# ufukpage/TripleD-Exploring-Depth-Estimation-with-Self-Supervised-Representation-Learning

Hardware: AMD Instinct MI355X
Metric: train imgs/sec at KITTI 192x640 bs=12/GPU (higher is better)
Workload: dtype bf16 convs (MFMA) + f32 loss kernels

## Files before the change

include/tripled_hip.h:

```cpp
#ifndef TRIPLED_HIP_H
#define TRIPLED_HIP_H

#include <stddef.h>
#include <stdint.h>

#ifdef __cplusplus
extern "C" {
#endif

#define TD_ABI_VERSION 3
#define TD_MAX_SRC 4

#define TD_OK 0
#define TD_ERR_BAD_ARG (-1)
#define TD_ERR_UNSUPPORTED (-2)
#define TD_ERR_LAUNCH (-3)
#define TD_ERR_WORKSPACE (-4)

typedef void* td_stream_t;

int td_abi_version(void);
const char* td_error_string(int code);
const char* td_last_hip_error(void);

int td_photo_num_blocks(int B, int H, int W);
int td_photo_bwd_num_blocks(int B, int H, int W);

int td_pack_rgbx(const float* img, int B, int H, int W, float* out, td_stream_t stream);

int td_photo_identity(const float* tgt, const float* const* src, int n_src,
                      int B, int H, int W, float* idloss, float* tgt_rgbx, float* const* src_rgbx, td_stream_t stream);

int td_photo_fwd(const float* tgt, const float* const* src, int n_src,
                 const float* disp, const float* P, const float* invK,
                 const float* idloss, const float* noise,
                 int B, int H, int W, int hs, int ws,
                 float min_depth, float max_depth,
                 uint8_t* argmin, float* warped, float* min_map, float* partial, float* coef,
                 td_stream_t stream);

int td_photo_bwd(const float* tgt, const float* const* src, const float* tgt_rgbx, const float* const* src_rgbx, int n_src,
                 const float* disp, const float* P, const float* invK,
                 const uint8_t* argmin, const float* coef, int automask,
                 const float* gscale, float inv_count,
                 int B, int H, int W, int hs, int ws,
                 float min_depth, float max_depth,
                 float* d_up, float* dP_partial, td_stream_t stream);

int td_upsample_adjoint(const float* d_up, int B, int H, int W, int hs, int ws,
                        float* d_disp, int accumulate, td_stream_t stream);
int td_upsample_adjoint_planes(const float* d_up, int n_planes, int B, int H, int W, int hs, int ws,
                               float* d_disp, int accumulate, td_stream_t stream);

int td_reduce_dP(const float* dP_partial, int n_src, int B, int H, int W,
                 float* dP , td_stream_t stream);

int td_sum_scaled(const float* partial, int n, float scale, float* out, td_stream_t stream);

int td_area_downsample(const float* img, int B, int C, int H, int W, int h, int w,
                       float* out, td_stream_t stream);

int td_smooth_num_blocks(int B, int h, int w);

int td_smooth_fwd(const float* disp, const float* img, int B, int h, int w, int normalize,
                  float* mean, float* partial, td_stream_t stream);

int td_smooth_finish(const float* partial, int B, int h, int w, float weight, float* loss,
                     td_stream_t stream);

int td_smooth_bwd(const float* disp, const float* img, const float* mean,
                  int B, int h, int w, int normalize,
                  const float* gscale, float weight,
                  float* g_hat, float* dot_partial, float* d_disp, int accumulate,
                  td_stream_t stream);

#define TD_DTYPE_F32 0
#define TD_DTYPE_BF16 1

int td_maxpool5_fwd(const void* in, int dtype, int N, int H, int W, int C, void* out, uint8_t* idx,
                    td_stream_t stream);
int td_maxpool5_bwd(const void* grad_out, const uint8_t* idx, int dtype, int N, int H, int W, int C,
                    void* grad_in, td_stream_t stream);
int td_maxpool5_bwd_add(const void* grad_out, const uint8_t* idx, const void* add, int dtype, int N, int H, int W, int C,
                        void* grad_in, td_stream_t stream);

int td_maxpool3s2_fwd(const void* in, int dtype, int N, int H, int W, int C, void* out, uint8_t* idx,
                      td_stream_t stream);
int td_maxpool3s2_bwd(const void* grad_out, const uint8_t* idx, int dtype, int N, int H, int W, int C,
                      void* grad_in, td_stream_t stream);

int td_join_fwd(const void* a, const void* b, const void* tail, int dtype, long long npix, int C0, int C1, int C2,
                void* out, td_stream_t stream);
int td_join_bwd(const void* grad_out, int dtype, long long npix, int C0, int C1, int C2, void* grad_a, void* grad_b,
                void* grad_tail, td_stream_t stream);
int td_join_up2_fwd(const void* a, const void* b_half, const void* tail, int dtype, int N, int H, int W, int C0, int C1,
                    int C2, void* out, td_stream_t stream);
int td_join_up2_bwd(const void* grad_out, int dtype, int N, int H, int W, int C0, int C1, int C2, void* grad_a,
                    void* grad_b_half, void* grad_tail, td_stream_t stream);

long long td_bn_workspace_floats(long long M, int groups, int C);
int td_bn_fwd(const void* x, const void* residual, int dtype, const float* gamma, const float* beta,
              float* running_mean, float* running_var, float momentum, float eps, int relu, long long M, int groups,
              int C, void* y, float* save_mean, float* save_invstd, float* workspace, td_stream_t stream);
int td_bn_bwd(const void* dy, const void* x, const void* y, int dtype, const float* gamma, const float* beta, const float* save_mean,
              const float* save_invstd, int relu, long long M, int groups, int C, void* dx, void* dresidual,
              float* dgamma, float* dbeta, float* workspace, td_stream_t stream);

int td_conv1x1_stat_rows(long long M, int groups, int N);
int td_conv1x1_fwd(const void* x, const void* w, long long M, int groups, int K, int N, int Hi, int Wi, int stride, void* y,
                   float* stat_partials, td_stream_t stream);
int td_conv3x3_fwd(const void* x, const void* w, int B, int groups, int Hi, int Wi, int Cin, int N, int stride, int pad, void* y,
                   float* stat_partials, td_stream_t stream);
long long td_conv3x3_wgrad_workspace_floats(int B, int Ho, int Wo, int C, int N);
int td_conv3x3_wgrad(const void* dy, const void* x, int B, int Ho, int Wo, int C, int N, int pad, int dw_dtype, void* dw,
                     float* workspace, td_stream_t stream);
long long td_conv1x1_wgrad_workspace_floats(long long M, int K, int N);
int td_conv1x1_wgrad(const void* dy, const void* x, long long M, int K, int N, int Hi, int Wi, int stride, int dw_dtype, void* dw,
                     float* workspace, td_stream_t stream);
int td_conv1x1_wgrad_group(int n, const void* const* dy, const void* const* x, const long long* M, const int* K, const int* N,
                           const int* Hi, const int* Wi, const int* stride, const int* dw_dtype, void* const* dw,
                           float* const* workspace, td_stream_t stream);
int td_bn_fwd_from_partials(const void* x, const void* residual, int dtype, const float* gamma, const float* beta,
                            float* running_mean, float* running_var, float momentum, float eps, int relu, long long M,
                            int groups, int C, float* partials, int stat_rows, void* y, float* save_mean,
                            float* save_invstd, td_stream_t stream);

long long td_bias_act_workspace_floats(long long M, int C);
int td_bias_act_fwd(const void* y, const void* bias, int bias_dtype, int dtype, long long M, int C, int act, void* a, td_stream_t stream);
int td_bias_act_bwd(const void* g, const void* a, int dtype, long long M, int C, int act, void* gy, void* dbias, int dbias_dtype,
                    float* workspace, td_stream_t stream);

int td_adam_flat(float* w, const float* grad, float* exp_avg, float* exp_avg_sq, void* lowp, long long n, long long n_lowp,
                 const float* step, const float* lr_dev, float lr_host, double beta1, double beta2, float eps, const float* total_norm,
                 float max_norm, td_stream_t stream);

int td_gather_flat(const void* const* srcs, const long long* dst_offsets, const long long* numels, int n, int src_dtype, float* flat,
                   td_stream_t stream);

int td_bn_partial_rows(long long M, int groups, int C);
int td_bn_fwd_partials(const void* x, int dtype, long long M, int groups, int C, float* partials, td_stream_t stream);
int td_bn_bwd_partials(const void* dy, const void* x, const void* y, int dtype, const float* gamma, const float* beta,
                       const float* save_mean, const float* save_invstd, int relu, long long M, int groups, int C, float* partials,
                       td_stream_t stream);
int td_bn_bwd_from_partials(const void* dy, const void* x, const void* y, int dtype, const float* gamma, const float* beta,
                            const float* save_mean, const float* save_invstd, int relu, long long M, int groups, int C,
                            float* partials, int stat_rows, void* dx, void* dresidual, float* dgamma, float* dbeta,
                            td_stream_t stream);
int td_conv1x1_fwd_bnrelu(const void* z, const void* w, long long M, int groups, int K, int N, float* in_partials, int in_rows,
                          const float* gamma, const float* beta, float* running_mean, float* running_var, float momentum, float eps,
                          float* save_mean, float* save_invstd, void* a_side, void* y, float* stat_partials, td_stream_t stream);
int td_conv1x1_dgrad(const void* dy, const void* w, long long M, int groups, int Cout, int Cin, const void* residual, void* dx,
                     td_stream_t stream);
int td_conv1x1_fwd_sum(const void* x, const void* w, long long M, int K, int N, const void* run_in, void* y, void* run_out,
                       td_stream_t stream);
int td_conv1x1_dgrad_bnsums(const void* dy, const void* w, long long M, int groups, int Cout, int Cin, const void* z,
                            const float* gamma, const float* beta, const float* save_mean, const float* save_invstd, void* dx,
                            float* out_partials, td_stream_t stream);
int td_conv1x1_dgrad_bnbwd(const void* g, const void* z, const void* w, long long M, int groups, int Cout, int Cin, float* in_partials,
                           int in_rows, const float* gamma, const float* beta, const float* save_mean, const float* save_invstd,
                           float* dgamma, float* dbeta, void* dz_side, const void* residual, void* dx, td_stream_t stream);

int td_bn_sync_fwd_sums(const void* x, int dtype, long long M, int groups, int C, float* sums, float* workspace,
                        td_stream_t stream);
int td_bn_sync_fwd_apply(const void* x, const void* residual, int dtype, const float* sums, const float* count,
                         const float* gamma, const float* beta, float* running_mean, float* running_var, float momentum,
                         float eps, int relu, long long M, int groups, int C, void* y, float* save_mean,
                         float* save_invstd, td_stream_t stream);
int td_bn_sync_bwd_sums(const void* dy, const void* x, const void* y, int dtype, const float* gamma, const float* beta,
                        const float* save_mean, const float* save_invstd, int relu, long long M, int groups, int C,
                        float* sums, float* workspace, td_stream_t stream);
int td_bn_sync_bwd_dx(const void* dy, const void* x, const void* y, int dtype, const float* local_sums,
                      const float* global_sums, const float* count, const float* gamma, const float* beta,
                      const float* save_mean, const float* save_invstd, int relu, long long M, int groups, int C,
                      void* dx, void* dresidual, float* dgamma, float* dbeta, float* coef, td_stream_t stream);

int td_edge_weights(const float* img, int B, int h, int w, float a, const float* scale6, float* Wt,
                    td_stream_t stream);
int td_featreg_num_blocks(int B, int h, int w, int C);
int td_featreg_fwd(const void* feat, int dtype, const float* Wt, int B, int h, int w, int C,
                   float* partial, td_stream_t stream);
int td_featreg_bwd(const void* feat, int dtype, const float* Wt, const float* gscale, int B, int h, int w,
                   int C, void* grad, td_stream_t stream);

int td_recon_num_tasks(int B, int h, int w);
int td_recon_fwd(const float* x, const float* y, const float* hole, int B, int h, int w,
                 float* partial, td_stream_t stream);
int td_recon_bwd(const float* x, const float* y, const float* hole, const float* gscale, int B, int h,
                 int w, float* dx, td_stream_t stream);

int td_reflpad1_fwd(const void* in, int dtype, int N, int H, int W, int C, void* out, td_stream_t stream);
int td_reflpad1_bwd(const void* grad_out, int dtype, int N, int H, int W, int C, void* grad_in,
                    td_stream_t stream);

int td_up2_reflpad1_fwd(const void* in, int dtype, int N, int H, int W, int C, void* out, td_stream_t stream);
int td_up2_reflpad1_bwd(const void* grad_out, int dtype, int N, int H, int W, int C, void* grad_in,
                        td_stream_t stream);

int td_featwarp_num_blocks(int B, int h, int w);
int td_featwarp_fwd(const void* tgt, const void* const* src, int n_src, int dtype, const float* disp,
                    const float* P, const float* invK, int B, int h, int w, int C, int hs, int ws,
                    float min_depth, float max_depth, uint8_t* argmin, float* partial, td_stream_t stream);
int td_featwarp_bwd(const void* tgt, const void* const* src, int n_src, int dtype, const float* disp,
                    const float* P, const float* invK, const uint8_t* argmin, const float* gscale,
                    float inv_count, int B, int h, int w, int C, int hs, int ws, float min_depth,
                    float max_depth, void* d_tgt, int* const* d_src, float* d_up, float* dP_partial,
                    td_stream_t stream);
int td_featwarp_dsrc_finish(const int* acc, const float* gscale, float inv_count, int C, long long n, int dtype, void* out,
                            td_stream_t stream);
int td_reduce_partials(const float* partial, int n_src, int B, int blocks_per_sample, float* dP,
                       td_stream_t stream);

int td_l1map_fwd(const void* pred, int dtype, const long long* pred_strides, const float* target, int B, int C,
                 int H, int W, float weight, float* out, td_stream_t stream);
int td_l1map_bwd(const void* pred, int dtype, const long long* pred_strides, const float* target,
                 const float* gmap, int B, int C, int H, int W, float weight, void* dpred, td_stream_t stream);

int td_rgb2lab(const float* rgb, int B, int H, int W, float l_cent, float l_norm, float ab_norm, float* lab,
               td_stream_t stream);

int td_pose_fwd(const float* axisangle, const float* translation, const int* invert, const float* K,
                int n_pairs, int B, float* T, float* P, td_stream_t stream);
int td_pose_bwd(const float* axisangle, const float* translation, const int* invert, const float* K,
                int n_pairs, int B, const float* gT, const float* gP, float* g_axisangle,
                float* g_translation, td_stream_t stream);

int td_color_jitter(const uint8_t* frames_u8, const float* aug, int N, int H, int W, float* means_scratch, float* color,
                    float* color_aug, td_stream_t stream);

int td_fp8_num_blocks(long long n);
int td_fp8_amax_partials(const void* x, int dtype, long long n, float* partials, td_stream_t stream);
int td_fp8_quantize(const void* x, int dtype, long long n, const float* partials, uint8_t* q, float* inv_scale,
                    td_stream_t stream);

int td_infer_preprocess(const uint8_t* img_u8, int B, int H0, int W0, int h, int w, int mirror, float* out,
                        td_stream_t stream);
int td_disp_postprocess(const void* disp, int dtype, int B, int h, int w, int paired, int H0, int W0, float a, float b,
                        float depth_scale, float* disp_out, float* depth_out, td_stream_t stream);
int td_colorize(const float* x, int B, long long n, const float* vmin, const float* vmax, const uint8_t* lut, uint8_t* out,
                td_stream_t stream);

#define TD_STEREO_SCALE_FACTOR 36
long long td_eval_depth_workspace_bytes(int B, int Hmax, int Wmax);
int td_eval_depth(const void* disp, int dtype, int B, int h, int w, float a, float b, const float* gt, int Hmax, int Wmax,
                  const int* sizes, const int* crops, float min_depth, float max_depth, int stereo, void* workspace,
                  long long workspace_bytes, float* metrics, int* counts, td_stream_t stream);
long long td_masked_median_workspace_bytes(int B);
int td_masked_median(const float* values, int B, long long n, void* workspace, long long workspace_bytes, float* median,
                     int* count, td_stream_t stream);

int td_pose_pairs_u8(const uint8_t* frames, int n, int H, int W, int first, int count, int dtype, void* out, long long out_first,
                     td_stream_t stream);
int td_odom_trajectory(const void* rel, int rel_f64, int n, double* poses, td_stream_t stream);
int td_odom_snippet_ate(const void* rel, int rel_f64, const double* gt_poses, int n, int track_length, double* ates,
                        td_stream_t stream);
int td_odom_sequence_errors(const double* gt_poses, const double* pred_poses, int m, const double* lengths, int n_lengths, int step,
                            int align_scale, double* dist, double* rows, uint8_t* valid, double* summary, td_stream_t stream);

int td_lanczos_resize_u8(const uint8_t* src, const int* meta, const int* meta_host, const int* tables, long long table_ints,
                         const int* desc, int n_sizes, int N, int Hc, int Wc, int H, int W, uint8_t* dst, int* status,
                         td_stream_t stream);

int td_lanczos_resize_u8_indexed(const uint8_t* store, long long store_bytes, const long long* offsets, const long long* offsets_host,
                                 const int* meta, const int* meta_host, const int* tables, long long table_ints, const int* desc,
                                 int n_sizes, int N, int H, int W, uint8_t* dst, int* status, td_stream_t stream);

int td_cloud_keys(const float* depth, const uint8_t* color, const double* poses, const double* inv_K, int B, int H, int W,
                  double depth_scale, double pose_scale, double inv_voxel, int stride, int border, double min_depth, double max_range,
                  float edge, long long* key, unsigned long long* payload, long long* stats, td_stream_t stream);
int td_cloud_heads(const long long* keys, long long N, int* flags, td_stream_t stream);
int td_cloud_reduce_packed(const long long* keys, const long long* seg, const long long* perm, const unsigned long long* payload,
                           long long n_src, long long N, long long V, long long* out_keys, long long* sums, td_stream_t stream);
int td_cloud_reduce_rows(const long long* keys, const long long* seg, const long long* perm, const long long* rows, long long n_src,
                         long long N, long long V, long long* out_keys, long long* sums, td_stream_t stream);
int td_cloud_finish(const long long* keys, const long long* sums, long long V, double voxel, long long min_count, float* xyz,
                    uint8_t* rgb, int* count, uint8_t* keep, td_stream_t stream);

int td_cloud_views(const float* depth, const double* poses, const double* K, const double* inv_K, int N, int H, int W, int c0, int c1,
                   int lo, int hi, int radius, int min_views, double tol, double depth_scale, double pose_scale, double min_depth,
                   double max_range, long long* key, unsigned long long* payload, uint8_t* votes, long long* stats, td_stream_t stream);

long long td_velo_depth_workspace_bytes(int B, int Hmax, int Wmax);
int td_velo_depth(const float* points, const long long* offsets, int B, const double* P, const int* sizes, int Hmax, int Wmax,
                  int vel_depth, void* workspace, long long workspace_bytes, float* gt, long long* stats, td_stream_t stream);

long long td_cloud_render_workspace_bytes(int C, int H, int W);
int td_cloud_render(const float* xyz, const uint8_t* rgb, long long V, const double* poses, const double* K, int C, int H, int W,
                    double pose_scale, double z_near, double z_far, double splat, int ortho, int bg_r, int bg_g, int bg_b,
                    void* workspace, long long workspace_bytes, float* depth, uint8_t* color, int* index, long long* stats,
                    td_stream_t stream);

int td_scan_keys(const float* points, long long n, const long long* offsets, int S, const double* Tr, const double* poses,
                 const double* K, int H, int W, double min_depth, double max_range, double inv_voxel, long long* key,
                 unsigned long long* payload, long long* stats, td_stream_t stream);
int td_nn_query(const double* query, long long N, const double* points, const long long* order, long long M, const long long* cell_key,
                const long long* cell_start, long long C, double tau, const double* thr2, int K, double* d2, long long* index,
                long long* counts, td_stream_t stream);

int td_cloud_transform(const double* src, long long N, double c, const double* R, const double* t, double* out, td_stream_t stream);
long long td_icp_moments_workspace(long long N);
int td_icp_moments(const double* cur, long long N, const double* ref, long long M, const long long* index, const double* d2, double trim2,
                   const double* origin, void* workspace, long long workspace_bytes, double* out, td_stream_t stream);

int td_cloud_normals(const double* query, long long N, const double* points, long long M, const long long* cell_key,
                     const long long* cell_start, long long C, double tau, double radius, double Q, long long min_neighbours,
                     double max_curvature, double* normal, double* curvature, long long* count, long long* counters, td_stream_t stream);
long long td_icp_plane_moments_workspace(long long N);
int td_icp_plane_moments(const double* cur, long long N, const double* ref, const double* normals, long long M, const long long* index,
                         const double* d2, double trim2, const double* origin, void* workspace, long long workspace_bytes, double* out,
                         td_stream_t stream);

int td_normals_orient(const float* xyz, const float* normal, long long V, const double* poses, int C, double pose_scale,
                      float* out_normal, int* camera, long long* stats, td_stream_t stream);
int td_cloud_render_surfels(const float* xyz, const uint8_t* rgb, const float* normal, long long V, const double* poses, const double* K,
// ... 9 lines not shown
```

tripled-exploring-depth-estimation-with-self-supervised-representation-learning_amd/csrc/td_bn.hip:

```cpp
#include <hip/hip_bf16.h>

#include "td_common.h"
#include "td_vec8.h"

namespace td {

constexpr int BN_RY = 32;
constexpr int BN_UNROLL = 4;
constexpr int BN_THREADS = 256;

template <typename T, int MODE>
__global__ __launch_bounds__(BN_THREADS) void bn_partials_kernel(const T* __restrict__ x, const T* __restrict__ dy,
                                                                 const T* __restrict__ y, const float* __restrict__ mean,
                                                                 const float* __restrict__ invstd, const float* __restrict__ gamma,
                                                                 const float* __restrict__ beta,
                                                                 long long M, int C, int rows_per_split, int relu,
                                                                 float* __restrict__ ws) {
  __shared__ float lds[2][BN_RY][64 + 1];
  const int tid = threadIdx.x, cx = tid & 7, ry = tid >> 3;
  const int cg = blockIdx.x, s = blockIdx.y, grp = blockIdx.z;
  const long long base = (long long)grp * M;
  const long long r0 = base + (long long)s * rows_per_split;
  const long long r1 = (r0 + rows_per_split < base + M) ? r0 + rows_per_split : base + M;
  const size_t col = (size_t)cg * 64 + (size_t)cx * 8;
  ws += (size_t)grp * gridDim.y * C * 2;
  if (MODE == 1) { mean += (size_t)grp * C; invstd += (size_t)grp * C; }
  float a[8], b[8], mu[8], sc[8], sh[8];
#pragma unroll
  for (int i = 0; i < 8; ++i) { a[i] = 0.f; b[i] = 0.f; mu[i] = 0.f; sc[i] = 0.f; sh[i] = 0.f; }
  if (MODE == 1) {
#pragma unroll
    for (int i = 0; i < 8; ++i) mu[i] = mean[col + i];
    if (relu == 2) {
#pragma unroll
      for (int i = 0; i < 8; ++i) {
        sc[i] = gamma[col + i] * invstd[col + i];
        sh[i] = beta[col + i] - mu[i] * sc[i];
      }
    }
  }
  for (long long r = r0 + ry; r < r1; r += BN_UNROLL * BN_RY) {
    float vx[BN_UNROLL][8], vg[BN_UNROLL][8], vy[BN_UNROLL][8];
    bool ok[BN_UNROLL];
#pragma unroll
    for (int u = 0; u < BN_UNROLL; ++u) {
      const long long rr = r + (long long)u * BN_RY;
      ok[u] = rr < r1;
      const size_t off = (size_t)(ok[u] ? rr : r) * C + col;
      load8(x + off, vx[u]);
      if (MODE == 1) {
        load8(dy + off, vg[u]);
        if (relu == 1) load8(y + off, vy[u]);
      }
    }
#pragma unroll
    for (int u = 0; u < BN_UNROLL; ++u) {
#pragma unroll
      for (int i = 0; i < 8; ++i) {
        if (MODE == 0) {
          const float t = ok[u] ? vx[u][i] : 0.f;
          a[i] += t;
          b[i] = fmaf(t, t, b[i]);
        } else {
          float g = vg[u][i];
          if (relu == 1) g = vy[u][i] <= 0.f ? 0.f : g;
          if (relu == 2) g = fmaf(vx[u][i], sc[i], sh[i]) <= 0.f ? 0.f : g;
          g = ok[u] ? g : 0.f;
          a[i] += g;
          b[i] = fmaf(g, vx[u][i] - mu[i], b[i]);
        }
      }
    }
  }
#pragma unroll
  for (int i = 0; i < 8; ++i) { lds[0][ry][cx * 8 + i] = a[i]; lds[1][ry][cx * 8 + i] = b[i]; }
  __syncthreads();
  if (tid < 128) {
    const int which = tid >> 6, c = tid & 63;
    float acc = 0.f;
#pragma unroll
    for (int j = 0; j < BN_RY; ++j) acc += lds[which][j][c];
    ws[((size_t)s * C + (size_t)cg * 64 + c) * 2 + which] = acc;
  }
}

constexpr int BN_FIN_CH = 16;
constexpr int BN_FIN_PARTS = 16;
constexpr int BN_FIN_THREADS = BN_FIN_CH * BN_FIN_PARTS;
__device__ __forceinline__ void bn_sum_partials(const float* __restrict__ ws, int S, int C, int cg, float& A, float& B) {
  __shared__ float red[2][BN_FIN_PARTS][BN_FIN_CH];
  const int tid = threadIdx.x, c = tid % BN_FIN_CH, part = tid / BN_FIN_CH;
  float a = 0.f, b = 0.f;
  int s = part;
  for (; s + 11 * BN_FIN_PARTS < S; s += 12 * BN_FIN_PARTS) {
    float2 p[12];
#pragma unroll
    for (int u = 0; u < 12; ++u) p[u] = *reinterpret_cast<const float2*>(ws + ((size_t)(s + u * BN_FIN_PARTS) * C + (size_t)cg * BN_FIN_CH + c) * 2);
#pragma unroll
    for (int u = 0; u < 12; ++u) { a += p[u].x; b += p[u].y; }
  }
  for (; s < S; s += BN_FIN_PARTS) {
    const float2 p = *reinterpret_cast<const float2*>(ws + ((size_t)s * C + (size_t)cg * BN_FIN_CH + c) * 2);
    a += p.x;
    b += p.y;
  }
  red[0][part][c] = a;
  red[1][part][c] = b;
  __syncthreads();
  A = 0.f;
  B = 0.f;
  if (tid < BN_FIN_CH) {
#pragma unroll
    for (int j = 0; j < BN_FIN_PARTS; ++j) { A += red[0][j][c]; B += red[1][j][c]; }
  }
}

__global__ __launch_bounds__(BN_FIN_THREADS) void bn_shrink_kernel(float* __restrict__ ws, int S, int C, int Sq) {
  const int q = blockIdx.y, grp = blockIdx.z;
  float* w = ws + ((size_t)grp * S + (size_t)q * Sq) * C * 2;
  const int rows = S - q * Sq < Sq ? S - q * Sq : Sq;
  float A, B;
  bn_sum_partials(w, rows, C, blockIdx.x, A, B);
  if (threadIdx.x < BN_FIN_CH) {
    float* o = w + ((size_t)blockIdx.x * BN_FIN_CH + threadIdx.x) * 2;
    o[0] = A;
    o[1] = B;
  }
}

__global__ __launch_bounds__(64) void bn_stats_from_sums_kernel(const float* __restrict__ sums, const float* __restrict__ count,
                                                               int C, int G, float eps, float momentum,
                                                               float* __restrict__ running_mean, float* __restrict__ running_var,
                                                               float* __restrict__ save_mean, float* __restrict__ save_invstd) {
  const int c = blockIdx.x * 64 + threadIdx.x;
  if (c >= C) return;
  const double M = (double)count[0];
  for (int grp = 0; grp < G; ++grp) {
    const size_t i = (size_t)grp * C + c;
    const double m = (double)sums[i * 2] / M;
    double var = (double)sums[i * 2 + 1] / M - m * m;
    var = var > 0.0 ? var : 0.0;
    save_mean[i] = (float)m;
    save_invstd[i] = (float)(1.0 / sqrt(var + (double)eps));
    if (running_mean) {
      const double unbiased = M > 1.0 ? var * (M / (M - 1.0)) : var;
      running_mean[c] = (float)((1.0 - momentum) * running_mean[c] + momentum * m);
      running_var[c] = (float)((1.0 - momentum) * running_var[c] + momentum * unbiased);
    }
  }
}

__global__ __launch_bounds__(64) void bn_coef_from_sums_kernel(const float* __restrict__ local, const float* __restrict__ global,
                                                              const float* __restrict__ count, int C, int G,
                                                              const float* __restrict__ gamma, const float* __restrict__ mean,
                                                              const float* __restrict__ invstd, float* __restrict__ dgamma,
                                                              float* __restrict__ dbeta, float* __restrict__ coef) {
  const int c = blockIdx.x * 64 + threadIdx.x;
  if (c >= C) return;
  const float inv_m = 1.f / count[0];
  float dg_tot = 0.f, db_tot = 0.f;
  for (int grp = 0; grp < G; ++grp) {
    const size_t i = (size_t)grp * C + c;
    const float is = invstd[i], mu = mean[i];
    dg_tot += local[i * 2 + 1] * is;
    db_tot += local[i * 2];
    const float A = global[i * 2], dg = global[i * 2 + 1] * is;
    const float k0 = gamma[c] * is;
    const float k1 = -k0 * is * dg * inv_m;
    coef[i * 3 + 0] = k0;
    coef[i * 3 + 1] = k1;
    coef[i * 3 + 2] = -k0 * A * inv_m - k1 * mu;
  }
  dgamma[c] = dg_tot;
  dbeta[c] = db_tot;
}

constexpr int BN_PRO_MAX_S = 96;
constexpr int BN_PRO_PARTS = BN_THREADS / 64;
constexpr int BN_PRO_DEPTH = BN_PRO_MAX_S / BN_PRO_PARTS;
__device__ __forceinline__ void bn_tile_sums(const float* __restrict__ ws, int S, int stride, int C, int ct, float& A, float& B) {
  __shared__ float red[2][BN_PRO_PARTS][64];
  const int tid = threadIdx.x, c = tid & 63, part = tid >> 6;
  const float* p = ws + ((size_t)ct * 64 + c) * 2;
  float2 v[BN_PRO_DEPTH];
#pragma unroll
  for (int u = 0; u < BN_PRO_DEPTH; ++u) {
    const int row = part + BN_PRO_PARTS * u;
    v[u] = *reinterpret_cast<const float2*>(p + (size_t)(row < S ? row : 0) * stride * C * 2);
  }
  float a = 0.f, b = 0.f;
#pragma unroll
  for (int u = 0; u < BN_PRO_DEPTH; ++u) {
    const bool ok = part + BN_PRO_PARTS * u < S;
    a += ok ? v[u].x : 0.f;
    b += ok ? v[u].y : 0.f;
  }
  red[0][part][c] = a;
  red[1][part][c] = b;
  __syncthreads();
  A = 0.f;
  B = 0.f;
  if (tid < 64) {
#pragma unroll
    for (int j = 0; j < BN_PRO_PARTS; ++j) { A += red[0][j][c]; B += red[1][j][c]; }
  }
  __syncthreads();
}

struct BnFinFwd {
  const float* ws;
  int S, stride, rows, G;
  float eps, momentum;
  float* running_mean;
  float* running_var;
  float* save_mean;
  float* save_invstd;
};
struct BnFinBwd {
  const float* ws;
  int S, stride, rows, G;
  float* dgamma;
  float* dbeta;
};
// ... 122 lines not shown
  const int grp = blockIdx.z;
  const long long base = (long long)grp * M;
  const long long r0 = base + (long long)blockIdx.y * rows_per_split;
  const long long r1 = (r0 + rows_per_split < base + M) ? r0 + rows_per_split : base + M;
  const size_t col = (size_t)blockIdx.x * 64 + (size_t)cx * 8;
  Raw8<T> qx[BN_UNROLL], qg[BN_UNROLL], qy[BN_UNROLL];
  bool ok[BN_UNROLL];
#define BN_DX_ISSUE(rr0)                                                          \
  {                                                                               \
    _Pragma("unroll") for (int u = 0; u < BN_UNROLL; ++u) {                       \
      const long long rr = (rr0) + (long long)u * BN_RY;                          \
      ok[u] = rr < r1;                                                            \
      const size_t off = (size_t)(ok[u] ? rr : (rr0)) * C + col;                  \
      qx[u].load(x + off);                                                        \
      qg[u].load(dy + off);                                                       \
      if (relu == 1) qy[u].load(y + off);                                         \
    }                                                                             \
  }
  long long r = r0 + ry;
  if (r < r1) BN_DX_ISSUE(r)
  float k0[8], k1[8], k2[8];
  if constexpr (FIN) {
    __shared__ float s_k[3][64];
    const int c = blockIdx.x * 64 + (tid & 63);
    const float inv_m = 1.f / (float)M;
    float A, B;
    bn_tile_sums(fin.ws + (size_t)grp * fin.rows * C * 2, fin.S, fin.stride, C, blockIdx.x, A, B);
    if (tid < 64) {
      const float is = invstd[(size_t)grp * C + c], mu = mean[(size_t)grp * C + c];
      const float dg = B * is;
      const float c0 = gamma[c] * is;
      const float c1 = -c0 * is * dg * inv_m;
      s_k[0][tid] = c0;
      s_k[1][tid] = c1;
      s_k[2][tid] = -c0 * A * inv_m - c1 * mu;
    }
    if (blockIdx.y == 0 && blockIdx.z == 0) {
      float dg_tot = 0.f, db_tot = 0.f;
      for (int g2 = 0; g2 < fin.G; ++g2) {
        float A2 = A, B2 = B;
        if (g2 != 0) bn_tile_sums(fin.ws + (size_t)g2 * fin.rows * C * 2, fin.S, fin.stride, C, blockIdx.x, A2, B2);
        if (tid < 64) {
          dg_tot += B2 * invstd[(size_t)g2 * C + c];
          db_tot += A2;
        }
      }
      if (tid < 64) { fin.dgamma[c] = dg_tot; fin.dbeta[c] = db_tot; }
    }
    __syncthreads();
#pragma unroll
    for (int i = 0; i < 8; ++i) { k0[i] = s_k[0][cx * 8 + i]; k1[i] = s_k[1][cx * 8 + i]; k2[i] = s_k[2][cx * 8 + i]; }
  } else {
    coef += (size_t)grp * C * 3;
#pragma unroll
    for (int i = 0; i < 8; ++i) {
      k0[i] = coef[(col + i) * 3 + 0];
      k1[i] = coef[(col + i) * 3 + 1];
      k2[i] = coef[(col + i) * 3 + 2];
    }
  }
  mean += (size_t)grp * C;
  invstd += (size_t)grp * C;
  float sc[8], sh[8];
#pragma unroll
  for (int i = 0; i < 8; ++i) { sc[i] = 0.f; sh[i] = 0.f; }
  if (relu == 2) {
#pragma unroll
    for (int i = 0; i < 8; ++i) {
      sc[i] = gamma[col + i] * invstd[col + i];
      sh[i] = beta[col + i] - mean[col + i] * sc[i];
    }
  }
  for (; r < r1; r += BN_UNROLL * BN_RY) {
    float vx[BN_UNROLL][8], vg[BN_UNROLL][8], vy[BN_UNROLL][8];
    bool okc[BN_UNROLL];
#pragma unroll
    for (int u = 0; u < BN_UNROLL; ++u) {
      qx[u].unpack(vx[u]);
      qg[u].unpack(vg[u]);
      if (relu == 1) qy[u].unpack(vy[u]);
      okc[u] = ok[u];
    }
    const long long rn = r + BN_UNROLL * BN_RY;
    if (rn < r1) BN_DX_ISSUE(rn)
#pragma unroll
    for (int u = 0; u < BN_UNROLL; ++u) {
      float o[8], g[8];
#pragma unroll
      for (int i = 0; i < 8; ++i) {
        g[i] = vg[u][i];
        if (relu == 1) g[i] = vy[u][i] <= 0.f ? 0.f : g[i];
        if (relu == 2) g[i] = fmaf(vx[u][i], sc[i], sh[i]) <= 0.f ? 0.f : g[i];
        o[i] = fmaf(k0[i], g[i], fmaf(k1[i], vx[u][i], k2[i]));
      }
      if (okc[u]) {
        const size_t off = (size_t)(r + (long long)u * BN_RY) * C + col;
        store8(dx + off, o);
        if (dres) store8(dres + off, g);
      }
    }
  }
#undef BN_DX_ISSUE
}

constexpr int BN_STAT_BLOCKS = 512;
static inline int bn_splits(long long M, int C, int target_blocks, int cap) {
  const int groups = C / 64;
  long long s = (target_blocks + groups - 1) / groups;
  const long long by_rows = (M + 63) / 64;
  if (s > by_rows) s = by_rows;
  if (s > cap) s = cap;
  if (s < 1) s = 1;
  return (int)s;
}
static inline int bn_rows_per_split(long long M, int S) {
  const long long r = (M + S - 1) / S;
  return (int)((r + BN_RY - 1) / BN_RY * BN_RY);
}

BnRows bn_shrink_partials_to(float* partials, int S, int G, int C, int max_rows, hipStream_t st) {
  if (S <= max_rows) return {S, 1};
  const int Sq = (S + max_rows - 1) / max_rows, Q = (S + Sq - 1) / Sq;
  hipLaunchKernelGGL(bn_shrink_kernel, dim3(C / BN_FIN_CH, Q, G), dim3(BN_FIN_THREADS), 0, st, partials, S, C, Sq);
  return {Q, Sq};
}
static BnRows shrink_partials(float* partials, int S, int G, int C, hipStream_t st) {
  return bn_shrink_partials_to(partials, S, G, C, BN_PRO_MAX_S, st);
}

template <typename T>
static void launch_bn_finalize_apply(const void* x, const void* res, const float* gamma, const float* beta, float* rmean, float* rvar,
                                     float momentum, float eps, int relu, long long Mg, int G, int C, float* partials, int S, void* y,
                                     float* save_mean, float* save_invstd, hipStream_t st) {
  const BnRows rows = shrink_partials(partials, S, G, C, st);
  const int S2 = bn_splits(Mg, C, BN_STAT_BLOCKS, 4096), rps2 = bn_rows_per_split(Mg, S2);
  const dim3 grid(C / 64, (unsigned)((Mg + rps2 - 1) / rps2), G);
  const BnFinFwd fin = {partials, rows.n, rows.stride, S, G, eps, momentum, rmean, rvar, save_mean, save_invstd};
  hipLaunchKernelGGL((bn_apply_kernel<T, true>), grid, dim3(BN_THREADS), 0, st, (const T*)x, (const T*)res, gamma, beta,
                     (const float*)nullptr, (const float*)nullptr, Mg, C, rps2, relu, (T*)y, fin);
}

static inline int bn_stat_splits(long long Mg, int C) {
  const int S = bn_splits(Mg, C, BN_STAT_BLOCKS, 512);
  if (S > 16 && (C / 64) * 16 >= 128) return bn_splits(Mg, C, (C / 64) * 16, 16);
  return S;
}
static inline int bn_stat_rows(long long Mg, int C) {
  const int S = bn_stat_splits(Mg, C), rps = bn_rows_per_split(Mg, S);
  return (int)((Mg + rps - 1) / rps);
}

template <typename T>
static int run_bn_partials(int mode, const void* x, const void* dy, const void* y, const float* gamma, const float* beta, const float* mean,
                           const float* invstd, int relu, long long M, int G, int C, float* ws, hipStream_t st) {
  const long long Mg = M / G;
  const int S = bn_stat_splits(Mg, C), rps = bn_rows_per_split(Mg, S);
  const int S_eff = (int)((Mg + rps - 1) / rps);
  if (mode == 0)
    hipLaunchKernelGGL((bn_partials_kernel<T, 0>), dim3(C / 64, S_eff, G), dim3(BN_THREADS), 0, st, (const T*)x, (const T*)nullptr,
                       (const T*)nullptr, (const float*)nullptr, (const float*)nullptr, (const float*)nullptr, (const float*)nullptr, Mg, C,
                       rps, 0, ws);
  else
    hipLaunchKernelGGL((bn_partials_kernel<T, 1>), dim3(C / 64, S_eff, G), dim3(BN_THREADS), 0, st, (const T*)x, (const T*)dy,
                       (const T*)y, mean, invstd, gamma, beta, Mg, C, rps, relu, ws);
  return hipGetLastError() == hipSuccess ? TD_OK : TD_ERR_LAUNCH;
}

template <typename T>
static int run_bn_dx_from_partials(const void* dy, const void* x, const void* y, const float* gamma, const float* beta, const float* mean,
                                   const float* invstd, int relu, long long M, int G, int C, float* partials, int S, void* dx, void* dres,
                                   float* dgamma, float* dbeta, hipStream_t st) {
  const long long Mg = M / G;
  const BnRows rows = shrink_partials(partials, S, G, C, st);
  const int S2 = bn_splits(Mg, C, BN_STAT_BLOCKS, 4096), rps2 = bn_rows_per_split(Mg, S2);
  const dim3 grid(C / 64, (unsigned)((Mg + rps2 - 1) / rps2), G);
  const BnFinBwd fin = {partials, rows.n, rows.stride, S, G, dgamma, dbeta};
  hipLaunchKernelGGL((bn_dx_kernel<T, true>), grid, dim3(BN_THREADS), 0, st, (const T*)dy, (const T*)x, (const T*)y, (const float*)nullptr,
                     mean, invstd, gamma, beta, Mg, C, rps2, relu, (T*)dx, (T*)dres, fin);
  return hipGetLastError() == hipSuccess ? TD_OK : TD_ERR_LAUNCH;
}

template <typename T>
static int run_bn_fwd(const void* x, const void* res, const float* gamma, const float* beta, float* rmean, float* rvar,
                      float momentum, float eps, int relu, long long M, int G, int C, void* y, float* save_mean, float* save_invstd,
                      float* ws, hipStream_t st) {
  const long long Mg = M / G;
  const int S = bn_splits(Mg, C, BN_STAT_BLOCKS, 512), rps = bn_rows_per_split(Mg, S);
  const int S_eff = (int)((Mg + rps - 1) / rps);
  hipLaunchKernelGGL((bn_partials_kernel<T, 0>), dim3(C / 64, S_eff, G), dim3(BN_THREADS), 0, st, (const T*)x, (const T*)nullptr,
                     (const T*)nullptr, (const float*)nullptr, (const float*)nullptr, (const float*)nullptr, (const float*)nullptr, Mg, C, rps, 0, ws);
  launch_bn_finalize_apply<T>(x, res, gamma, beta, rmean, rvar, momentum, eps, relu, Mg, G, C, ws, S_eff, y, save_mean, save_invstd, st);
  return hipGetLastError() == hipSuccess ? TD_OK : TD_ERR_LAUNCH;
}

template <typename T>
static int run_bn_bwd(const void* dy, const void* x, const void* y, const float* gamma, const float* beta, const float* mean, const float* invstd,
                      int relu, long long M, int G, int C, void* dx, void* dres, float* dgamma, float* dbeta, float* ws, hipStream_t st) {
  const long long Mg = M / G;
  const int S = bn_splits(Mg, C, BN_STAT_BLOCKS, 512), rps = bn_rows_per_split(Mg, S);
  const int S_eff = (int)((Mg + rps - 1) / rps);
  hipLaunchKernelGGL((bn_partials_kernel<T, 1>), dim3(C / 64, S_eff, G), dim3(BN_THREADS), 0, st, (const T*)x, (const T*)dy,
                     (const T*)y, mean, invstd, gamma, beta, Mg, C, rps, relu, ws);
  const BnRows rows = shrink_partials(ws, S_eff, G, C, st);
  const int S2 = bn_splits(Mg, C, BN_STAT_BLOCKS, 4096), rps2 = bn_rows_per_split(Mg, S2);
  const dim3 grid(C / 64, (unsigned)((Mg + rps2 - 1) / rps2), G);
  const BnFinBwd fin = {ws, rows.n, rows.stride, S_eff, G, dgamma, dbeta};
  hipLaunchKernelGGL((bn_dx_kernel<T, true>), grid, dim3(BN_THREADS), 0, st, (const T*)dy, (const T*)x, (const T*)y, (const float*)nullptr,
                     mean, invstd, gamma, beta, Mg, C, rps2, relu, (T*)dx, (T*)dres, fin);
  return hipGetLastError() == hipSuccess ? TD_OK : TD_ERR_LAUNCH;
}

template <typename T>
static int run_bn_local_sums(int mode, const void* x, const void* dy, const void* y, const float* gamma, const float* beta,
                             const float* mean, const float* invstd, int relu, long long M, int G, int C, float* sums, float* ws,
                             hipStream_t st) {
  const long long Mg = M / G;
  const int S = bn_splits(Mg, C, BN_STAT_BLOCKS, 512), rps = bn_rows_per_split(Mg, S);
  const int S_eff = (int)((Mg + rps - 1) / rps);
  if (mode == 0)
    hipLaunchKernelGGL((bn_partials_kernel<T, 0>), dim3(C / 64, S_eff, G), dim3(BN_THREADS), 0, st, (const T*)x, (const T*)nullptr,
                       (const T*)nullptr, (const float*)nullptr, (const float*)nullptr, (const float*)nullptr, (const float*)nullptr, Mg, C,
                       rps, 0, ws);
  else
    hipLaunchKernelGGL((bn_partials_kernel<T, 1>), dim3(C / 64, S_eff, G), dim3(BN_THREADS), 0, st, (const T*)x, (const T*)dy,
                       (const T*)y, mean, invstd, gamma, beta, Mg, C, rps, relu, ws);
  const BnRows rows = shrink_partials(ws, S_eff, G, C, st);
  hipLaunchKernelGGL(bn_tile_reduce_kernel, dim3(C / 64), dim3(BN_THREADS), 0, st, (const float*)ws, rows.n, rows.stride, S_eff, C, G, sums);
  return hipGetLastError() == hipSuccess ? TD_OK : TD_ERR_LAUNCH;
}

template <typename T>
static int run_bn_sync_apply(const void* x, const void* res, const float* sums, const float* count, const float* gamma, const float* beta,
                             float* rmean, float* rvar, float momentum, float eps, int relu, long long M, int G, int C, void* y,
                             float* save_mean, float* save_invstd, hipStream_t st) {
  const long long Mg = M / G;
  hipLaunchKernelGGL(bn_stats_from_sums_kernel, dim3(C / 64), dim3(64), 0, st, sums, count, C, G, eps, momentum, rmean, rvar, save_mean,
                     save_invstd);
  const int S2 = bn_splits(Mg, C, 2048 / G, 4096), rps2 = bn_rows_per_split(Mg, S2);
  hipLaunchKernelGGL((bn_apply_kernel<T, false>), dim3(C / 64, (unsigned)((Mg + rps2 - 1) / rps2), G), dim3(BN_THREADS), 0, st, (const T*)x,
                     (const T*)res, gamma, beta, (const float*)save_mean, (const float*)save_invstd, Mg, C, rps2, relu, (T*)y, BnFinFwd{});
  return hipGetLastError() == hipSuccess ? TD_OK : TD_ERR_LAUNCH;
}

template <typename T>
static int run_bn_sync_dx(const void* dy, const void* x, const void* y, const float* local, const float* global, const float* count,
                          const float* gamma, const float* beta, const float* mean, const float* invstd, int relu, long long M, int G,
                          int C, void* dx, void* dres, float* dgamma, float* dbeta, float* coef, hipStream_t st) {
  const long long Mg = M / G;
  hipLaunchKernelGGL(bn_coef_from_sums_kernel, dim3(C / 64), dim3(64), 0, st, local, global, count, C, G, gamma, mean, invstd, dgamma, dbeta,
                     coef);
  const int S2 = bn_splits(Mg, C, 2048 / G, 4096), rps2 = bn_rows_per_split(Mg, S2);
  hipLaunchKernelGGL((bn_dx_kernel<T, false>), dim3(C / 64, (unsigned)((Mg + rps2 - 1) / rps2), G), dim3(BN_THREADS), 0, st, (const T*)dy,
                     (const T*)x, (const T*)y, (const float*)coef, mean, invstd, gamma, beta, Mg, C, rps2, relu, (T*)dx, (T*)dres, BnFinBwd{});
  return hipGetLastError() == hipSuccess ? TD_OK : TD_ERR_LAUNCH;
}

}

static bool bn_shape_ok(long long M, int G, int C) { return G >= 1 && G <= 64 && M > 0 && C > 0 && M % G == 0; }

extern "C" long long td_bn_workspace_floats(long long M, int groups, int C) {
  if (!bn_shape_ok(M, groups, C) || C % 64 != 0) return 0;
  const int S = td::bn_splits(M / groups, C, td::BN_STAT_BLOCKS, 512);
  return ((long long)2 * S * C + (long long)3 * C) * groups;
}

extern "C" int td_bn_fwd(const void* x, const void* residual, int dtype, const float* gamma, const float* beta,
                         float* running_mean, float* running_var, float momentum, float eps, int relu, long long M, int groups,
                         int C, void* y, float* save_mean, float* save_invstd, float* workspace, td_stream_t stream) {
  if (!x || !gamma || !beta || !y || !save_mean || !save_invstd || !workspace || !bn_shape_ok(M, groups, C)) return TD_ERR_BAD_ARG;
  if ((running_mean == nullptr) != (running_var == nullptr)) return TD_ERR_BAD_ARG;
  if (C % 64 != 0 || M * (long long)C >= (1ll << 40)) return TD_ERR_UNSUPPORTED;
  if (dtype == TD_DTYPE_BF16)
    return td::run_bn_fwd<__hip_bfloat16>(x, residual, gamma, beta, running_mean, running_var, momentum, eps, relu, M, groups, C, y,
                                          save_mean, save_invstd, workspace, (hipStream_t)stream);
  if (dtype == TD_DTYPE_F32)
    return td::run_bn_fwd<float>(x, residual, gamma, beta, running_mean, running_var, momentum, eps, relu, M, groups, C, y, save_mean,
                                 save_invstd, workspace, (hipStream_t)stream);
  return TD_ERR_UNSUPPORTED;
}

extern "C" int td_bn_bwd(const void* dy, const void* x, const void* y, int dtype, const float* gamma, const float* beta, const float* save_mean,
                         const float* save_invstd, int relu, long long M, int groups, int C, void* dx, void* dresidual,
                         float* dgamma, float* dbeta, float* workspace, td_stream_t stream) {
  if (!dy || !x || !gamma || !save_mean || !save_invstd || !dx || !dgamma || !dbeta || !workspace || !bn_shape_ok(M, groups, C))
    return TD_ERR_BAD_ARG;
  if (relu < 0 || relu > 1) return TD_ERR_BAD_ARG;
  if (relu && !y && (!beta || dresidual)) return TD_ERR_BAD_ARG;
  if (relu && !y) relu = 2;
  if (C % 64 != 0 || M * (long long)C >= (1ll << 40)) return TD_ERR_UNSUPPORTED;
  if (dtype == TD_DTYPE_BF16)
    return td::run_bn_bwd<__hip_bfloat16>(dy, x, y, gamma, beta, save_mean, save_invstd, relu, M, groups, C, dx, dresidual, dgamma, dbeta,
                                          workspace, (hipStream_t)stream);
  if (dtype == TD_DTYPE_F32)
    return td::run_bn_bwd<float>(dy, x, y, gamma, beta, save_mean, save_invstd, relu, M, groups, C, dx, dresidual, dgamma, dbeta, workspace,
                                 (hipStream_t)stream);
  return TD_ERR_UNSUPPORTED;
}

extern "C" int td_bn_fwd_from_partials(const void* x, const void* residual, int dtype, const float* gamma, const float* beta,
                                       float* running_mean, float* running_var, float momentum, float eps, int relu, long long M,
                                       int groups, int C, float* partials, int stat_rows, void* y, float* save_mean,
                                       float* save_invstd, td_stream_t stream) {
  if (!x || !gamma || !beta || !y || !save_mean || !save_invstd || !partials || stat_rows < 1 || !bn_shape_ok(M, groups, C))
    return TD_ERR_BAD_ARG;
  if ((running_mean == nullptr) != (running_var == nullptr)) return TD_ERR_BAD_ARG;
  if (C % 64 != 0 || M * (long long)C >= (1ll << 40)) return TD_ERR_UNSUPPORTED;
  if (dtype != TD_DTYPE_BF16 && dtype != TD_DTYPE_F32) return TD_ERR_UNSUPPORTED;
  hipStream_t st = (hipStream_t)stream;
  const long long Mg = M / groups;
  if (dtype == TD_DTYPE_BF16)
    td::launch_bn_finalize_apply<__hip_bfloat16>(x, residual, gamma, beta, running_mean, running_var, momentum, eps, relu, Mg, groups, C, partials,
                                                 stat_rows, y, save_mean, save_invstd, st);
  else
    td::launch_bn_finalize_apply<float>(x, residual, gamma, beta, running_mean, running_var, momentum, eps, relu, Mg, groups, C, partials, stat_rows,
                                        y, save_mean, save_invstd, st);
  return hipGetLastError() == hipSuccess ? TD_OK : TD_ERR_LAUNCH;
}

extern "C" int td_bn_partial_rows(long long M, int groups, int C) {
  if (!bn_shape_ok(M, groups, C) || C % 64 != 0) return 0;
  return td::bn_stat_rows(M / groups, C);
}

extern "C" int td_bn_fwd_partials(const void* x, int dtype, long long M, int groups, int C, float* partials, td_stream_t stream) {
  if (!x || !partials || !bn_shape_ok(M, groups, C)) return TD_ERR_BAD_ARG;
  if (C % 64 != 0 || M * (long long)C >= (1ll << 40)) return TD_ERR_UNSUPPORTED;
  if (dtype == TD_DTYPE_BF16)
    return td::run_bn_partials<__hip_bfloat16>(0, x, nullptr, nullptr, nullptr, nullptr, nullptr, nullptr, 0, M, groups, C, partials, (hipStream_t)stream);
  if (dtype == TD_DTYPE_F32)
    return td::run_bn_partials<float>(0, x, nullptr, nullptr, nullptr, nullptr, nullptr, nullptr, 0, M, groups, C, partials, (hipStream_t)stream);
  return TD_ERR_UNSUPPORTED;
}

extern "C" int td_bn_bwd_partials(const void* dy, const void* x, const void* y, int dtype, const float* gamma, const float* beta,
                                  const float* save_mean, const float* save_invstd, int relu, long long M, int groups, int C,
                                  float* partials, td_stream_t stream) {
  if (!dy || !x || !gamma || !save_mean || !save_invstd || !partials || !bn_shape_ok(M, groups, C)) return TD_ERR_BAD_ARG;
  if (relu < 0 || relu > 1 || (relu && !y && !beta)) return TD_ERR_BAD_ARG;
  if (relu && !y) relu = 2;
  if (C % 64 != 0 || M * (long long)C >= (1ll << 40)) return TD_ERR_UNSUPPORTED;
  if (dtype == TD_DTYPE_BF16)
    return td::run_bn_partials<__hip_bfloat16>(1, x, dy, y, gamma, beta, save_mean, save_invstd, relu, M, groups, C, partials, (hipStream_t)stream);
  if (dtype == TD_DTYPE_F32)
    return td::run_bn_partials<float>(1, x, dy, y, gamma, beta, save_mean, save_invstd, relu, M, groups, C, partials, (hipStream_t)stream);
  return TD_ERR_UNSUPPORTED;
}

extern "C" int td_bn_bwd_from_partials(const void* dy, const void* x, const void* y, int dtype, const float* gamma, const float* beta,
                                       const float* save_mean, const float* save_invstd, int relu, long long M, int groups, int C,
                                       float* partials, int stat_rows, void* dx, void* dresidual, float* dgamma, float* dbeta,
                                       td_stream_t stream) {
  if (!dy || !x || !gamma || !save_mean || !save_invstd || !dx || !dgamma || !dbeta || !partials || stat_rows < 1 || !bn_shape_ok(M, groups, C))
    return TD_ERR_BAD_ARG;
  if (relu < 0 || relu > 1) return TD_ERR_BAD_ARG;
  if (relu && !y && (!beta || dresidual)) return TD_ERR_BAD_ARG;
  if (relu && !y) relu = 2;
  if (C % 64 != 0 || M * (long long)C >= (1ll << 40)) return TD_ERR_UNSUPPORTED;
  if (dtype == TD_DTYPE_BF16)
    return td::run_bn_dx_from_partials<__hip_bfloat16>(dy, x, y, gamma, beta, save_mean, save_invstd, relu, M, groups, C, partials, stat_rows,
                                                       dx, dresidual, dgamma, dbeta, (hipStream_t)stream);
  if (dtype == TD_DTYPE_F32)
    return td::run_bn_dx_from_partials<float>(dy, x, y, gamma, beta, save_mean, save_invstd, relu, M, groups, C, partials, stat_rows, dx,
                                              dresidual, dgamma, dbeta, (hipStream_t)stream);
  return TD_ERR_UNSUPPORTED;
}


extern "C" int td_bn_sync_fwd_sums(const void* x, int dtype, long long M, int groups, int C, float* sums, float* workspace,
                                   td_stream_t stream) {
  if (!x || !sums || !workspace || !bn_shape_ok(M, groups, C)) return TD_ERR_BAD_ARG;
  if (C % 64 != 0 || M * (long long)C >= (1ll << 40)) return TD_ERR_UNSUPPORTED;
  if (dtype == TD_DTYPE_BF16)
    return td::run_bn_local_sums<__hip_bfloat16>(0, x, nullptr, nullptr, nullptr, nullptr, nullptr, nullptr, 0, M, groups, C, sums, workspace,
                                                 (hipStream_t)stream);
  if (dtype == TD_DTYPE_F32)
    return td::run_bn_local_sums<float>(0, x, nullptr, nullptr, nullptr, nullptr, nullptr, nullptr, 0, M, groups, C, sums, workspace,
                                        (hipStream_t)stream);
  return TD_ERR_UNSUPPORTED;
}

extern "C" int td_bn_sync_fwd_apply(const void* x, const void* residual, int dtype, const float* sums, const float* count,
                                    const float* gamma, const float* beta, float* running_mean, float* running_var, float momentum,
                                    float eps, int relu, long long M, int groups, int C, void* y, float* save_mean, float* save_invstd,
                                    td_stream_t stream) {
  if (!x || !sums || !count || !gamma || !beta || !y || !save_mean || !save_invstd || !bn_shape_ok(M, groups, C)) return TD_ERR_BAD_ARG;
  if ((running_mean == nullptr) != (running_var == nullptr)) return TD_ERR_BAD_ARG;
  if (C % 64 != 0 || M * (long long)C >= (1ll << 40)) return TD_ERR_UNSUPPORTED;
  if (dtype == TD_DTYPE_BF16)
    return td::run_bn_sync_apply<__hip_bfloat16>(x, residual, sums, count, gamma, beta, running_mean, running_var, momentum, eps, relu, M,
                                                 groups, C, y, save_mean, save_invstd, (hipStream_t)stream);
  if (dtype == TD_DTYPE_F32)
    return td::run_bn_sync_apply<float>(x, residual, sums, count, gamma, beta, running_mean, running_var, momentum, eps, relu, M, groups, C,
                                        y, save_mean, save_invstd, (hipStream_t)stream);
  return TD_ERR_UNSUPPORTED;
}

extern "C" int td_bn_sync_bwd_sums(const void* dy, const void* x, const void* y, int dtype, const float* gamma, const float* beta,
                                   const float* save_mean, const float* save_invstd, int relu, long long M, int groups, int C,
                                   float* sums, float* workspace, td_stream_t stream) {
  if (!dy || !x || !gamma || !save_mean || !save_invstd || !sums || !workspace || !bn_shape_ok(M, groups, C)) return TD_ERR_BAD_ARG;
  if (relu < 0 || relu > 1 || (relu && !y && !beta)) return TD_ERR_BAD_ARG;
  if (relu && !y) relu = 2;
  if (C % 64 != 0 || M * (long long)C >= (1ll << 40)) return TD_ERR_UNSUPPORTED;
  if (dtype == TD_DTYPE_BF16)
    return td::run_bn_local_sums<__hip_bfloat16>(1, x, dy, y, gamma, beta, save_mean, save_invstd, relu, M, groups, C, sums, workspace,
                                                 (hipStream_t)stream);
  if (dtype == TD_DTYPE_F32)
    return td::run_bn_local_sums<float>(1, x, dy, y, gamma, beta, save_mean, save_invstd, relu, M, groups, C, sums, workspace,
                                        (hipStream_t)stream);
  return TD_ERR_UNSUPPORTED;
}

extern "C" int td_bn_sync_bwd_dx(const void* dy, const void* x, const void* y, int dtype, const float* local_sums, const float* global_sums,
                                 const float* count, const float* gamma, const float* beta, const float* save_mean,
                                 const float* save_invstd, int relu, long long M, int groups, int C, void* dx, void* dresidual,
                                 float* dgamma, float* dbeta, float* coef, td_stream_t stream) {
  if (!dy || !x || !local_sums || !global_sums || !count || !gamma || !save_mean || !save_invstd || !dx || !dgamma || !dbeta || !coef ||
      !bn_shape_ok(M, groups, C))
    return TD_ERR_BAD_ARG;
  if (relu < 0 || relu > 1 || (relu && !y && (!beta || dresidual))) return TD_ERR_BAD_ARG;
  if (relu && !y) relu = 2;
  if (C % 64 != 0 || M * (long long)C >= (1ll << 40)) return TD_ERR_UNSUPPORTED;
  if (dtype == TD_DTYPE_BF16)
    return td::run_bn_sync_dx<__hip_bfloat16>(dy, x, y, local_sums, global_sums, count, gamma, beta, save_mean, save_invstd, relu, M, groups,
                                              C, dx, dresidual, dgamma, dbeta, coef, (hipStream_t)stream);
  if (dtype == TD_DTYPE_F32)
    return td::run_bn_sync_dx<float>(dy, x, y, local_sums, global_sums, count, gamma, beta, save_mean, save_invstd, relu, M, groups, C, dx,
                                     dresidual, dgamma, dbeta, coef, (hipStream_t)stream);
  return TD_ERR_UNSUPPORTED;
}
```

tripled-exploring-depth-estimation-with-self-supervised-representation-learning_amd/csrc/td_conv1x1.hip:

```cpp
#include "td_conv_tile.h"

namespace td {

struct ConvRows {
  int Wo, HoWo, Wi, HiWi, stride;
};

__device__ __forceinline__ long long cv_src_row(long long m, const ConvRows& g) {
  if (g.stride == 1) return m;
  const long long b = m / g.HoWo;
  const int rem = (int)(m - b * g.HoWo);
  const int ho = rem / g.Wo, wo = rem - ho * g.Wo;
  return b * g.HiWi + (long long)ho * g.stride * g.Wi + (long long)wo * g.stride;
}

struct CvFuse {
  const __hip_bfloat16* a2;
  const float* part;
  int part_S, part_stride, part_rows;
  const float* gamma;
  const float* beta;
  float* mean;
  float* invstd;
  float* rmean;
  float* rvar;
  float momentum, eps;
  float* dgamma;
  float* dbeta;
  __hip_bfloat16* a_side;
  int G;
  CvEpi ep;
};

constexpr int CV_PRO_MAX_K = 512;
constexpr int CV_PRO_MAX_S = 16;

__device__ __forceinline__ uint4 cv_pro1(uint4 x, const float* sc, const float* sh) {
  const unsigned w[4] = {x.x, x.y, x.z, x.w};
  unsigned o[4];
#pragma unroll
  for (int e = 0; e < 4; ++e) {
    float v0 = fmaf(bf2f((unsigned short)(w[e] & 0xffff)), sc[2 * e], sh[2 * e]);
    float v1 = fmaf(bf2f((unsigned short)(w[e] >> 16)), sc[2 * e + 1], sh[2 * e + 1]);
    v0 = v0 < 0.f ? 0.f : v0;
    v1 = v1 < 0.f ? 0.f : v1;
    o[e] = (unsigned)f2bf(v0) | ((unsigned)f2bf(v1) << 16);
  }
  return make_uint4(o[0], o[1], o[2], o[3]);
}
__device__ __forceinline__ uint4 cv_pro2(uint4 g, uint4 z, const float* k0, const float* k1, const float* k2, const float* sc,
                                         const float* sh) {
  const unsigned gw[4] = {g.x, g.y, g.z, g.w}, zw[4] = {z.x, z.y, z.z, z.w};
  unsigned o[4];
#pragma unroll
  for (int e = 0; e < 4; ++e) {
    const float z0 = bf2f((unsigned short)(zw[e] & 0xffff)), z1 = bf2f((unsigned short)(zw[e] >> 16));
    float g0 = bf2f((unsigned short)(gw[e] & 0xffff)), g1 = bf2f((unsigned short)(gw[e] >> 16));
    g0 = fmaf(z0, sc[2 * e], sh[2 * e]) <= 0.f ? 0.f : g0;
    g1 = fmaf(z1, sc[2 * e + 1], sh[2 * e + 1]) <= 0.f ? 0.f : g1;
    const float v0 = fmaf(k0[2 * e], g0, fmaf(k1[2 * e], z0, k2[2 * e]));
    const float v1 = fmaf(k0[2 * e + 1], g1, fmaf(k1[2 * e + 1], z1, k2[2 * e + 1]));
    o[e] = (unsigned)f2bf(v0) | ((unsigned)f2bf(v1) << 16);
  }
  return make_uint4(o[0], o[1], o[2], o[3]);
}

__device__ __forceinline__ void cv_sum_rows(const float* __restrict__ part, int S, int stride, int K, int c, float& A, float& B) {
  float2 v[CV_PRO_MAX_S];
#pragma unroll
  for (int u = 0; u < CV_PRO_MAX_S; ++u)
    v[u] = *reinterpret_cast<const float2*>(part + ((size_t)(u < S ? u : 0) * stride * K + c) * 2);
  A = 0.f;
  B = 0.f;
#pragma unroll
  for (int u = 0; u < CV_PRO_MAX_S; ++u) {
    A += u < S ? v[u].x : 0.f;
    B += u < S ? v[u].y : 0.f;
  }
}

template <int BM, int BN, bool BT, int PRO, int EPI, bool DEEP>
__global__ __launch_bounds__(CV_THREADS, 2) void conv1x1_mfma_kernel(
    const __hip_bfloat16* __restrict__ x, const __hip_bfloat16* __restrict__ w, __hip_bfloat16* __restrict__ y,
    float* __restrict__ ws, long long Mg, int K, int N, int tiles_per_group, int total_blocks, ConvRows geom, CvFuse fz) {
  using T = CvTile<BM, BN, BT>;
  constexpr int A_BYTES = T::A_BYTES, STAGE = T::STAGE, TN = T::TN, TM = T::TM;
  __shared__ __attribute__((aligned(16))) unsigned char lds[T::LDS_BYTES];
  __shared__ __attribute__((aligned(16))) float s_pro[PRO == 0 ? 4 : (PRO == 1 ? 2 : 5) * CV_PRO_MAX_K];

  const int tid = threadIdx.x, lane = tid & 63, wid = tid >> 6;
  const int wm = wid >> 1, wn = wid & 1, l31 = lane & 31, h = lane >> 5;

  const int L = cv_xcd_tile(blockIdx.x, total_blocks);
  const int NT = N / BN;
  const int nt = L % NT, mt = L / NT;
  const int grp = mt / tiles_per_group, s = mt - grp * tiles_per_group;
  const long long row0 = (long long)grp * Mg + (long long)s * BM;
  const int rows_valid = (int)((Mg - (long long)s * BM) < BM ? (Mg - (long long)s * BM) : BM);
  const int n0 = nt * BN;

  const int lc = tid & 7, lr = tid >> 3;
  constexpr int NA = BM / 32, NB = BN / 32;
  auto a_off = [&](int i) {
    int r = lr + 32 * i;
    r = r < rows_valid ? r : rows_valid - 1;
    return cv_src_row(row0 + r, geom) * (long long)K + lc * 8;
  };
  const long long oa0 = a_off(0), oa1 = a_off(1), oa2 = NA > 2 ? a_off(2) : oa0, oa3 = NA > 2 ? a_off(3) : oa0;
  const __hip_bfloat16 *pa0 = x + oa0, *pa1 = x + oa1, *pa2 = x + oa2, *pa3 = x + oa3;
  constexpr int CPR = BN / 8, RPP = CV_THREADS / CPR;
  const int bc = tid % CPR, br = tid / CPR;
  const __hip_bfloat16* pb0 = BT ? w + (long long)br * N + n0 + bc * 8 : w + (long long)(n0 + lr) * K + lc * 8;
  const long long bstep = BT ? (long long)RPP * N : 32ll * K;
  const __hip_bfloat16 *pb1 = pb0 + bstep, *pb2 = pb0 + (NB > 2 ? 2 : 0) * bstep, *pb3 = pb0 + (NB > 2 ? 3 : 0) * bstep;
  const long long bkt = BT ? (long long)CV_BK * N : (long long)CV_BK;
#define CV_DECL(S)                                                                          \
  uint4 ra0##S, ra1##S, ra2##S, ra3##S, rb0##S, rb1##S, rb2##S, rb3##S, rz0##S, rz1##S, rz2##S, rz3##S; \
  ra0##S = ra1##S = ra2##S = ra3##S = rb0##S = rb1##S = rb2##S = rb3##S = make_uint4(0, 0, 0, 0);       \
  rz0##S = rz1##S = rz2##S = rz3##S = make_uint4(0, 0, 0, 0);
  CV_DECL(A)
  CV_DECL(B)
#define CV_LD(p, kt) (*reinterpret_cast<const uint4*>((p) + (kt) * CV_BK))
#define CV_LDB(p, kt) (*reinterpret_cast<const uint4*>((p) + (kt) * bkt))
#define CV_LOAD_GLOBAL(kt, S)                                  \
  {                                                            \
    ra0##S = CV_LD(pa0, kt);                                   \
    ra1##S = CV_LD(pa1, kt);                                   \
    if (NA > 2) { ra2##S = CV_LD(pa2, kt); ra3##S = CV_LD(pa3, kt); } \
    if constexpr (PRO == 2) {                                  \
      rz0##S = CV_LD(fz.a2 + oa0, kt);                         \
      rz1##S = CV_LD(fz.a2 + oa1, kt);                         \
      if (NA > 2) { rz2##S = CV_LD(fz.a2 + oa2, kt); rz3##S = CV_LD(fz.a2 + oa3, kt); } \
    }                                                          \
    rb0##S = CV_LDB(pb0, kt);                                  \
    rb1##S = CV_LDB(pb1, kt);                                  \
    if (NB > 2) { rb2##S = CV_LDB(pb2, kt); rb3##S = CV_LDB(pb3, kt); } \
  }
#define CV_ST(base, i, v) (*reinterpret_cast<uint4*>((base) + cv_swz(lr + 32 * (i), lc)) = (v))
#define CV_STB(base, i, v)                                                                              \
  {                                                                                                     \
    if constexpr (BT) *reinterpret_cast<uint4*>((base) + (br + RPP * (i)) * T::PITCH_T + bc * 16) = (v); \
    else CV_ST(base, i, v);                                                                             \
  }
#define CV_PRO_A(kt, S)                                                                                 \
  {                                                                                                     \
    if constexpr (PRO != 0) {                                                                           \
      const int c0_ = (kt) * CV_BK + lc * 8;                                                            \
      float q0[8], q1[8], q2[8], q3[8], q4[8];                                                          \
      _Pragma("unroll") for (int e = 0; e < 8; ++e) {                                                   \
        q0[e] = s_pro[0 * CV_PRO_MAX_K + c0_ + e];                                                      \
        q1[e] = s_pro[1 * CV_PRO_MAX_K + c0_ + e];                                                      \
        if constexpr (PRO == 2) {                                                                       \
          q2[e] = s_pro[2 * CV_PRO_MAX_K + c0_ + e];                                                    \
          q3[e] = s_pro[3 * CV_PRO_MAX_K + c0_ + e];                                                    \
          q4[e] = s_pro[4 * CV_PRO_MAX_K + c0_ + e];                                                    \
        }                                                                                               \
      }                                                                                                 \
      if constexpr (PRO == 1) {                                                                         \
        ra0##S = cv_pro1(ra0##S, q0, q1);                                                               \
        ra1##S = cv_pro1(ra1##S, q0, q1);                                                               \
        if (NA > 2) { ra2##S = cv_pro1(ra2##S, q0, q1); ra3##S = cv_pro1(ra3##S, q0, q1); }             \
      } else {                                                                                          \
        ra0##S = cv_pro2(ra0##S, rz0##S, q0, q1, q2, q3, q4);                                           \
        ra1##S = cv_pro2(ra1##S, rz1##S, q0, q1, q2, q3, q4);                                           \
        if (NA > 2) { ra2##S = cv_pro2(ra2##S, rz2##S, q0, q1, q2, q3, q4); ra3##S = cv_pro2(ra3##S, rz3##S, q0, q1, q2, q3, q4); } \
      }                                                                                                 \
      if (fz.a_side && nt == 0) {                                                                       \
        __hip_bfloat16* sd_ = fz.a_side + (row0 + lr) * (long long)K + c0_;                             \
        if (lr < rows_valid) *reinterpret_cast<uint4*>(sd_) = ra0##S;                                   \
        if (lr + 32 < rows_valid) *reinterpret_cast<uint4*>(sd_ + 32ll * K) = ra1##S;                   \
        if (NA > 2) {                                                                                   \
          if (lr + 64 < rows_valid) *reinterpret_cast<uint4*>(sd_ + 64ll * K) = ra2##S;                 \
          if (lr + 96 < rows_valid) *reinterpret_cast<uint4*>(sd_ + 96ll * K) = ra3##S;                 \
        }                                                                                               \
      }                                                                                                 \
    }                                                                                                   \
  }
#define CV_WRITE_LDS(stage, kt, S)                                       \
  {                                                                      \
    unsigned char* base_ = lds + (stage) * STAGE;                        \
    CV_PRO_A(kt, S)                                                      \
    CV_ST(base_, 0, ra0##S);                                             \
    CV_ST(base_, 1, ra1##S);                                             \
    if (NA > 2) { CV_ST(base_, 2, ra2##S); CV_ST(base_, 3, ra3##S); }    \
    CV_STB(base_ + A_BYTES, 0, rb0##S);                                  \
    CV_STB(base_ + A_BYTES, 1, rb1##S);                                  \
    if (NB > 2) { CV_STB(base_ + A_BYTES, 2, rb2##S); CV_STB(base_ + A_BYTES, 3, rb3##S); } \
  }

  CvAcc<BM, BN> acc;
#pragma unroll
  for (int i = 0; i < TN; ++i)
#pragma unroll
    for (int j = 0; j < TM; ++j)
#pragma unroll
      for (int e = 0; e < 16; ++e) acc.v[i][j][e] = 0.f;

  const int nk = K / CV_BK;
  CV_LOAD_GLOBAL(0, A)
  if constexpr (DEEP) CV_LOAD_GLOBAL(nk > 1 ? 1 : 0, B)

  if constexpr (PRO == 1) {
    const float* part = fz.part + (size_t)grp * fz.part_rows * K * 2;
    const bool first = (s == 0 && nt == 0);
    for (int c = tid; c < K; c += CV_THREADS) {
      float A, B;
      cv_sum_rows(part, fz.part_S, fz.part_stride, K, c, A, B);
      const double m = (double)A / (double)Mg;
      double var = (double)B / (double)Mg - m * m;
      var = var > 0.0 ? var : 0.0;
      const float mf = (float)m, isf = (float)(1.0 / sqrt(var + (double)fz.eps));
      const float scv = fz.gamma[c] * isf;
      s_pro[c] = scv;
      s_pro[CV_PRO_MAX_K + c] = fz.beta[c] - mf * scv;
      if (first) {
        fz.mean[(size_t)grp * K + c] = mf;
        fz.invstd[(size_t)grp * K + c] = isf;
      }
      if (fz.rmean && first && grp == 0) {
        double rm = fz.rmean[c], rv = fz.rvar[c];
        for (int g2 = 0; g2 < fz.G; ++g2) {
          float A2 = A, B2 = B;
          if (g2 != 0) cv_sum_rows(fz.part + (size_t)g2 * fz.part_rows * K * 2, fz.part_S, fz.part_stride, K, c, A2, B2);
          const double m2 = (double)A2 / (double)Mg;
          double v2 = (double)B2 / (double)Mg - m2 * m2;
          v2 = v2 > 0.0 ? v2 : 0.0;
          const double unbiased = Mg > 1 ? v2 * ((double)Mg / (double)(Mg - 1)) : v2;
          rm = (double)(float)((1.0 - fz.momentum) * rm + fz.momentum * m2);
          rv = (double)(float)((1.0 - fz.momentum) * rv + fz.momentum * unbiased);
        }
        fz.rmean[c] = (float)rm;
        fz.rvar[c] = (float)rv;
      }
    }
    __syncthreads();
  }
  if constexpr (PRO == 2) {
    const float* part = fz.part + (size_t)grp * fz.part_rows * K * 2;
    const float inv_m = 1.f / (float)Mg;
    const bool first = (s == 0 && nt == 0 && grp == 0);
    for (int c = tid; c < K; c += CV_THREADS) {
      float A, B;
      cv_sum_rows(part, fz.part_S, fz.part_stride, K, c, A, B);
      const float is = fz.invstd[(size_t)grp * K + c], mu = fz.mean[(size_t)grp * K + c];
      const float dg = B * is;
      const float c0 = fz.gamma[c] * is;
      const float c1 = -c0 * is * dg * inv_m;
      s_pro[0 * CV_PRO_MAX_K + c] = c0;
      s_pro[1 * CV_PRO_MAX_K + c] = c1;
      s_pro[2 * CV_PRO_MAX_K + c] = -c0 * A * inv_m - c1 * mu;
      s_pro[3 * CV_PRO_MAX_K + c] = c0;
      s_pro[4 * CV_PRO_MAX_K + c] = fz.beta[c] - mu * c0;
      if (first) {
        float dg_tot = 0.f, db_tot = 0.f;
        for (int g2 = 0; g2 < fz.G; ++g2) {
          float A2 = A, B2 = B;
          if (g2 != 0) cv_sum_rows(fz.part + (size_t)g2 * fz.part_rows * K * 2, fz.part_S, fz.part_stride, K, c, A2, B2);
          dg_tot += B2 * fz.invstd[(size_t)g2 * K + c];
          db_tot += A2;
        }
        fz.dgamma[c] = dg_tot;
        fz.dbeta[c] = db_tot;
      }
    }
    __syncthreads();
  }

  CV_WRITE_LDS(0, 0, A)
  __syncthreads();
  if constexpr (!DEEP) {
    for (int kt = 0; kt < nk; ++kt) {
      const bool more = kt + 1 < nk;
      if (more) CV_LOAD_GLOBAL(kt + 1, A)
      const unsigned char* sa = lds + (kt & 1) * STAGE;
      cv_stage_mfma<BM, BN, BT>(acc, sa, sa + A_BYTES, wm, wn, l31, h);
      if (more) CV_WRITE_LDS((kt + 1) & 1, kt + 1, A)
      __syncthreads();
    }
  } else {
    const int last = nk - 1;
    for (int kt = 0; kt < nk; kt += 2) {
      const int k2 = kt + 2 < last ? kt + 2 : last, k1 = kt + 1 < last ? kt + 1 : last, k3 = kt + 3 < last ? kt + 3 : last;
      CV_LOAD_GLOBAL(k2, A)
      __builtin_amdgcn_sched_barrier(0);
      cv_stage_mfma<BM, BN, BT>(acc, lds, lds + A_BYTES, wm, wn, l31, h);
      CV_WRITE_LDS(1, k1, B)
      __syncthreads();
      if (kt + 1 >= nk) break;
      CV_LOAD_GLOBAL(k3, B)
      __builtin_amdgcn_sched_barrier(0);
      cv_stage_mfma<BM, BN, BT>(acc, lds + STAGE, lds + STAGE + A_BYTES, wm, wn, l31, h);
      CV_WRITE_LDS(0, k2, A)
      __syncthreads();
    }
  }

  CvEpi ep = fz.ep;
  if constexpr (EPI == 2) { ep.mean += (size_t)grp * N; ep.invstd += (size_t)grp * N; }
  cv_epilogue<BM, BN, EPI>(acc, lds, y, ws, row0, rows_valid, n0, N, (long long)grp * tiles_per_group + s, tid, wm, wn, l31, h, ep);
}

#undef CV_LOAD_GLOBAL
#undef CV_DECL
#undef CV_WRITE_LDS
#undef CV_PRO_A
#undef CV_LD
#undef CV_LDB
#undef CV_ST
#undef CV_STB

constexpr int WG_T = 64;
constexpr int WG_PITCH = WG_T * 2 + 64;

typedef __attribute__((ext_vector_type(4))) short cv_s16x4;

__device__ __forceinline__ cv_bf16x8 wg_frag(const unsigned char* tile, int col0, int ks, int lane) {
  const int g = lane >> 4, i = lane & 15;
  const int row = 16 * ks + 8 * (g >> 1) + (i >> 2);
  const unsigned char* p = tile + row * WG_PITCH + (col0 + 16 * (g & 1) + 4 * (i & 3)) * 2;
  typedef __attribute__((address_space(3))) cv_s16x4* lds_ptr;
  const cv_s16x4 lo = __builtin_amdgcn_ds_read_tr16_b64_v4i16((lds_ptr)(p));
  const cv_s16x4 hi = __builtin_amdgcn_ds_read_tr16_b64_v4i16((lds_ptr)(p + 4 * WG_PITCH));
  typedef __attribute__((ext_vector_type(8))) short s16x8;
  const s16x8 v = {lo[0], lo[1], lo[2], lo[3], hi[0], hi[1], hi[2], hi[3]};
  return __builtin_bit_cast(cv_bf16x8, v);
}

constexpr int WG_TILE_BYTES = WG_T * WG_PITCH, WG_STAGE = 2 * WG_TILE_BYTES, WG_LDS_BYTES = 2 * WG_STAGE;

__device__ __forceinline__ void wgrad_block(
    const __hip_bfloat16* __restrict__ dy, const __hip_bfloat16* __restrict__ x, float* __restrict__ part, long long M, int K, int N,
    int rows_per_split, int tiles_n, int tiles_k, ConvRows geom, int L, unsigned char* lds) {
  constexpr int TILE_BYTES = WG_TILE_BYTES, STAGE = WG_STAGE;
  const int tid = threadIdx.x, lane = tid & 63, wid = tid >> 6;
  const int wn = wid >> 1, wk = wid & 1;
  const int nt = L % tiles_n, kt = (L / tiles_n) % tiles_k, sp = L / (tiles_n * tiles_k);
  const int n0 = nt * WG_T, k0 = kt * WG_T;
  const long long m_lo = (long long)sp * rows_per_split;
  const long long m_hi = (m_lo + rows_per_split < M) ? m_lo + rows_per_split : M;
  const int nstage = (int)((m_hi - m_lo + WG_T - 1) / WG_T);

  const int lc = tid & 7, lr = tid >> 3;
  uint4 ry0a, ry1a, rx0a, rx1a, ry0b, ry1b, rx0b, rx1b;
#define WG_LOAD(st, S)                                                                                             \
  {                                                                                                                \
    const long long r0 = m_lo + (long long)(st) * WG_T + lr, r1 = r0 + 32;                                         \
    const uint4 z = make_uint4(0, 0, 0, 0);                                                                        \
    ry0##S = r0 < m_hi ? *reinterpret_cast<const uint4*>(dy + r0 * N + n0 + lc * 8) : z;                           \
    ry1##S = r1 < m_hi ? *reinterpret_cast<const uint4*>(dy + r1 * N + n0 + lc * 8) : z;                           \
    rx0##S = r0 < m_hi ? *reinterpret_cast<const uint4*>(x + cv_src_row(r0, geom) * (long long)K + k0 + lc * 8) : z; \
    rx1##S = r1 < m_hi ? *reinterpret_cast<const uint4*>(x + cv_src_row(r1, geom) * (long long)K + k0 + lc * 8) : z; \
  }
#define WG_WRITE(buf, S)                                                                         \
  {                                                                                              \
    unsigned char* b_ = lds + (buf) * STAGE;                                                     \
    *reinterpret_cast<uint4*>(b_ + lr * WG_PITCH + lc * 16) = ry0##S;                            \
    *reinterpret_cast<uint4*>(b_ + (lr + 32) * WG_PITCH + lc * 16) = ry1##S;                     \
    *reinterpret_cast<uint4*>(b_ + TILE_BYTES + lr * WG_PITCH + lc * 16) = rx0##S;               \
    *reinterpret_cast<uint4*>(b_ + TILE_BYTES + (lr + 32) * WG_PITCH + lc * 16) = rx1##S;        \
  }
#define WG_MFMA(buf)                                                                             \
  {                                                                                              \
    const unsigned char* ty = lds + (buf) * STAGE;                                               \
    const unsigned char* tx = ty + TILE_BYTES;                                                   \
    _Pragma("unroll") for (int ks = 0; ks < WG_T / 16; ++ks) {                                   \
      const cv_bf16x8 fa = wg_frag(ty, wn * 32, ks, lane);                  \
      const cv_bf16x8 fb = wg_frag(tx, wk * 32, ks, lane);                  \
      acc = __builtin_amdgcn_mfma_f32_32x32x16_bf16(fa, fb, acc, 0, 0, 0);                       \
    }                                                                                            \
  }
  cv_f32x16 acc;
#pragma unroll
  for (int e = 0; e < 16; ++e) acc[e] = 0.f;
  WG_LOAD(0, a)
  if (nstage > 1) WG_LOAD(1, b)
  WG_WRITE(0, a)
  __syncthreads();
  for (int st = 0; st < nstage; st += 2) {
    if (st + 2 < nstage) WG_LOAD(st + 2, a)
    WG_MFMA(0)
    if (st + 1 < nstage) WG_WRITE(1, b)
    __syncthreads();
    if (st + 1 >= nstage) break;
    if (st + 3 < nstage) WG_LOAD(st + 3, b)
    WG_MFMA(1)
    if (st + 2 < nstage) WG_WRITE(0, a)
    __syncthreads();
  }
#undef WG_MFMA
#undef WG_LOAD
#undef WG_WRITE
  float* out = part + ((size_t)sp * N + n0 + wn * 32 + 4 * (lane >> 5)) * K + k0 + wk * 32 + (lane & 31);
#pragma unroll
  for (int r = 0; r < 16; ++r) out[(size_t)((r & 3) + 8 * (r >> 2)) * K] = acc[r];
}

__global__ __launch_bounds__(CV_THREADS, 2) void conv1x1_wgrad_kernel(
    const __hip_bfloat16* __restrict__ dy, const __hip_bfloat16* __restrict__ x, float* __restrict__ part, long long M, int K, int N,
    int rows_per_split, int tiles_n, int tiles_k, ConvRows geom) {
  __shared__ __attribute__((aligned(16))) unsigned char lds[WG_LDS_BYTES];
  wgrad_block(dy, x, part, M, K, N, rows_per_split, tiles_n, tiles_k, geom, cv_xcd_tile(blockIdx.x, gridDim.x), lds);
}

constexpr int WG_GROUP_MAX = 40;
struct WgProblem {
  const __hip_bfloat16* dy;
  const __hip_bfloat16* x;
  float* part;
  long long M;
  int K, N, rows_per_split, tiles_n, tiles_k;
  ConvRows geom;
};
struct WgGroupArgs {
  WgProblem p[WG_GROUP_MAX];
  int first_block[WG_GROUP_MAX + 1];
  int n;
};
__global__ __launch_bounds__(CV_THREADS, 2) void conv1x1_wgrad_group_kernel(const WgGroupArgs a) {
  __shared__ __attribute__((aligned(16))) unsigned char lds[WG_LDS_BYTES];
  const int L = cv_xcd_tile(blockIdx.x, gridDim.x);
  int lo = 0, hi = a.n;
  while (hi - lo > 1) {
    const int mid = (lo + hi) >> 1;
    if (a.first_block[mid] <= L) lo = mid; else hi = mid;
  }
  const WgProblem& q = a.p[lo];
  wgrad_block(q.dy, q.x, q.part, q.M, q.K, q.N, q.rows_per_split, q.tiles_n, q.tiles_k, q.geom, L - a.first_block[lo], lds);
}

template <typename T>
__global__ __launch_bounds__(TD_THREADS) void conv1x1_wgrad_reduce_kernel(const float* __restrict__ part, int P, long long NK, T* __restrict__ dw) {
  __shared__ float4 red[16][16];
  const int c = threadIdx.x & 15, g = threadIdx.x >> 4;
  const long long i = ((long long)blockIdx.x * 16 + c) * 4;
  float4 a = make_float4(0.f, 0.f, 0.f, 0.f);
  if (i < NK) {
    for (int p = g; p < P; p += 16) {
      const float4 b = *reinterpret_cast<const float4*>(part + (size_t)p * NK + i);
      a.x += b.x; a.y += b.y; a.z += b.z; a.w += b.w;
    }
  }
  red[g][c] = a;
  __syncthreads();
  if (g == 0 && i < NK) {
#pragma unroll
    for (int j = 1; j < 16; ++j) {
      const float4 b = red[j][c];
      a.x += b.x; a.y += b.y; a.z += b.z; a.w += b.w;
    }
    if constexpr (sizeof(T) == 2) {
      uint2 o;
      o.x = (unsigned)f2bf(a.x) | ((unsigned)f2bf(a.y) << 16);
      o.y = (unsigned)f2bf(a.z) | ((unsigned)f2bf(a.w) << 16);
      *reinterpret_cast<uint2*>(dw + i) = o;
    } else {
      *reinterpret_cast<float4*>(dw + i) = a;
    }
  }
}

constexpr int RD_GROUP_MAX = 96;
struct RdProblem {
  const float* part;
  void* dw;
  long long NK;
  int P, bf16;
};
struct RdGroupArgs {
  RdProblem p[RD_GROUP_MAX];
  int first_block[RD_GROUP_MAX + 1];
  int n;
};
__global__ __launch_bounds__(TD_THREADS) void conv1x1_wgrad_reduce_group_kernel(const RdGroupArgs a) {
  __shared__ float4 red[16][16];
  int lo = 0, hi = a.n;
  const int b = (int)blockIdx.x;
  while (hi - lo > 1) {
    const int mid = (lo + hi) >> 1;
    if (a.first_block[mid] <= b) lo = mid; else hi = mid;
  }
  const RdProblem& q = a.p[lo];
  const int c = threadIdx.x & 15, g = threadIdx.x >> 4;
  const long long i = ((long long)(b - a.first_block[lo]) * 16 + c) * 4;
  float4 s4 = make_float4(0.f, 0.f, 0.f, 0.f);
  if (i < q.NK) {
    for (int p = g; p < q.P; p += 16) {
      const float4 v = *reinterpret_cast<const float4*>(q.part + (size_t)p * q.NK + i);
      s4.x += v.x; s4.y += v.y; s4.z += v.z; s4.w += v.w;
    }
  }
  red[g][c] = s4;
  __syncthreads();
  if (g == 0 && i < q.NK) {
#pragma unroll
    for (int j = 1; j < 16; ++j) {
      const float4 v = red[j][c];
      s4.x += v.x; s4.y += v.y; s4.z += v.z; s4.w += v.w;
    }
    if (q.bf16) {
      uint2 o;
      o.x = (unsigned)f2bf(s4.x) | ((unsigned)f2bf(s4.y) << 16);
      o.y = (unsigned)f2bf(s4.z) | ((unsigned)f2bf(s4.w) << 16);
      *reinterpret_cast<uint2*>(reinterpret_cast<__hip_bfloat16*>(q.dw) + i) = o;
    } else {
      *reinterpret_cast<float4*>(reinterpret_cast<float*>(q.dw) + i) = s4;
    }
  }
}

int cv_wgrad_reduce(const float* part, int P, long long NK, int dw_dtype, void* dw, hipStream_t st) {
  const unsigned blocks = (unsigned)((NK / 4 + 15) / 16);
  if (dw_dtype == TD_DTYPE_BF16)
    hipLaunchKernelGGL((conv1x1_wgrad_reduce_kernel<__hip_bfloat16>), dim3(blocks), dim3(TD_THREADS), 0, st, part, P, NK, (__hip_bfloat16*)dw);
  else
    hipLaunchKernelGGL((conv1x1_wgrad_reduce_kernel<float>), dim3(blocks), dim3(TD_THREADS), 0, st, part, P, NK, (float*)dw);
  return hipGetLastError() == hipSuccess ? TD_OK : TD_ERR_LAUNCH;
}

static inline int wg_splits(long long M, int K, int N) {
  const long long tiles = (long long)(N / WG_T) * (K / WG_T);
  long long p = (768 + tiles - 1) / tiles;
  const long long by_rows = (M + 4 * WG_T - 1) / (4 * WG_T);
  if (p > by_rows) p = by_rows;
  if (p > 512) p = 512;
  return (int)(p < 1 ? 1 : p);
}

template <int BM, int BN, bool BT, int PRO, int EPI, bool DEEP>
static int cv_launch(const void* x, const void* w, void* y, float* ws, long long Mg, int G, int K, int N, ConvRows geom, hipStream_t st,
                     const CvFuse& fz) {
  const int tpg = (int)((Mg + BM - 1) / BM);
  const long long nblk = (long long)G * tpg * (N / BN);
  if (nblk > 0x7fffffffll) return TD_ERR_UNSUPPORTED;
  hipLaunchKernelGGL((conv1x1_mfma_kernel<BM, BN, BT, PRO, EPI, DEEP>), dim3((unsigned)nblk), dim3(CV_THREADS), 0, st, (const __hip_bfloat16*)x,
                     (const __hip_bfloat16*)w, (__hip_bfloat16*)y, ws, Mg, K, N, tpg, (int)nblk, geom, fz);
  return hipGetLastError() == hipSuccess ? TD_OK : TD_ERR_LAUNCH;
}

template <bool BT, int PRO, int EPI>
static int cv_dispatch(const void* x, const void* w, void* y, float* ws, long long M, int G, int K, int N, ConvRows geom, hipStream_t st,
                       const CvFuse& fz) {
  const long long Mg = M / G;
  ConvTile t = cv_pick_tile(Mg, G, N);
  const bool deep = K >= 3 * CV_BK;
  if constexpr (PRO == 2) {
    if (t.bm == 128 && t.bn == 128) t.bn = 64;
  } else
    if (t.bm == 128 && t.bn == 128) return cv_launch<128, 128, BT, PRO, EPI, false>(x, w, y, ws, Mg, G, K, N, geom, st, fz);
  if (t.bm == 128 && t.bn == 64) {
    if constexpr (PRO == 0)
      if (deep) return cv_launch<128, 64, BT, PRO, EPI, true>(x, w, y, ws, Mg, G, K, N, geom, st, fz);
    return cv_launch<128, 64, BT, PRO, EPI, false>(x, w, y, ws, Mg, G, K, N, geom, st, fz);
  }
  if (deep) return cv_launch<64, 64, BT, PRO, EPI, true>(x, w, y, ws, Mg, G, K, N, geom, st, fz);
  return cv_launch<64, 64, BT, PRO, EPI, false>(x, w, y, ws, Mg, G, K, N, geom, st, fz);
}

}

static bool cv_shape_ok(long long M, int G, int K, int N) {
  return M > 0 && G >= 1 && G <= 64 && M % G == 0 && K > 0 && N > 0 && K % 64 == 0 && N % 64 == 0;
}

extern "C" int td_conv1x1_stat_rows(long long M, int groups, int N) {
  if (M <= 0 || groups < 1 || M % groups != 0 || N <= 0 || N % 64 != 0) return 0;
  const td::ConvTile t = td::cv_pick_tile(M / groups, groups, N);
  return (int)((M / groups + t.bm - 1) / t.bm);
}

extern "C" int td_conv1x1_fwd(const void* x, const void* w, long long M, int groups, int K, int N, int Hi, int Wi, int stride, void* y,
                              float* stat_partials, td_stream_t stream) {
  if (!x || !w || !y || !cv_shape_ok(M, groups, K, N) || stride < 1) return TD_ERR_BAD_ARG;
  td::ConvRows geom = {0, 0, 0, 0, 1};
  if (stride > 1) {
    if (Hi <= 0 || Wi <= 0) return TD_ERR_BAD_ARG;
    const int Ho = (Hi - 1) / stride + 1, Wo = (Wi - 1) / stride + 1;
    if (M % ((long long)Ho * Wo) != 0) return TD_ERR_BAD_ARG;
    geom = {Wo, Ho * Wo, Wi, Hi * Wi, stride};
  }
  if (M * (long long)(K > N ? K : N) >= (1ll << 40)) return TD_ERR_UNSUPPORTED;
  return td::cv_dispatch<false, 0, 0>(x, w, y, stat_partials, M, groups, K, N, geom, (hipStream_t)stream, td::CvFuse{});
}

namespace td {
BnRows bn_shrink_partials_to(float* partials, int S, int G, int C, int max_rows, hipStream_t st);
}

extern "C" int td_conv1x1_fwd_bnrelu(const void* z, const void* w, long long M, int groups, int K, int N, float* in_partials,
                                     int in_rows, const float* gamma, const float* beta, float* running_mean, float* running_var,
                                     float momentum, float eps, float* save_mean, float* save_invstd, void* a_side, void* y,
                                     float* stat_partials, td_stream_t stream) {
  if (!z || !w || !y || !in_partials || in_rows < 1 || !gamma || !beta || !save_mean || !save_invstd || !cv_shape_ok(M, groups, K, N))
    return TD_ERR_BAD_ARG;
  if ((running_mean == nullptr) != (running_var == nullptr)) return TD_ERR_BAD_ARG;
  if (K > td::CV_PRO_MAX_K || M * (long long)(K > N ? K : N) >= (1ll << 40)) return TD_ERR_UNSUPPORTED;
  hipStream_t st = (hipStream_t)stream;
  const td::BnRows rows = td::bn_shrink_partials_to(in_partials, in_rows, groups, K, td::CV_PRO_MAX_S, st);
  td::CvFuse fz = {};
  fz.part = in_partials; fz.part_S = rows.n; fz.part_stride = rows.stride; fz.part_rows = in_rows;
  fz.gamma = gamma; fz.beta = beta; fz.mean = save_mean; fz.invstd = save_invstd; fz.rmean = running_mean; fz.rvar = running_var;
  fz.momentum = momentum; fz.eps = eps; fz.a_side = (__hip_bfloat16*)a_side; fz.G = groups;
  return td::cv_dispatch<false, 1, 0>(z, w, y, stat_partials, M, groups, K, N, td::ConvRows{0, 0, 0, 0, 1}, st, fz);
}

extern "C" int td_conv1x1_fwd_sum(const void* x, const void* w, long long M, int K, int N, const void* run_in, void* y, void* run_out,
                                  td_stream_t stream) {
  if (!x || !w || !y || !run_in || !run_out || !cv_shape_ok(M, 1, K, N)) return TD_ERR_BAD_ARG;
  if (M * (long long)(K > N ? K : N) >= (1ll << 40)) return TD_ERR_UNSUPPORTED;
  td::CvFuse fz = {};
  fz.ep.res = (const __hip_bfloat16*)run_in;
  fz.ep.y2 = (__hip_bfloat16*)run_out;
  return td::cv_dispatch<false, 0, 3>(x, w, y, nullptr, M, 1, K, N, td::ConvRows{0, 0, 0, 0, 1}, (hipStream_t)stream, fz);
}

extern "C" int td_conv1x1_dgrad(const void* dy, const void* w, long long M, int groups, int Cout, int Cin, const void* residual,
                                void* dx, td_stream_t stream) {
  if (!dy || !w || !dx || !cv_shape_ok(M, groups, Cout, Cin)) return TD_ERR_BAD_ARG;
  if (M * (long long)(Cout > Cin ? Cout : Cin) >= (1ll << 40)) return TD_ERR_UNSUPPORTED;
  td::CvFuse fz = {};
  fz.ep.res = (const __hip_bfloat16*)residual;
  const td::ConvRows geom = {0, 0, 0, 0, 1};
  if (residual) return td::cv_dispatch<true, 0, 1>(dy, w, dx, nullptr, M, groups, Cout, Cin, geom, (hipStream_t)stream, fz);
  return td::cv_dispatch<true, 0, 0>(dy, w, dx, nullptr, M, groups, Cout, Cin, geom, (hipStream_t)stream, fz);
}

extern "C" int td_conv1x1_dgrad_bnsums(const void* dy, const void* w, long long M, int groups, int Cout, int Cin, const void* z,
                                       const float* gamma, const float* beta, const float* save_mean, const float* save_invstd,
                                       void* dx, float* out_partials, td_stream_t stream) {
  if (!dy || !w || !dx || !z || !gamma || !beta || !save_mean || !save_invstd || !out_partials || !cv_shape_ok(M, groups, Cout, Cin))
    return TD_ERR_BAD_ARG;
  if (M * (long long)(Cout > Cin ? Cout : Cin) >= (1ll << 40)) return TD_ERR_UNSUPPORTED;
  td::CvFuse fz = {};
  fz.ep.z = (const __hip_bfloat16*)z; fz.ep.gamma = gamma; fz.ep.beta = beta; fz.ep.mean = save_mean; fz.ep.invstd = save_invstd;
  return td::cv_dispatch<true, 0, 2>(dy, w, dx, out_partials, M, groups, Cout, Cin, td::ConvRows{0, 0, 0, 0, 1}, (hipStream_t)stream, fz);
}

extern "C" int td_conv1x1_dgrad_bnbwd(const void* g, const void* z, const void* w, long long M, int groups, int Cout, int Cin,
                                      float* in_partials, int in_rows, const float* gamma, const float* beta, const float* save_mean,
                                      const float* save_invstd, float* dgamma, float* dbeta, void* dz_side, const void* residual,
                                      void* dx, td_stream_t stream) {
  if (!g || !z || !w || !dx || !in_partials || in_rows < 1 || !gamma || !beta || !save_mean || !save_invstd || !dgamma || !dbeta ||
      !cv_shape_ok(M, groups, Cout, Cin))
    return TD_ERR_BAD_ARG;
  if (Cout > td::CV_PRO_MAX_K || M * (long long)(Cout > Cin ? Cout : Cin) >= (1ll << 40)) return TD_ERR_UNSUPPORTED;
  hipStream_t st = (hipStream_t)stream;
  const td::BnRows rows = td::bn_shrink_partials_to(in_partials, in_rows, groups, Cout, td::CV_PRO_MAX_S, st);
  td::CvFuse fz = {};
  fz.a2 = (const __hip_bfloat16*)z; fz.part = in_partials; fz.part_S = rows.n; fz.part_stride = rows.stride; fz.part_rows = in_rows;
  fz.gamma = gamma; fz.beta = beta; fz.mean = const_cast<float*>(save_mean); fz.invstd = const_cast<float*>(save_invstd);
  fz.dgamma = dgamma; fz.dbeta = dbeta; fz.a_side = (__hip_bfloat16*)dz_side; fz.G = groups;
  fz.ep.res = (const __hip_bfloat16*)residual;
  const td::ConvRows geom = {0, 0, 0, 0, 1};
  if (residual) return td::cv_dispatch<true, 2, 1>(g, w, dx, nullptr, M, groups, Cout, Cin, geom, st, fz);
  return td::cv_dispatch<true, 2, 0>(g, w, dx, nullptr, M, groups, Cout, Cin, geom, st, fz);
}

extern "C" long long td_conv1x1_wgrad_workspace_floats(long long M, int K, int N) {
  if (M <= 0 || K <= 0 || N <= 0 || K % 64 != 0 || N % 64 != 0) return 0;
  return (long long)td::wg_splits(M, K, N) * N * K;
}

extern "C" int td_conv1x1_wgrad(const void* dy, const void* x, long long M, int K, int N, int Hi, int Wi, int stride, int dw_dtype,
                                void* dw, float* workspace, td_stream_t stream) {
  if (!dy || !x || !dw || !workspace || M <= 0 || K <= 0 || N <= 0 || K % 64 != 0 || N % 64 != 0 || stride < 1) return TD_ERR_BAD_ARG;
  if (dw_dtype != TD_DTYPE_BF16 && dw_dtype != TD_DTYPE_F32) return TD_ERR_UNSUPPORTED;
  td::ConvRows geom = {0, 0, 0, 0, 1};
  if (stride > 1) {
    if (Hi <= 0 || Wi <= 0) return TD_ERR_BAD_ARG;
    const int Ho = (Hi - 1) / stride + 1, Wo = (Wi - 1) / stride + 1;
    if (M % ((long long)Ho * Wo) != 0) return TD_ERR_BAD_ARG;
    geom = {Wo, Ho * Wo, Wi, Hi * Wi, stride};
  }
  if (M * (long long)(K > N ? K : N) >= (1ll << 40)) return TD_ERR_UNSUPPORTED;
  hipStream_t st = (hipStream_t)stream;
  const int P = td::wg_splits(M, K, N);
  long long rps = (M + P - 1) / P;
  rps = (rps + td::WG_T - 1) / td::WG_T * td::WG_T;
  const int P_eff = (int)((M + rps - 1) / rps);
  const int tn = N / td::WG_T, tk = K / td::WG_T;
  hipLaunchKernelGGL(td::conv1x1_wgrad_kernel, dim3((unsigned)(tn * tk * P_eff)), dim3(td::CV_THREADS), 0, st, (const __hip_bfloat16*)dy,
                     (const __hip_bfloat16*)x, workspace, M, K, N, (int)rps, tn, tk, geom);
  const long long NK = (long long)N * K;
  const unsigned blocks = (unsigned)((NK / 4 + 15) / 16);
  if (dw_dtype == TD_DTYPE_BF16)
    hipLaunchKernelGGL((td::conv1x1_wgrad_reduce_kernel<__hip_bfloat16>), dim3(blocks), dim3(TD_THREADS), 0, st, (const float*)workspace, P_eff,
                       NK, (__hip_bfloat16*)dw);
  else
    hipLaunchKernelGGL((td::conv1x1_wgrad_reduce_kernel<float>), dim3(blocks), dim3(TD_THREADS), 0, st, (const float*)workspace, P_eff, NK,
                       (float*)dw);
  return hipGetLastError() == hipSuccess ? TD_OK : TD_ERR_LAUNCH;
}

extern "C" int td_conv1x1_wgrad_group(int n, const void* const* dy, const void* const* x, const long long* M, const int* K, const int* N,
                                      const int* Hi, const int* Wi, const int* stride, const int* dw_dtype, void* const* dw,
                                      float* const* workspace, td_stream_t stream) {
  if (n < 0 || (n > 0 && (!dy || !x || !M || !K || !N || !Hi || !Wi || !stride || !dw_dtype || !dw || !workspace))) return TD_ERR_BAD_ARG;
  hipStream_t st = (hipStream_t)stream;
  for (int i = 0; i < n; ++i) {
    if (!dy[i] || !x[i] || !dw[i] || !workspace[i] || M[i] <= 0 || K[i] <= 0 || N[i] <= 0 || K[i] % 64 != 0 || N[i] % 64 != 0 || stride[i] < 1)
      return TD_ERR_BAD_ARG;
    if (dw_dtype[i] != TD_DTYPE_BF16 && dw_dtype[i] != TD_DTYPE_F32) return TD_ERR_UNSUPPORTED;
    if (M[i] * (long long)(K[i] > N[i] ? K[i] : N[i]) >= (1ll << 40)) return TD_ERR_UNSUPPORTED;
    if (stride[i] > 1) {
      if (Hi[i] <= 0 || Wi[i] <= 0) return TD_ERR_BAD_ARG;
      const int Ho = (Hi[i] - 1) / stride[i] + 1, Wo = (Wi[i] - 1) / stride[i] + 1;
      if (M[i] % ((long long)Ho * Wo) != 0) return TD_ERR_BAD_ARG;
    }
  }
  int P_eff[4096];
  if (n > 4096) return TD_ERR_UNSUPPORTED;
  for (int base = 0; base < n; base += td::WG_GROUP_MAX) {
    td::WgGroupArgs a;
    a.n = n - base < td::WG_GROUP_MAX ? n - base : td::WG_GROUP_MAX;
    long long blocks = 0;
    for (int j = 0; j < a.n; ++j) {
      const int i = base + j;
      td::ConvRows geom = {0, 0, 0, 0, 1};
      if (stride[i] > 1) {
        const int Ho = (Hi[i] - 1) / stride[i] + 1, Wo = (Wi[i] - 1) / stride[i] + 1;
        geom = {Wo, Ho * Wo, Wi[i], Hi[i] * Wi[i], stride[i]};
      }
      const int P = td::wg_splits(M[i], K[i], N[i]);
      long long rps = (M[i] + P - 1) / P;
      rps = (rps + td::WG_T - 1) / td::WG_T * td::WG_T;
      P_eff[i] = (int)((M[i] + rps - 1) / rps);
      td::WgProblem& q = a.p[j];
      q.dy = (const __hip_bfloat16*)dy[i]; q.x = (const __hip_bfloat16*)x[i]; q.part = workspace[i]; q.M = M[i]; q.K = K[i]; q.N = N[i];
      q.rows_per_split = (int)rps; q.tiles_n = N[i] / td::WG_T; q.tiles_k = K[i] / td::WG_T; q.geom = geom;
      a.first_block[j] = (int)blocks;
      blocks += (long long)q.tiles_n * q.tiles_k * P_eff[i];
      if (blocks > 0x7fffffffll) return TD_ERR_UNSUPPORTED;
    }
    for (int j = a.n; j <= td::WG_GROUP_MAX; ++j) a.first_block[j] = (int)blocks;
    hipLaunchKernelGGL(td::conv1x1_wgrad_group_kernel, dim3((unsigned)blocks), dim3(td::CV_THREADS), 0, st, a);
  }
  for (int base = 0; base < n; base += td::RD_GROUP_MAX) {
    td::RdGroupArgs a;
    a.n = n - base < td::RD_GROUP_MAX ? n - base : td::RD_GROUP_MAX;
    long long blocks = 0;
    for (int j = 0; j < a.n; ++j) {
      const int i = base + j;
      td::RdProblem& q = a.p[j];
      q.part = workspace[i]; q.dw = dw[i]; q.NK = (long long)N[i] * K[i]; q.P = P_eff[i]; q.bf16 = dw_dtype[i] == TD_DTYPE_BF16;
      a.first_block[j] = (int)blocks;
      blocks += (q.NK / 4 + 15) / 16;
    }
    for (int j = a.n; j <= td::RD_GROUP_MAX; ++j) a.first_block[j] = (int)blocks;
    hipLaunchKernelGGL(td::conv1x1_wgrad_reduce_group_kernel, dim3((unsigned)blocks), dim3(TD_THREADS), 0, st, a);
  }
  return hipGetLastError() == hipSuccess ? TD_OK : TD_ERR_LAUNCH;
}
```

tripled-exploring-depth-estimation-with-self-supervised-representation-learning_amd/hostside/mono/model/networks.py:

```python
import os

import numpy as np
import torch
import torch.nn as nn
import torch.nn.functional as F



FUSED_BN_OFF = bool(os.environ.get("TD_NO_FUSED_BN"))


def _ops():
    from tripled_amd import ops
    return ops


def _dense_cl(x):
    if x.is_cuda and x.dim() == 4 and x.shape[1] % 8 == 0 and x.dtype in (torch.float32, torch.bfloat16) \
            and not x.is_contiguous(memory_format=torch.channels_last) and x.stride(1) == 1:
        return x.contiguous(memory_format=torch.channels_last)
    return x


def _fell_back(site, x, why=""):
    if x.is_cuda and torch.is_grad_enabled():
        from tripled_amd import dispatch
        dispatch.fallback(site, why or "dtype %s, shape %s, channels_last %s" % (
            x.dtype, tuple(x.shape), x.dim() == 4 and x.is_contiguous(memory_format=torch.channels_last)))


class BatchNorm(nn.BatchNorm2d):

    _pending = 0
    _sync = None

    def _hip_ok_params(self):
        return bool(self.training and self.track_running_stats and self.momentum is not None and self.affine) and not FUSED_BN_OFF

    def _hip_ok(self, x):
        if not (x.is_cuda and self._hip_ok_params()):
            return False
        return _ops().batchnorm_act_supported(x, self.weight)

    def forward(self, x):
        if self.training and self.track_running_stats and self.momentum is not None:
            g = _BN_GROUPS[0]
            self._pending += g
            if self._hip_ok(x):
                if self._sync is not None:
                    return _ops().sync_batchnorm_act(x, self.weight, self.bias, self.running_mean, self.running_var,
                                                     self.momentum, self.eps, self._sync[0], groups=g)
                return _ops().batchnorm_act(x, self.weight, self.bias, self.running_mean, self.running_var,
                                            self.momentum, self.eps, groups=g)
            _fell_back("BatchNorm", x)
            if self._sync is not None:
                return _ATenSyncBatchNorm.apply(x, self.weight, self.bias, self.running_mean, self.running_var,
                                                self.momentum, self.eps, g, self._sync[0])
            if g > 1:
                return torch.cat([F.batch_norm(c, self.running_mean, self.running_var, self.weight, self.bias, True,
                                               self.momentum, self.eps) for c in x.chunk(g, 0)], 0)
            return F.batch_norm(x, self.running_mean, self.running_var, self.weight, self.bias, True,
                                self.momentum, self.eps)
        return super().forward(x)

    def fused(self, x, residual=None, relu=True):
        if self._hip_ok(x):
            g = _BN_GROUPS[0]
            self._pending += g
            if self._sync is not None:
                return _ops().sync_batchnorm_act(x, self.weight, self.bias, self.running_mean, self.running_var,
                                                 self.momentum, self.eps, self._sync[0], residual=residual, relu=relu, groups=g)
            return _ops().batchnorm_act(x, self.weight, self.bias, self.running_mean, self.running_var,
                                        self.momentum, self.eps, residual=residual, relu=relu, groups=g)
        return _plain_bn_act(self, x, residual, relu)


_BN_GROUPS = [1]


class _ATenSyncBatchNorm(torch.autograd.Function):

    @staticmethod
    def forward(ctx, x, weight, bias, running_mean, running_var, momentum, eps, groups, process_group):
        import torch.distributed as dist
        n, c = x.shape[0], x.shape[1]
        xs = x.float().reshape(groups, n // groups, c, -1)
        packed = torch.cat([xs.sum((1, 3)).reshape(-1), (xs * xs).sum((1, 3)).reshape(-1),
                            xs.new_full((1,), float(xs.shape[1] * xs.shape[3]))])
        dist.all_reduce(packed, op=dist.ReduceOp.SUM, group=process_group)
        count = packed[-1]
        mean = (packed[:groups * c] / count).reshape(groups, 1, c, 1)
        var = ((packed[groups * c:2 * groups * c] / count).reshape(groups, 1, c, 1) - mean * mean).clamp_min(0)
        invstd = torch.rsqrt(var + eps)
        if running_mean is not None:
            with torch.no_grad():
                for g in range(groups):
                    running_mean.mul_(1 - momentum).add_(momentum * mean[g].reshape(-1))
                    running_var.mul_(1 - momentum).add_(momentum * (var[g].reshape(-1) * (count / (count - 1))))
        xhat = (xs - mean) * invstd
        y = xhat * weight.float().reshape(1, 1, c, 1) + bias.float().reshape(1, 1, c, 1)
        ctx.save_for_backward(xhat, invstd, weight, count)
        ctx.shape, ctx.dtype, ctx.groups, ctx.group = x.shape, x.dtype, groups, process_group
        return y.reshape(x.shape).to(x.dtype)

    @staticmethod
    def backward(ctx, dy):
        import torch.distributed as dist
        xhat, invstd, weight, count = ctx.saved_tensors
        groups, c = ctx.groups, ctx.shape[1]
        g = dy.float().reshape(xhat.shape)
        sg, sgx = g.sum((1, 3)), (g * xhat).sum((1, 3))
        total = torch.cat([sg.reshape(-1), sgx.reshape(-1)])
        dist.all_reduce(total, op=dist.ReduceOp.SUM, group=ctx.group)
        tg = (total[:groups * c] / count).reshape(groups, 1, c, 1)
        tgx = (total[groups * c:] / count).reshape(groups, 1, c, 1)
        dx = (g - tg - xhat * tgx) * (invstd * weight.float().reshape(1, 1, c, 1))
        return (dx.reshape(ctx.shape).to(ctx.dtype), sgx.sum(0).to(weight.dtype), sg.sum(0).to(weight.dtype),
                None, None, None, None, None, None)


def enable_sync_batchnorm(model, process_group=None, force=False):
    import torch.distributed as dist
    if not (dist.is_available() and dist.is_initialized()):
        raise RuntimeError("enable_sync_batchnorm needs an initialised process group")
    if dist.get_world_size(process_group) == 1 and not force:
        return 0
    n = 0
    for m in model.modules():
        if isinstance(m, BatchNorm):
            m._sync = (process_group,)
            n += 1

    def foreign(parent):
        for name, child in parent.named_children():
            if isinstance(child, nn.modules.batchnorm._BatchNorm) and not isinstance(child, (BatchNorm, nn.SyncBatchNorm)):
                setattr(parent, name, nn.SyncBatchNorm.convert_sync_batchnorm(child, process_group))
            else:
                foreign(child)
    foreign(model)
    return n


class bn_groups:

    def __init__(self, groups):
        self.groups = int(groups)

    def __enter__(self):
        self.prev = _BN_GROUPS[0]
        _BN_GROUPS[0] = self.groups

    def __exit__(self, *exc):
        _BN_GROUPS[0] = self.prev
        return False


def bn_groups_supported(model):
    return not any(isinstance(m, nn.modules.batchnorm._BatchNorm) and not isinstance(m, BatchNorm)
                   for m in model.modules())


def _plain_bn_act(bn, x, residual, relu):
    y = bn(x)
    if residual is not None:
        y = y + residual
    return F.relu(y, inplace=True) if relu else y


def bn_act(bn, x, residual=None, relu=True):
    if isinstance(bn, BatchNorm):
        return bn.fused(x, residual, relu)
    return _plain_bn_act(bn, x, residual, relu)


FUSED_1X1_OFF = bool(os.environ.get("TD_NO_MFMA_1X1"))
FUSED_BLOCK_OFF = bool(os.environ.get("TD_NO_FUSED_BLOCK"))


def conv_bn_act(conv, bn, x, residual=None, relu=True):
    if (not FUSED_1X1_OFF and conv.kernel_size == (1, 1) and conv.padding == (0, 0) and conv.groups == 1 and conv.bias is None
            and conv.stride[0] == conv.stride[1] and isinstance(bn, BatchNorm) and bn._sync is None and not _FP8_1X1[0]
            and x.is_cuda and torch.is_autocast_enabled() and torch.get_autocast_gpu_dtype() == torch.bfloat16
            and bn._hip_ok_params()):
        xb = _dense_cl(x if x.dtype == torch.bfloat16 else x.to(torch.bfloat16))
        w = conv.weight if conv.weight.dtype == torch.bfloat16 else conv.weight.to(torch.bfloat16)
        if _ops().conv1x1_bn_act_supported(xb, w, bn.weight, conv.stride[0]):
            g = _BN_GROUPS[0]
            bn._pending += g
            return _ops().conv1x1_bn_act(xb, w, bn.weight, bn.bias, bn.running_mean, bn.running_var, bn.momentum, bn.eps,
                                         residual=residual, relu=relu, groups=g, stride=conv.stride[0])
    return bn_act(bn, conv(x), residual, relu)


def bump_batch_counters(model):
    counters, amounts = [], []
    for m in model.modules():
        if isinstance(m, BatchNorm) and m._pending:
            counters.append(m.num_batches_tracked)
            amounts.append(m._pending)
            m._pending = 0
    if counters:
        torch._foreach_add_(counters, amounts)


def install_counter_hook(model):
    def hook(module, args, output):
        if module.training:
            bump_batch_counters(module)
    model.register_forward_hook(hook)


RESNET_SPECS = {18: ("basic", (2, 2, 2, 2)), 34: ("basic", (3, 4, 6, 3)),
                50: ("bottleneck", (3, 4, 6, 3)), 101: ("bottleneck", (3, 4, 23, 3))}


_FP8_1X1 = [False]


def set_fp8_conv1x1(on):
    prev = _FP8_1X1[0]
    _FP8_1X1[0] = bool(on)
    return prev


class Conv2d(nn.Conv2d):

    def forward(self, x):
        if _FP8_1X1[0] and self.kernel_size == (1, 1) and self.stride == (1, 1) and self.padding == (0, 0) and self.groups == 1 \
                and x.is_cuda and torch.is_autocast_enabled():
            xb = x if x.dtype == torch.bfloat16 else x.to(torch.bfloat16)
            xb = _dense_cl(xb)
            if _ops().conv1x1_fp8_supported(xb, self.weight):
                return _ops().conv1x1_fp8(xb, self.weight, self.bias)
            _fell_back("Conv2d.fp8_1x1", x)
        return super().forward(x)


def _conv(cin, cout, k, stride=1, pad=0, bias=False):
    return Conv2d(cin, cout, kernel_size=k, stride=stride, padding=pad, bias=bias)


class BasicBlock(nn.Module):
    expansion = 1

    def __init__(self, inplanes, planes, stride=1, downsample=None, use_residual=True):
        super().__init__()
        self.conv1 = _conv(inplanes, planes, 3, stride, 1)
        self.bn1 = BatchNorm(planes)
        self.relu = nn.ReLU(inplace=True)
        self.conv2 = _conv(planes, planes, 3, 1, 1)
        self.bn2 = BatchNorm(planes)
        self.downsample = downsample
        self.stride = stride
        self.use_residual = use_residual

    def forward(self, x):
        y = bn_act(self.bn1, self.conv1(x))
        shortcut = None
        if self.use_residual:
            ds = self.downsample
            if ds is None:
                shortcut = x
            elif isinstance(ds, nn.Sequential) and len(ds) == 2 and isinstance(ds[0], nn.Conv2d):
                shortcut = conv_bn_act(ds[0], ds[1], x, relu=False)
            else:
                shortcut = ds(x)
        return bn_act(self.bn2, self.conv2(y), shortcut)


class Bottleneck(nn.Module):
    expansion = 4

    def __init__(self, inplanes, planes, stride=1, downsample=None):
        super().__init__()
        self.conv1 = _conv(inplanes, planes, 1)
        self.bn1 = BatchNorm(planes)
        self.conv2 = _conv(planes, planes, 3, stride, 1)
        self.bn2 = BatchNorm(planes)
        self.conv3 = _conv(planes, planes * 4, 1)
        self.bn3 = BatchNorm(planes * 4)
        self.relu = nn.ReLU(inplace=True)
        self.downsample = downsample
        self.stride = stride

    def _shortcut(self, x):
        ds = self.downsample
        if ds is None:
            return x
        if isinstance(ds, nn.Sequential) and len(ds) == 2 and isinstance(ds[0], nn.Conv2d):
            return conv_bn_act(ds[0], ds[1], x, relu=False)
        return ds(x)

    def _fused(self, x):
        if FUSED_BLOCK_OFF or FUSED_1X1_OFF or _FP8_1X1[0] or not (self.training and x.is_cuda and torch.is_grad_enabled()):
            return None
        if not (torch.is_autocast_enabled() and torch.get_autocast_gpu_dtype() == torch.bfloat16):
            return None
        ds = self.downsample
        bns = [self.bn1, self.bn2, self.bn3]
        wd = bnd = None
        if ds is not None:
            if not (isinstance(ds, nn.Sequential) and len(ds) == 2 and isinstance(ds[0], nn.Conv2d) and ds[0].kernel_size == (1, 1)
                    and ds[0].bias is None and ds[0].stride == (self.stride, self.stride)):
                return None
            wd, bnd = ds[0].weight, ds[1]
            bns.append(bnd)
        if not all(isinstance(b, BatchNorm) and b._sync is None and b._hip_ok_params() for b in bns):
            return None
        if any(cv.bias is not None or cv.groups != 1 for cv in (self.conv1, self.conv2, self.conv3)):
            return None
        bf = lambda w: w if w.dtype == torch.bfloat16 else w.to(torch.bfloat16)
        xb = _dense_cl(x if x.dtype == torch.bfloat16 else x.to(torch.bfloat16))
        w1, w2, w3 = bf(self.conv1.weight), bf(self.conv2.weight), bf(self.conv3.weight)
        wd = bf(wd) if wd is not None else None
        if not _ops().bottleneck_supported(xb, w1, w2, w3, self.bn1.weight, wd, self.stride):
            return None
        g = _BN_GROUPS[0]
        for b in bns:
            b._pending += g
        return _ops().bottleneck(xb, w1, self.bn1, w2, self.bn2, w3, self.bn3, wd, bnd, groups=g, stride=self.stride)

    def forward(self, x):
        y = self._fused(x)
        if y is not None:
            return y
        y = conv_bn_act(self.conv1, self.bn1, x)
        y = bn_act(self.bn2, self.conv2(y))
        return conv_bn_act(self.conv3, self.bn3, y, self._shortcut(x))


class ResNet(nn.Module):

    def __init__(self, block, layers, num_classes=1000, in_channels=3):
        super().__init__()
        self.inplanes = 64
        self.conv1 = _conv(in_channels, 64, 7, 2, 3)
        self.bn1 = BatchNorm(64)
        self.relu = nn.ReLU(inplace=True)
        self.maxpool = nn.MaxPool2d(kernel_size=3, stride=2, padding=1)
        self.layer1 = self._make_layer(block, 64, layers[0])
        self.layer2 = self._make_layer(block, 128, layers[1], stride=2)
        self.layer3 = self._make_layer(block, 256, layers[2], stride=2)
        self.layer4 = self._make_layer(block, 512, layers[3], stride=2)
        self.avgpool = nn.AdaptiveAvgPool2d((1, 1))
        self.fc = nn.Linear(512 * block.expansion, num_classes)
        init_resnet_weights(self)

    def _make_layer(self, block, planes, blocks, stride=1):
        out_ch = planes * block.expansion
        shortcut = None
        if stride != 1 or self.inplanes != out_ch:
            shortcut = nn.Sequential(_conv(self.inplanes, out_ch, 1, stride), BatchNorm(out_ch))
        stage = [block(self.inplanes, planes, stride, shortcut)]
        self.inplanes = out_ch
        stage += [block(out_ch, planes) for _ in range(1, blocks)]
        return nn.Sequential(*stage)

    def stem(self, x):
        return bn_act(self.bn1, self.conv1(x))

    def pool(self, x):
        if x.is_cuda and x.shape[1] % 8 == 0 and x.dtype in (torch.float32, torch.bfloat16) \
                and x.is_contiguous(memory_format=torch.channels_last) and not os.environ.get("TD_NO_HIP_STEM_POOL"):
            return _ops().maxpool3s2(x)
        _fell_back("ResNet.maxpool", x)
        return self.maxpool(x)

    def pyramid(self, x, extra=None):
        if extra is None:
            f0 = self.stem(x)
            f1 = self.layer1(self.pool(f0))
            f2 = self.layer2(f1)
            f3 = self.layer3(f2)
            return [f0, f1, f2, f3, self.layer4(f3)]
        f0 = self.stem(x) + extra[0]
        f1 = self.layer1(self.pool(f0)) + extra[1]
        f2 = self.layer2(f1) + extra[2]
        f3 = self.layer3(f2) + extra[3]
        f4 = self.layer4(f3) + extra[4]
        return [f0, f1, f2, f3, f4]

    def forward(self, x):
        return self.pyramid(x)[-1]


def init_resnet_weights(net):
    for m in net.modules():
        if isinstance(m, nn.Conv2d):
            nn.init.kaiming_normal_(m.weight, mode="fan_out", nonlinearity="relu")
        elif isinstance(m, nn.BatchNorm2d):
            nn.init.constant_(m.weight, 1)
            nn.init.constant_(m.bias, 0)


def build_resnet(num_layers, in_channels=3):
    if num_layers not in RESNET_SPECS:
        raise ValueError("{} is not a valid number of resnet layers".format(num_layers))
    kind, layers = RESNET_SPECS[num_layers]
    return ResNet(BasicBlock if kind == "basic" else Bottleneck, list(layers), in_channels=in_channels)


def resnet18(pretrained_path=None):
    return _maybe_load(build_resnet(18), pretrained_path)


def resnet34(pretrained_path=None, **kw):
    return _maybe_load(build_resnet(34), pretrained_path, "resnet34.pth")


def resnet50(pretrained_path=None, **kw):
    return _maybe_load(build_resnet(50), pretrained_path, "resnet50.pth")


def resnet101(pretrained_path=None, **kw):
    return _maybe_load(build_resnet(101), pretrained_path, "resnet101.pth")


def _maybe_load(net, path, fname=None):
    if path is not None:
        import os
        full = os.path.join(path, fname) if fname else path
        net.load_state_dict(torch.load(full, map_location="cpu", weights_only=True))
    return net


def enc_channels(num_layers):
    ch = np.array([64, 64, 128, 256, 512])
    if num_layers > 34:
        ch[1:] *= 4
    return ch


def _load_encoder_weights(net, path, n_images=1):
    state = torch.load(path, map_location="cpu", weights_only=True)
    if n_images > 1:
        state["conv1.weight"] = torch.cat([state["conv1.weight"]] * n_images, 1) / n_images
    net.load_state_dict(state, strict=False)


class DepthEncoder(nn.Module):

    def __init__(self, num_layers, pretrained_path=None):
        super().__init__()
        self.num_ch_enc = enc_channels(num_layers)
        self.encoder = build_resnet(num_layers)
        if pretrained_path is not None:
            _load_encoder_weights(self.encoder, pretrained_path)

    def forward(self, input_image):
        self.features = self.encoder.pyramid((input_image - 0.45) / 0.225)
        return self.features


class PoseEncoder(nn.Module):

    def __init__(self, num_layers, pretrained_path=None, num_input_images=2):
        super().__init__()
        self.num_ch_enc = enc_channels(num_layers)
        self.encoder = build_resnet(num_layers, in_channels=3 * num_input_images)
        if pretrained_path is not None:
            _load_encoder_weights(self.encoder, pretrained_path, num_input_images)

    def forward(self, input_image):
        self.features = self.encoder.pyramid((input_image - 0.45) / 0.225)
        return self.features


class Encoder(nn.Module):

    def __init__(self, num_layers, pretrained_path=None):
        super().__init__()
        self.num_ch_enc = enc_channels(num_layers)
        self.encoder = build_resnet(num_layers)
        if pretrained_path is not None:
            _load_encoder_weights(self.encoder, pretrained_path)
        self.features = []

    def forward(self, input_image, input_features=None):
        self.features = self.encoder.pyramid(input_image, input_features)
        return self.features

    def stem_only(self, input_image):
        return self.encoder.stem(input_image)


class PoseDecoder(nn.Module):

    def __init__(self, num_ch_enc, stride=1):
        super().__init__()
        self.reduce = Conv2d(int(num_ch_enc[-1]), 256, 1)
        self.conv1 = nn.Conv2d(256, 256, 3, stride, 1)
        self.conv2 = nn.Conv2d(256, 256, 3, stride, 1)
        self.conv3 = nn.Conv2d(256, 6, 1)
        self.relu = nn.ReLU()

    def forward(self, input_features):
        x = self.relu(self.reduce(input_features[-1]))
        x = self.relu(self.conv1(x))
        x = self.relu(self.conv2(x))
        x = self.conv3(x).float()
        x = 0.01 * x.mean(3).mean(2).view(-1, 1, 1, 6)
        return x[..., :3], x[..., 3:]



def upsample(x):
    if x.is_cuda and torch.is_autocast_enabled():
        with torch.autocast("cuda", enabled=False):
            return F.interpolate(x, scale_factor=2, mode="nearest")
# ... 386 lines not shown
```

tripled-exploring-depth-estimation-with-self-supervised-representation-learning_amd/native.py:

```python
import ctypes
import os

import torch

from . import dispatch

_HERE = os.path.dirname(os.path.abspath(__file__))
LIB_PATH = os.path.join(_HERE, "lib", "libtripled_hip.so")

TD_MAX_SRC = 4

_PTRARR = ctypes.POINTER(ctypes.c_void_p)
_I, _F, _P = ctypes.c_int, ctypes.c_float, ctypes.c_void_p
_LLARR = ctypes.POINTER(ctypes.c_longlong)
_IARR = ctypes.POINTER(ctypes.c_int)
ABI_VERSION = 3

SIGNATURES = {
    "td_abi_version": (_I, []),
    "td_error_string": (ctypes.c_char_p, [_I]),
    "td_last_hip_error": (ctypes.c_char_p, []),
    "td_photo_num_blocks": (_I, [_I, _I, _I]),
    "td_photo_bwd_num_blocks": (_I, [_I, _I, _I]),
    "td_photo_identity": (_I, [_P, _PTRARR, _I, _I, _I, _I, _P, _P, _PTRARR, _P]),
    "td_photo_fwd": (_I, [_P, _PTRARR, _I, _P, _P, _P, _P, _P, _I, _I, _I, _I, _I, _F, _F, _P, _P, _P, _P, _P, _P]),
    "td_photo_bwd": (_I, [_P, _PTRARR, _P, _PTRARR, _I, _P, _P, _P, _P, _P, _I, _P, _F, _I, _I, _I, _I, _I, _F, _F, _P, _P, _P]),
    "td_pack_rgbx": (_I, [_P, _I, _I, _I, _P, _P]),
    "td_upsample_adjoint": (_I, [_P, _I, _I, _I, _I, _I, _P, _I, _P]),
    "td_upsample_adjoint_planes": (_I, [_P, _I, _I, _I, _I, _I, _I, _P, _I, _P]),
    "td_reduce_dP": (_I, [_P, _I, _I, _I, _I, _P, _P]),
    "td_sum_scaled": (_I, [_P, _I, _F, _P, _P]),
    "td_area_downsample": (_I, [_P, _I, _I, _I, _I, _I, _I, _P, _P]),
    "td_smooth_num_blocks": (_I, [_I, _I, _I]),
    "td_smooth_fwd": (_I, [_P, _P, _I, _I, _I, _I, _P, _P, _P]),
    "td_smooth_finish": (_I, [_P, _I, _I, _I, _F, _P, _P]),
    "td_smooth_bwd": (_I, [_P, _P, _P, _I, _I, _I, _I, _P, _F, _P, _P, _P, _I, _P]),
    "td_maxpool5_fwd": (_I, [_P, _I, _I, _I, _I, _I, _P, _P, _P]),
    "td_maxpool5_bwd": (_I, [_P, _P, _I, _I, _I, _I, _I, _P, _P]),
    "td_maxpool5_bwd_add": (_I, [_P, _P, _P, _I, _I, _I, _I, _I, _P, _P]),
    "td_conv1x1_fwd_sum": (_I, [_P, _P, ctypes.c_longlong, _I, _I, _P, _P, _P, _P]),
    "td_maxpool3s2_fwd": (_I, [_P, _I, _I, _I, _I, _I, _P, _P, _P]),
    "td_maxpool3s2_bwd": (_I, [_P, _P, _I, _I, _I, _I, _I, _P, _P]),
    "td_join_fwd": (_I, [_P, _P, _P, _I, ctypes.c_longlong, _I, _I, _I, _P, _P]),
    "td_join_bwd": (_I, [_P, _I, ctypes.c_longlong, _I, _I, _I, _P, _P, _P, _P]),
    "td_join_up2_fwd": (_I, [_P, _P, _P, _I, _I, _I, _I, _I, _I, _I, _P, _P]),
    "td_join_up2_bwd": (_I, [_P, _I, _I, _I, _I, _I, _I, _I, _P, _P, _P, _P]),
    "td_bn_workspace_floats": (ctypes.c_longlong, [ctypes.c_longlong, _I, _I]),
    "td_bn_fwd": (_I, [_P, _P, _I, _P, _P, _P, _P, _F, _F, _I, ctypes.c_longlong, _I, _I, _P, _P, _P, _P, _P]),
    "td_conv1x1_stat_rows": (_I, [ctypes.c_longlong, _I, _I]),
    "td_conv1x1_fwd": (_I, [_P, _P, ctypes.c_longlong, _I, _I, _I, _I, _I, _I, _P, _P, _P]),
    "td_conv3x3_fwd": (_I, [_P, _P, _I, _I, _I, _I, _I, _I, _I, _I, _P, _P, _P]),
    "td_conv3x3_wgrad_workspace_floats": (ctypes.c_longlong, [_I, _I, _I, _I, _I]),
    "td_conv3x3_wgrad": (_I, [_P, _P, _I, _I, _I, _I, _I, _I, _I, _P, _P, _P]),
    "td_conv1x1_wgrad_workspace_floats": (ctypes.c_longlong, [ctypes.c_longlong, _I, _I]),
    "td_conv1x1_wgrad": (_I, [_P, _P, ctypes.c_longlong, _I, _I, _I, _I, _I, _I, _P, _P, _P]),
    "td_conv1x1_wgrad_group": (_I, [_I, _PTRARR, _PTRARR, _LLARR, _IARR, _IARR, _IARR, _IARR, _IARR, _IARR, _PTRARR, _PTRARR, _P]),
    "td_bn_fwd_from_partials": (_I, [_P, _P, _I, _P, _P, _P, _P, _F, _F, _I, ctypes.c_longlong, _I, _I, _P, _I, _P, _P, _P, _P]),
    "td_bias_act_workspace_floats": (ctypes.c_longlong, [ctypes.c_longlong, _I]),
    "td_bias_act_fwd": (_I, [_P, _P, _I, _I, ctypes.c_longlong, _I, _I, _P, _P]),
    "td_bias_act_bwd": (_I, [_P, _P, _I, ctypes.c_longlong, _I, _I, _P, _P, _I, _P, _P]),
    "td_gather_flat": (_I, [_PTRARR, _LLARR, _LLARR, _I, _I, _P, _P]),
    "td_adam_flat": (_I, [_P, _P, _P, _P, _P, ctypes.c_longlong, ctypes.c_longlong, _P, _P, _F, ctypes.c_double, ctypes.c_double, _F, _P, _F, _P]),
    "td_bn_partial_rows": (_I, [ctypes.c_longlong, _I, _I]),
    "td_bn_fwd_partials": (_I, [_P, _I, ctypes.c_longlong, _I, _I, _P, _P]),
    "td_bn_bwd_partials": (_I, [_P, _P, _P, _I, _P, _P, _P, _P, _I, ctypes.c_longlong, _I, _I, _P, _P]),
    "td_bn_bwd_from_partials": (_I, [_P, _P, _P, _I, _P, _P, _P, _P, _I, ctypes.c_longlong, _I, _I, _P, _I, _P, _P, _P, _P, _P]),
    "td_conv1x1_fwd_bnrelu": (_I, [_P, _P, ctypes.c_longlong, _I, _I, _I, _P, _I, _P, _P, _P, _P, _F, _F, _P, _P, _P, _P, _P, _P]),
    "td_conv1x1_dgrad": (_I, [_P, _P, ctypes.c_longlong, _I, _I, _I, _P, _P, _P]),
    "td_conv1x1_dgrad_bnsums": (_I, [_P, _P, ctypes.c_longlong, _I, _I, _I, _P, _P, _P, _P, _P, _P, _P, _P]),
    "td_conv1x1_dgrad_bnbwd": (_I, [_P, _P, _P, ctypes.c_longlong, _I, _I, _I, _P, _I, _P, _P, _P, _P, _P, _P, _P, _P, _P, _P]),
    "td_bn_bwd": (_I, [_P, _P, _P, _I, _P, _P, _P, _P, _I, ctypes.c_longlong, _I, _I, _P, _P, _P, _P, _P, _P]),
    "td_edge_weights": (_I, [_P, _I, _I, _I, _F, ctypes.POINTER(ctypes.c_float), _P, _P]),
    "td_featreg_num_blocks": (_I, [_I, _I, _I, _I]),
    "td_featreg_fwd": (_I, [_P, _I, _P, _I, _I, _I, _I, _P, _P]),
    "td_featreg_bwd": (_I, [_P, _I, _P, _P, _I, _I, _I, _I, _P, _P]),
    "td_recon_num_tasks": (_I, [_I, _I, _I]),
    "td_recon_fwd": (_I, [_P, _P, _P, _I, _I, _I, _P, _P]),
    "td_recon_bwd": (_I, [_P, _P, _P, _P, _I, _I, _I, _P, _P]),
    "td_reflpad1_fwd": (_I, [_P, _I, _I, _I, _I, _I, _P, _P]),
    "td_reflpad1_bwd": (_I, [_P, _I, _I, _I, _I, _I, _P, _P]),
    "td_up2_reflpad1_fwd": (_I, [_P, _I, _I, _I, _I, _I, _P, _P]),
    "td_up2_reflpad1_bwd": (_I, [_P, _I, _I, _I, _I, _I, _P, _P]),
    "td_featwarp_num_blocks": (_I, [_I, _I, _I]),
    "td_featwarp_fwd": (_I, [_P, _PTRARR, _I, _I, _P, _P, _P, _I, _I, _I, _I, _I, _I, _F, _F, _P, _P, _P]),
    "td_featwarp_bwd": (_I, [_P, _PTRARR, _I, _I, _P, _P, _P, _P, _P, _F, _I, _I, _I, _I, _I, _I, _F, _F, _P, _PTRARR,
                             _P, _P, _P]),
    "td_featwarp_dsrc_finish": (_I, [_P, _P, _F, _I, ctypes.c_longlong, _I, _P, _P]),
    "td_reduce_partials": (_I, [_P, _I, _I, _I, _P, _P]),
    "td_bn_sync_fwd_sums": (_I, [_P, _I, ctypes.c_longlong, _I, _I, _P, _P, _P]),
    "td_bn_sync_fwd_apply": (_I, [_P, _P, _I, _P, _P, _P, _P, _P, _P, _F, _F, _I, ctypes.c_longlong, _I, _I, _P, _P, _P, _P]),
    "td_bn_sync_bwd_sums": (_I, [_P, _P, _P, _I, _P, _P, _P, _P, _I, ctypes.c_longlong, _I, _I, _P, _P, _P]),
    "td_bn_sync_bwd_dx": (_I, [_P, _P, _P, _I, _P, _P, _P, _P, _P, _P, _P, _I, ctypes.c_longlong, _I, _I, _P, _P, _P, _P, _P, _P]),
    "td_fp8_num_blocks": (_I, [ctypes.c_longlong]),
    "td_fp8_amax_partials": (_I, [_P, _I, ctypes.c_longlong, _P, _P]),
    "td_fp8_quantize": (_I, [_P, _I, ctypes.c_longlong, _P, _P, _P, _P]),
    "td_color_jitter": (_I, [_P, _P, _I, _I, _I, _P, _P, _P, _P]),
    "td_l1map_fwd": (_I, [_P, _I, _LLARR, _P, _I, _I, _I, _I, _F, _P, _P]),
    "td_l1map_bwd": (_I, [_P, _I, _LLARR, _P, _P, _I, _I, _I, _I, _F, _P, _P]),
    "td_rgb2lab": (_I, [_P, _I, _I, _I, _F, _F, _F, _P, _P]),
    "td_pose_fwd": (_I, [_P, _P, _IARR, _P, _I, _I, _P, _P, _P]),
    "td_pose_bwd": (_I, [_P, _P, _IARR, _P, _I, _I, _P, _P, _P, _P, _P]),
    "td_infer_preprocess": (_I, [_P, _I, _I, _I, _I, _I, _I, _P, _P]),
    "td_disp_postprocess": (_I, [_P, _I, _I, _I, _I, _I, _I, _I, _F, _F, _F, _P, _P, _P]),
    "td_colorize": (_I, [_P, _I, ctypes.c_longlong, _P, _P, _P, _P, _P]),
    "td_eval_depth_workspace_bytes": (ctypes.c_longlong, [_I, _I, _I]),
    "td_eval_depth": (_I, [_P, _I, _I, _I, _I, _F, _F, _P, _I, _I, _P, _P, _F, _F, _I, _P, ctypes.c_longlong, _P, _P, _P]),
    "td_masked_median_workspace_bytes": (ctypes.c_longlong, [_I]),
    "td_masked_median": (_I, [_P, _I, ctypes.c_longlong, _P, ctypes.c_longlong, _P, _P, _P]),
    "td_pose_pairs_u8": (_I, [_P, _I, _I, _I, _I, _I, _I, _P, ctypes.c_longlong, _P]),
    "td_odom_trajectory": (_I, [_P, _I, _I, _P, _P]),
    "td_odom_snippet_ate": (_I, [_P, _I, _P, _I, _I, _P, _P]),
    "td_odom_sequence_errors": (_I, [_P, _P, _I, ctypes.POINTER(ctypes.c_double), _I, _I, _I, _P, _P, _P, _P, _P]),
    "td_lanczos_resize_u8": (_I, [_P, _P, _IARR, _P, ctypes.c_longlong, _IARR, _I, _I, _I, _I, _I, _I, _P, _P, _P]),
    "td_lanczos_resize_u8_indexed": (_I, [_P, ctypes.c_longlong, _P, _LLARR, _P, _IARR, _P, ctypes.c_longlong, _IARR, _I, _I, _I, _I, _P,
                                          _P, _P]),
    "td_cloud_keys": (_I, [_P, _P, _P, ctypes.POINTER(ctypes.c_double), _I, _I, _I, ctypes.c_double, ctypes.c_double, ctypes.c_double,
                           _I, _I, ctypes.c_double, ctypes.c_double, _F, _P, _P, _P, _P]),
    "td_cloud_heads": (_I, [_P, ctypes.c_longlong, _P, _P]),
    "td_cloud_reduce_packed": (_I, [_P, _P, _P, _P, ctypes.c_longlong, ctypes.c_longlong, ctypes.c_longlong, _P, _P, _P]),
    "td_cloud_reduce_rows": (_I, [_P, _P, _P, _P, ctypes.c_longlong, ctypes.c_longlong, ctypes.c_longlong, _P, _P, _P]),
    "td_cloud_finish": (_I, [_P, _P, ctypes.c_longlong, ctypes.c_double, ctypes.c_longlong, _P, _P, _P, _P, _P]),
    "td_cloud_views": (_I, [_P, _P, ctypes.POINTER(ctypes.c_double), ctypes.POINTER(ctypes.c_double), _I, _I, _I, _I, _I, _I, _I, _I, _I,
                            ctypes.c_double, ctypes.c_double, ctypes.c_double, ctypes.c_double, ctypes.c_double, _P, _P, _P, _P, _P]),
    "td_velo_depth_workspace_bytes": (ctypes.c_longlong, [_I, _I, _I]),
    "td_velo_depth": (_I, [_P, _P, _I, _P, _P, _I, _I, _I, _P, ctypes.c_longlong, _P, _P, _P]),
    "td_cloud_render_workspace_bytes": (ctypes.c_longlong, [_I, _I, _I]),
    "td_cloud_render": (_I, [_P, _P, ctypes.c_longlong, _P, ctypes.POINTER(ctypes.c_double), _I, _I, _I, ctypes.c_double, ctypes.c_double,
                             ctypes.c_double, ctypes.c_double, _I, _I, _I, _I, _P, ctypes.c_longlong, _P, _P, _P, _P, _P]),
    "td_scan_keys": (_I, [_P, ctypes.c_longlong, _P, _I, ctypes.POINTER(ctypes.c_double), _P, ctypes.POINTER(ctypes.c_double), _I, _I,
                          ctypes.c_double, ctypes.c_double, ctypes.c_double, _P, _P, _P, _P]),
    "td_nn_query": (_I, [_P, ctypes.c_longlong, _P, _P, ctypes.c_longlong, _P, _P, ctypes.c_longlong, ctypes.c_double,
                         ctypes.POINTER(ctypes.c_double), _I, _P, _P, _P, _P]),
    "td_cloud_transform": (_I, [_P, ctypes.c_longlong, ctypes.c_double, ctypes.POINTER(ctypes.c_double), ctypes.POINTER(ctypes.c_double),
                                _P, _P]),
    "td_icp_moments_workspace": (ctypes.c_longlong, [ctypes.c_longlong]),
    "td_icp_moments": (_I, [_P, ctypes.c_longlong, _P, ctypes.c_longlong, _P, _P, ctypes.c_double, ctypes.POINTER(ctypes.c_double), _P,
                            ctypes.c_longlong, _P, _P]),
    "td_cloud_normals": (_I, [_P, ctypes.c_longlong, _P, ctypes.c_longlong, _P, _P, ctypes.c_longlong, ctypes.c_double, ctypes.c_double,
                              ctypes.c_double, ctypes.c_longlong, ctypes.c_double, _P, _P, _P, _P, _P]),
    "td_icp_plane_moments_workspace": (ctypes.c_longlong, [ctypes.c_longlong]),
    "td_icp_plane_moments": (_I, [_P, ctypes.c_longlong, _P, _P, ctypes.c_longlong, _P, _P, ctypes.c_double,
                                  ctypes.POINTER(ctypes.c_double), _P, ctypes.c_longlong, _P, _P]),
    "td_normals_orient": (_I, [_P, _P, ctypes.c_longlong, _P, _I, ctypes.c_double, _P, _P, _P, _P]),
    "td_cloud_render_surfels": (_I, [_P, _P, _P, ctypes.c_longlong, _P, ctypes.POINTER(ctypes.c_double), _I, _I, _I, ctypes.c_double,
                                     ctypes.c_double, ctypes.c_double, ctypes.c_double, _I, _I, ctypes.c_double, _I, _I, _I, _I, _P,
                                     ctypes.c_longlong, _P, _P, _P, _P, _P, _P]),
}

DTYPE_CODES = {torch.float32: 0, torch.bfloat16: 1}


class NativeLibraryError(RuntimeError):
    pass


_lib = None


def load(path=None):
    global _lib
    if _lib is not None:
        return _lib
    path = path or os.environ.get("TD_HIP_LIB") or LIB_PATH
    if not os.path.exists(path):
        raise NativeLibraryError(
            "libtripled_hip.so not found at %s -- build it with `python -c 'import __graft_entry__ as g; "
            "g.build()'` or `make -C <package>/csrc`; there is no non-HIP fallback" % path)
    try:
        lib = ctypes.CDLL(path)
    except OSError as e:
        raise NativeLibraryError("cannot load %s: %s" % (path, e)) from e
    for name, (res, args) in SIGNATURES.items():
        try:
            fn = getattr(lib, name)
        except AttributeError as e:
            raise NativeLibraryError("%s does not export %s" % (path, name)) from e
        fn.restype = res
        fn.argtypes = args
    if lib.td_abi_version() != ABI_VERSION:
        raise NativeLibraryError("ABI version mismatch: library %d, binding %d" % (lib.td_abi_version(), ABI_VERSION))
    _lib = lib
    return lib


def check(code, what):
    dispatch.hip(what)
    if code != 0:
        lib = load()
        msg = lib.td_error_string(code).decode()
        hip = lib.td_last_hip_error().decode()
        raise NativeLibraryError("%s failed: %s (%d)%s" % (what, msg, code, (" [" + hip + "]") if hip else ""))


def require_device(*tensors):
    for t in tensors:
        if not t.is_cuda:
            raise NativeLibraryError("libtripled_hip needs device tensors (got a %s tensor)" % t.device)


def ptr(t):
    if t is None:
        return None
    require_device(t)
    if not t.is_contiguous():
        raise NativeLibraryError("libtripled_hip needs contiguous tensors")
    return ctypes.c_void_p(t.data_ptr())


def ptr_array(tensors):
    arr = (ctypes.c_void_p * len(tensors))()
    for i, t in enumerate(tensors):
        arr[i] = t.data_ptr()
    return arr


def stream():
    return ctypes.c_void_p(torch._C._cuda_getCurrentRawStream(torch.cuda.current_device()))


_PLANS = {}


def _plan(name):
# ... 42 lines not shown
```

tripled-exploring-depth-estimation-with-self-supervised-representation-learning_amd/ops.py:

```python
import ctypes
import os
import types

import torch

from . import native
from .native import call

_CL = torch.channels_last


def _f32c(t):
    if t.dtype != torch.float32:
        t = t.float()
    return t if t.is_contiguous() else t.contiguous()


def _f32(n, like):
    return torch.empty(n, device=like.device, dtype=torch.float32)


def _cl(t, dtype=None):
    return (t if dtype is None else t.to(dtype)).contiguous(memory_format=_CL)

# ... 432 lines not shown
        y, mean, invstd = _bn_apply(yc, part, S, weight, bias, st, residual, relu, groups)
        ctx.save_for_backward(x, w, yc, y if (relu and residual is not None) else None, weight, bias, mean, invstd)
        ctx.relu, ctx.has_res, ctx.groups, ctx.stride = bool(relu), residual is not None, groups, stride
        return y

    @staticmethod
    def backward(ctx, dy):
        x, w, yc, y, weight, bias, mean, invstd = ctx.saved_tensors
        Nb, N, Ho, Wo = yc.shape
        dyc, dres, dgamma, dbeta = _bn_backward(_cl(dy, yc.dtype), yc, y, weight, bias, mean, invstd, ctx.relu, ctx.has_res,
                                                ctx.groups)
        dx = dw = None
        if ctx.needs_input_grad[0]:
            dx = torch.ops.aten.convolution_backward(dyc, x, w, None, [ctx.stride, ctx.stride], [0, 0], [1, 1], False, [0, 0], 1,
                                                     [True, False, False])[0]
        if ctx.needs_input_grad[1]:
            K, Hi, Wi = x.shape[1], x.shape[2], x.shape[3]
            dw = conv1x1_wgrad(dyc, x, w, Nb * Ho * Wo, K, N, Hi, Wi, ctx.stride)
        return dx, dw, dgamma.to(weight.dtype), dbeta.to(weight.dtype), None, None, dres, None, None, None, None, None


def conv1x1_bn_act_supported(x, w, bn_weight, stride=1):
    return (_cl_tensor(x, 64, _BF16) and w.dim() == 4 and _weight_1x1_ok(w)
            and w.shape[2] == 1 and w.shape[3] == 1 and w.shape[1] == x.shape[1] and w.shape[0] % 64 == 0
            and stride in (1, 2) and bn_weight is not None and bn_weight.dtype == torch.float32)


def conv1x1_bn_act(x, w, weight, bias, running_mean, running_var, momentum, eps, residual=None, relu=False, groups=1, stride=1):
    if x.shape[0] % groups:
        raise ValueError("batch %d is not %d stacked passes" % (x.shape[0], groups))
    if not conv1x1_bn_act_supported(x, w, weight, stride):
        raise native.NativeLibraryError("conv1x1_bn_act needs bf16 channels_last HIP tensors with Cin % 64 == Cout % 64 == 0")
    return _Conv1x1BatchNormAct.apply(x, w, weight, bias, running_mean, running_var, _residual(residual, x), momentum, eps, relu,
                                      groups, stride)


ACT_CODES = {None: 0, "elu": 1, "leaky_relu": 2}


class _ConvBiasAct(torch.autograd.Function):

    @staticmethod
    def forward(ctx, x, w, b, act):
        y = _cl(torch.ops.aten.convolution(x, w, None, [1, 1], [0, 0], [1, 1], False, [0, 0], 1))
        B, C, H, W = y.shape
        call("td_bias_act_fwd", y, b, b.dtype if b is not None else 0, y.dtype, B * H * W, C, ACT_CODES[act], y)
        ctx.save_for_backward(x, w, y if act is not None else None, b)
        ctx.act = act
        return y

    @staticmethod
    def backward(ctx, g):
        x, w, a, b = ctx.saved_tensors
        B, C, H, W = g.shape
        g = _cl(g, w.dtype)
        M = B * H * W
        gy = torch.empty_like(g, memory_format=_CL) if ctx.act is not None else g
        db = torch.empty_like(b) if b is not None and ctx.needs_input_grad[2] else None
        ws = _f32(native.load().td_bias_act_workspace_floats(M, C), g)
        if ctx.act is not None or db is not None:
            call("td_bias_act_bwd", g, a, g.dtype, M, C, ACT_CODES[ctx.act], gy if ctx.act is not None else None, db,
                 db.dtype if db is not None else 0, ws)
        dx, dw, _ = torch.ops.aten.convolution_backward(gy, x, w, None, [1, 1], [0, 0], [1, 1], False, [0, 0], 1,
                                                        [ctx.needs_input_grad[0], ctx.needs_input_grad[1], False])
        return dx, dw, db, None


def conv_bias_act_supported(x, w, b, act):
    cout = w.shape[0]
    return (act in ACT_CODES and _cl_tensor(x, 1, _BF16) and w.dtype == torch.bfloat16
            and (b is None or b.dtype in native.DTYPE_CODES)
            and 8 <= cout <= 256 and cout % 8 == 0 and 256 % (cout // 8) == 0 and x.shape[1] == w.shape[1])


def conv_bias_act(x, w, b, act=None):
    if not conv_bias_act_supported(x, w, b, act):
        raise native.NativeLibraryError("conv_bias_act needs bf16 channels_last HIP tensors, Cout in {8, 16, 32, 64, 128, 256}")
    return _ConvBiasAct.apply(x, w, b, act)


_WGRAD_QUEUE = None
WGRAD_GROUP = os.environ.get("TD_WGRAD_GROUP", "node")


class wgrad_group:

    def __init__(self, assign=False, scope="node"):
        self.assign, self.scope, self.items = assign, scope, []

    def __enter__(self):
        global _WGRAD_QUEUE
        self.prev = _WGRAD_QUEUE
        self.active = WGRAD_GROUP == self.scope and not (self.prev is not None and self.prev.assign)
        if self.active:
            _WGRAD_QUEUE = self
        return self

    def __exit__(self, *exc):
        global _WGRAD_QUEUE
        if self.active:
            _WGRAD_QUEUE = self.prev
            if self.items and exc[0] is None:
                flush_wgrads(self.items)
        return False


def deferred_wgrads():
    return wgrad_group(assign=True, scope="step")


def flush_wgrads(queue):
    ints = lambda key: native.int_array([q[key] for q in queue])
    tensors = lambda key: [q[key] for q in queue]
    call("td_conv1x1_wgrad_group", len(queue), tensors("dy"), tensors("x"), (ctypes.c_longlong * len(queue))(*[q["M"] for q in queue]),
         ints("K"), ints("N"), ints("Hi"), ints("Wi"), ints("stride"),
         native.int_array([native.DTYPE_CODES[q["dw"].dtype] for q in queue]), tensors("dw"), tensors("ws"))
    for q in queue:
        w = q["w"]
        if w is None:
            continue
        if w.grad is None:
            w.grad = q["dw"]
        else:
            w.grad.add_(q["dw"])


def conv1x1_wgrad(dz, inp, w, M, K, N, Hi, Wi, stride):
    dw = torch.empty_like(w)
    wsw = _f32(native.load().td_conv1x1_wgrad_workspace_floats(M, K, N), dz)
    q = _WGRAD_QUEUE
    if q is not None and (not q.assign or (w.is_leaf and w.requires_grad)):
        q.items.append(dict(dy=dz, x=inp, dw=dw, ws=wsw, w=w if q.assign else None, M=M, K=K, N=N, Hi=Hi, Wi=Wi, stride=stride))
        return None if q.assign else dw
    call("td_conv1x1_wgrad", dz, inp, M, K, N, Hi, Wi, stride, w.dtype, dw, wsw)
    return dw


def conv3x3_wgrad_wins(B, Ho, Wo, C, N, stride):
    return stride == 1 and C == 64 and N == 64 and Wo >= 160 and Ho >= 48 and B * Ho * Wo < (1 << 31) - 128


def conv3x3_wgrad(dy, x, w, pad):
    B, N, Ho, Wo = dy.shape
    C = x.shape[1]
    dw = torch.empty_like(w, memory_format=_CL)
    ws = _f32(native.load().td_conv3x3_wgrad_workspace_floats(B, Ho, Wo, C, N), x)
    call("td_conv3x3_wgrad", dy, x, B, Ho, Wo, C, N, pad, w.dtype, dw, ws)
    return dw


class _Bottleneck(torch.autograd.Function):

    @staticmethod
    def forward(ctx, x, w1, w2, w3, g1, b1, g2, b2, g3, b3, wd, gd, bd, st1, st2, st3, std, groups, stride):
        lib = native.load()
        Nb = x.shape[0]
        c, Cout = w1.shape[0], w3.shape[0]

        z1, p1, S1 = _conv1x1_stats(x, w1, groups, 1)
        a1, mean1, invstd1 = _bn_apply(z1, p1, S1, g1, b1, st1, None, True, groups)
        z2 = _cl(torch.ops.aten.convolution(a1, w2, None, [stride, stride], [1, 1], [1, 1], False, [0, 0], 1))
        Ho, Wo = z2.shape[2], z2.shape[3]
        M2 = Nb * Ho * Wo
        R2 = lib.td_bn_partial_rows(M2, groups, c)
        p2 = _f32(groups * R2 * c * 2, x)
        call("td_bn_fwd_partials", z2, z2.dtype, M2, groups, c, p2)
        z3 = _empty_cl(Nb, Cout, Ho, Wo, x, torch.bfloat16)
        a2 = _empty_cl(Nb, c, Ho, Wo, x, torch.bfloat16)
        S3 = lib.td_conv1x1_stat_rows(M2, groups, Cout)
        p3 = _f32(groups * S3 * Cout * 2, x)
        mean2, invstd2 = _f32(groups * c, x), _f32(groups * c, x)
        call("td_conv1x1_fwd_bnrelu", z2, w3, M2, groups, c, Cout, p2, R2, g2, b2, st2.running_mean, st2.running_var, st2.momentum,
             st2.eps, mean2, invstd2, a2, z3, p3)
        zd = meand = invstdd = None
        if wd is not None:
            zd, pd, Sd = _conv1x1_stats(x, wd, groups, stride)
            shortcut, meand, invstdd = _bn_apply(zd, pd, Sd, gd, bd, std, None, False, groups)
        else:
            shortcut = x
        y, mean3, invstd3 = _bn_apply(z3, p3, S3, g3, b3, st3, shortcut, True, groups)
        ctx.save_for_backward(x, w1, w2, w3, g1, b1, g2, b2, g3, b3, wd, gd, bd, z1, a1, z2, a2, z3, y, zd, mean1, invstd1,
                              mean2, invstd2, mean3, invstd3, meand, invstdd)
        ctx.groups, ctx.stride = groups, stride
        return y

    @staticmethod
    def backward(ctx, dy):
        with wgrad_group():
            return _Bottleneck._backward(ctx, dy)

    @staticmethod
    def _backward(ctx, dy):
        lib = native.load()
        (x, w1, w2, w3, g1, b1, g2, b2, g3, b3, wd, gd, bd, z1, a1, z2, a2, z3, y, zd, mean1, invstd1, mean2, invstd2, mean3,
         invstd3, meand, invstdd) = ctx.saved_tensors
        groups, stride = ctx.groups, ctx.stride
        Nb, Cin, H, W = x.shape
        c, Cout = w1.shape[0], w3.shape[0]
        Ho, Wo = z2.shape[2], z2.shape[3]
        M1, M2 = Nb * H * W, Nb * Ho * Wo
        BF = torch.bfloat16
        dy = _cl(dy, BF)

        wgrad = conv1x1_wgrad

        dz3, dres, dg3, db3 = _bn_backward(dy, z3, y, g3, b3, mean3, invstd3, True, True, groups)
        da2 = torch.empty_like(z2, memory_format=_CL)
        S2 = lib.td_conv1x1_stat_rows(M2, groups, c)
        q2 = _f32(groups * S2 * c * 2, x)
        call("td_conv1x1_dgrad_bnsums", dz3, w3, M2, groups, Cout, c, z2, g2, b2, mean2, invstd2, da2, q2)
        dw3 = wgrad(dz3, a2, w3, M2, c, Cout, Ho, Wo, 1)
        dz2 = torch.empty_like(z2, memory_format=_CL)
        dg2, db2 = _f32(c, x), _f32(c, x)
        call("td_bn_bwd_from_partials", da2, z2, None, BF, g2, b2, mean2, invstd2, 1, M2, groups, c, q2, S2, dz2, None, dg2, db2)
        own_wgrad = conv3x3_wgrad_wins(Nb, Ho, Wo, c, c, stride)
        da1, dw2, _ = torch.ops.aten.convolution_backward(dz2, a1, w2, None, [stride, stride], [1, 1], [1, 1], False, [0, 0], 1,
                                                          [True, not own_wgrad, False])
        if own_wgrad:
            dw2 = conv3x3_wgrad(dz2, a1, w2, pad=1)
        da1 = _cl(da1)
        R1 = lib.td_bn_partial_rows(M1, groups, c)
        q1 = _f32(groups * R1 * c * 2, x)
        call("td_bn_bwd_partials", da1, z1, None, BF, g1, b1, mean1, invstd1, 1, M1, groups, c, q1)
        dwd = dgd = dbd = None
        if wd is not None:
            dzd, _, dgd, dbd = _bn_backward(dres, zd, None, gd, bd, meand, invstdd, False, False, groups)
            if stride == 1:
                res_in = torch.empty_like(x, memory_format=_CL)
                call("td_conv1x1_dgrad", dzd, wd, M2, groups, Cout, Cin, None, res_in)
            else:
                res_in = _cl(torch.ops.aten.convolution_backward(dzd, x, wd, None, [stride, stride], [0, 0], [1, 1], False, [0, 0],
                                                                 1, [True, False, False])[0], BF)
            dwd = wgrad(dzd, x, wd, M2, Cin, Cout, H, W, stride)
        else:
            res_in = dres
        dx = torch.empty_like(x, memory_format=_CL)
        dz1 = torch.empty_like(z1, memory_format=_CL)
        dg1, db1 = _f32(c, x), _f32(c, x)
        call("td_conv1x1_dgrad_bnbwd", da1, z1, w1, M1, groups, c, Cin, q1, R1, g1, b1, mean1, invstd1, dg1, db1, dz1, res_in, dx)
        dw1 = wgrad(dz1, x, w1, M1, Cin, c, H, W, 1)
        cast = lambda t, like: None if t is None else t.to(like.dtype)
        return (dx, dw1, dw2, dw3, cast(dg1, g1), cast(db1, b1), cast(dg2, g2), cast(db2, b2), cast(dg3, g3), cast(db3, b3),
                dwd, cast(dgd, gd) if gd is not None else None, cast(dbd, bd) if bd is not None else None,
                None, None, None, None, None, None)


def bottleneck_supported(x, w1, w2, w3, g1, wd=None, stride=1):
    c = w1.shape[0]
    return (_cl_tensor(x, 64, _BF16) and _weight_1x1_ok(w1) and _weight_1x1_ok(w3)
            and w2.dtype == torch.bfloat16 and w2.is_contiguous(memory_format=_CL) and g1.dtype == torch.float32
            and c % 64 == 0 and c <= 512 and w3.shape[0] % 64 == 0 and stride in (1, 2)
            and tuple(w1.shape[1:]) == (x.shape[1], 1, 1) and tuple(w3.shape[1:]) == (c, 1, 1) and tuple(w2.shape) == (c, c, 3, 3)
            and (wd is None or (_weight_1x1_ok(wd) and tuple(wd.shape) == (w3.shape[0], x.shape[1], 1, 1)))
            and (wd is not None or (stride == 1 and w3.shape[0] == x.shape[1])))


def bottleneck(x, w1, bn1, w2, bn2, w3, bn3, wd=None, bnd=None, groups=1, stride=1):
    if x.shape[0] % groups:
        raise ValueError("batch %d is not %d stacked passes" % (x.shape[0], groups))
    if not bottleneck_supported(x, w1, w2, w3, bn1.weight, wd, stride):
        raise native.NativeLibraryError("bottleneck needs bf16 channels_last HIP tensors, channels % 64 == 0, planes <= 512")
    return _Bottleneck.apply(x, w1, w2, w3, bn1.weight, bn1.bias, bn2.weight, bn2.bias, bn3.weight, bn3.bias, wd,
                             bnd.weight if bnd is not None else None, bnd.bias if bnd is not None else None,
                             BnState(bn1), BnState(bn2), BnState(bn3), BnState(bnd) if bnd is not None else None, groups, stride)


def batchnorm_act_supported(x, weight):
    return _cl_tensor(x, 64) and weight is not None and weight.dtype == torch.float32


def batchnorm_act(x, weight, bias, running_mean, running_var, momentum, eps, residual=None, relu=False, groups=1):
    if x.shape[0] % groups:
        raise ValueError("batch %d is not %d stacked passes" % (x.shape[0], groups))
    if not batchnorm_act_supported(x, weight):
        raise native.NativeLibraryError("batchnorm_act needs a channels_last f32/bf16 HIP tensor with C % 64 == 0")
    return _BatchNormAct.apply(x, weight, bias, running_mean, running_var, _residual(residual, x), momentum, eps, relu, groups)


class _SyncBatchNormAct(torch.autograd.Function):

    @staticmethod
    def forward(ctx, x, weight, bias, running_mean, running_var, residual, momentum, eps, relu, groups, process_group):
        import torch.distributed as dist
        N, C, H, W = x.shape
        M = N * H * W
        packed = _f32(groups * C * 2 + 1, x)
        ws = _f32(native.load().td_bn_workspace_floats(M, groups, C), x)
        call("td_bn_sync_fwd_sums", x, x.dtype, M, groups, C, packed, ws)
        packed[-1:].fill_(float(M // groups))
        dist.all_reduce(packed, op=dist.ReduceOp.SUM, group=process_group)
        y = torch.empty_like(x, memory_format=_CL)
        mean, invstd = _f32(groups * C, x), _f32(groups * C, x)
        call("td_bn_sync_fwd_apply", x, residual, x.dtype, packed, packed[-1:], weight, bias, running_mean, running_var,
             float(momentum), float(eps), int(relu), M, groups, C, y, mean, invstd)
        ctx.save_for_backward(x, y if (relu and residual is not None) else None, weight, bias, mean, invstd, packed[-1:].clone())
        ctx.relu, ctx.has_res, ctx.groups, ctx.group = bool(relu), residual is not None, groups, process_group
        return y

    @staticmethod
    def backward(ctx, dy):
        import torch.distributed as dist
        x, y, weight, bias, mean, invstd, count = ctx.saved_tensors
        N, C, H, W = x.shape
        M = N * H * W
        G = ctx.groups
        dy = _cl(dy, x.dtype)
        local = _f32(G * C * 2, x)
        ws = _f32(native.load().td_bn_workspace_floats(M, G, C), x)
        call("td_bn_sync_bwd_sums", dy, x, y, x.dtype, weight, bias, mean, invstd, int(ctx.relu), M, G, C, local, ws)
        total = local.clone()
        dist.all_reduce(total, op=dist.ReduceOp.SUM, group=ctx.group)
        dx = torch.empty_like(x, memory_format=_CL)
        buf, dres = _dres(x, dy, ctx.has_res, ctx.relu)
        dgamma, dbeta, coef = _f32(C, x), _f32(C, x), _f32(G * C * 3, x)
        call("td_bn_sync_bwd_dx", dy, x, y, x.dtype, local, total, count, weight, bias, mean, invstd, int(ctx.relu), M, G, C, dx, buf,
             dgamma, dbeta, coef)
        return dx, dgamma.to(weight.dtype), dbeta.to(weight.dtype), None, None, dres, None, None, None, None, None


def sync_batchnorm_act(x, weight, bias, running_mean, running_var, momentum, eps, process_group, residual=None, relu=False,
                       groups=1):
    if x.shape[0] % groups:
        raise ValueError("batch %d is not %d stacked passes" % (x.shape[0], groups))
    if not batchnorm_act_supported(x, weight):
        raise native.NativeLibraryError("sync_batchnorm_act needs a channels_last f32/bf16 HIP tensor with C % 64 == 0")
    return _SyncBatchNormAct.apply(x, weight, bias, running_mean, running_var, _residual(residual, x), momentum, eps, relu, groups,
                                   process_group)


def edge_weights(img_at_scale, a, scale6):
    img = _f32c(img_at_scale.detach())
    B, _, h, w = img.shape
    out = torch.empty(B, 6, h, w, device=img.device, dtype=torch.float32)
    call("td_edge_weights", img, B, h, w, float(a), (ctypes.c_float * 6)(*[float(v) for v in scale6]), out)
    return out


class _FeatReg(torch.autograd.Function):
    @staticmethod
    def forward(ctx, feat, Wt):
        B, C, h, w = feat.shape
        nblk = native.load().td_featreg_num_blocks(B, h, w, C)
        partial, loss = _f32(nblk, feat), _f32(1, feat)
        call("td_featreg_fwd", feat, feat.dtype, Wt, B, h, w, C, partial)
        call("td_sum_scaled", partial, nblk, 1.0, loss)
        ctx.save_for_backward(feat, Wt)
        return loss.reshape(())

    @staticmethod
    def backward(ctx, g):
        feat, Wt = ctx.saved_tensors
        B, C, h, w = feat.shape
        grad = torch.empty_like(feat, memory_format=_CL)
        call("td_featreg_bwd", feat, feat.dtype, Wt, _f32c(g.reshape(1)), B, h, w, C, grad)
        return grad, None


def featreg_supported(feat):
    return _cl_tensor(feat, 8) and feat.shape[2] >= 3 and feat.shape[3] >= 3


def feature_regularization(feat, img_at_scale, dis, cvt):
    B, C, h, w = feat.shape
    n = float(B * C)
    counts = [n * h * (w - 1), n * (h - 1) * w, n * h * (w - 2), n * (h - 1) * (w - 1), n * (h - 1) * (w - 1),
              n * (h - 2) * w]
    coef = [-dis, -dis, cvt, cvt, cvt, cvt]
    Wt = edge_weights(img_at_scale, 1.0, [c / k for c, k in zip(coef, counts)])
    return _FeatReg.apply(feat, Wt)


class _ReconSum(torch.autograd.Function):
    @staticmethod
    def forward(ctx, x, y, hole):
        B, _, h, w = x.shape
        n = native.load().td_recon_num_tasks(B, h, w)
        partial, out = _f32(n, x), _f32(1, x)
        call("td_recon_fwd", x, y, hole, B, h, w, partial)
        call("td_sum_scaled", partial, n, 1.0, out)
        ctx.save_for_backward(x, y, hole)
        return out.reshape(())

    @staticmethod
    def backward(ctx, g):
        x, y, hole = ctx.saved_tensors
        B, _, h, w = x.shape
        dx = torch.empty_like(x)
        call("td_recon_bwd", x, y, hole, _f32c(g.reshape(1)), B, h, w, dx)
        return dx, None, None


def masked_reconstruction_sum(pred, target, hole):
    if pred.shape[2] < 3 or pred.shape[3] < 3:
        raise native.NativeLibraryError("masked_reconstruction_sum needs h, w >= 3")
    pred = pred.float().contiguous()
    return _ReconSum.apply(pred, _f32c(target.detach()), _f32c(hole.detach()))


def _pad_fwd(name, x, Ho, Wo):
    N, C, H, W = x.shape
    out = _empty_cl(N, C, Ho, Wo, x)
    call(name, x, x.dtype, N, H, W, C, out)
    return out


def _pad_bwd(name, g, H, W):
    N, C = g.shape[:2]
    g = _cl(g)
    gin = _empty_cl(N, C, H, W, g)
    call(name, g, g.dtype, N, H, W, C, gin)
    return gin


class _ReflPad1(torch.autograd.Function):
    @staticmethod
    def forward(ctx, x):
        return _pad_fwd("td_reflpad1_fwd", x, x.shape[2] + 2, x.shape[3] + 2)
# ... 231 lines not shown
```

Before: 438.6.

## Fuse bn3 backward apply into conv1x1 dgrad prologue inside bottleneck stages

```diff
diff --git a/include/tripled_hip.h b/include/tripled_hip.h
--- a/include/tripled_hip.h
+++ b/include/tripled_hip.h
@@ -159,6 +159,15 @@
 int td_conv1x1_dgrad_bnbwd(const void* g, const void* z, const void* w, long long M, int groups, int Cout, int Cin, float* in_partials,
                            int in_rows, const float* gamma, const float* beta, const float* save_mean, const float* save_invstd,
                            float* dgamma, float* dbeta, void* dz_side, const void* residual, void* dx, td_stream_t stream);
+int td_bn_bwd_partials_dres_rows(long long M, int groups, int C);
+int td_bn_bwd_partials_dres(const void* dy, const void* x, const void* y, int dtype, const float* gamma, const float* beta,
+                            const float* save_mean, const float* save_invstd, int relu, long long M, int groups, int C, float* partials,
+                            void* dresidual, td_stream_t stream);
+int td_conv1x1_dgrad_bnbwd_masked(const void* g, const void* z, const void* w, long long M, int groups, int Cout, int Cin,
+                                  float* in_partials, int in_rows, int finish_rows, const float* gamma, const float* save_mean,
+                                  const float* save_invstd, float* dgamma, float* dbeta, void* dz_side, const void* ez,
+                                  const float* egamma, const float* ebeta, const float* emean, const float* einvstd, float* out_partials,
+                                  void* dx, td_stream_t stream);
 
 int td_bn_sync_fwd_sums(const void* x, int dtype, long long M, int groups, int C, float* sums, float* workspace,
                         td_stream_t stream);
diff --git a/tripled-exploring-depth-estimation-with-self-supervised-representation-learning_amd/csrc/td_bn.hip b/tripled-exploring-depth-estimation-with-self-supervised-representation-learning_amd/csrc/td_bn.hip
--- a/tripled-exploring-depth-estimation-with-self-supervised-representation-learning_amd/csrc/td_bn.hip
+++ b/tripled-exploring-depth-estimation-with-self-supervised-representation-learning_amd/csrc/td_bn.hip
@@ -9,13 +9,13 @@
 constexpr int BN_UNROLL = 4;
 constexpr int BN_THREADS = 256;
 
-template <typename T, int MODE>
+template <typename T, int MODE, bool DRES = false>
 __global__ __launch_bounds__(BN_THREADS) void bn_partials_kernel(const T* __restrict__ x, const T* __restrict__ dy,
                                                                  const T* __restrict__ y, const float* __restrict__ mean,
                                                                  const float* __restrict__ invstd, const float* __restrict__ gamma,
                                                                  const float* __restrict__ beta,
                                                                  long long M, int C, int rows_per_split, int relu,
-                                                                 float* __restrict__ ws) {
+                                                                 float* __restrict__ ws, T* __restrict__ dres = nullptr) {
   __shared__ float lds[2][BN_RY][64 + 1];
   const int tid = threadIdx.x, cx = tid & 7, ry = tid >> 3;
   const int cg = blockIdx.x, s = blockIdx.y, grp = blockIdx.z;
@@ -55,6 +55,7 @@
     }
 #pragma unroll
     for (int u = 0; u < BN_UNROLL; ++u) {
+      float gm[8];
 #pragma unroll
       for (int i = 0; i < 8; ++i) {
         if (MODE == 0) {
@@ -65,10 +66,14 @@
           float g = vg[u][i];
           if (relu == 1) g = vy[u][i] <= 0.f ? 0.f : g;
           if (relu == 2) g = fmaf(vx[u][i], sc[i], sh[i]) <= 0.f ? 0.f : g;
+          gm[i] = g;
           g = ok[u] ? g : 0.f;
           a[i] += g;
           b[i] = fmaf(g, vx[u][i] - mu[i], b[i]);
         }
+      }
+      if constexpr (DRES && MODE == 1) {
+        if (ok[u]) store8(dres + (size_t)(r + (long long)u * BN_RY) * C + col, gm);
       }
     }
   }
@@ -497,14 +502,17 @@
 
 template <typename T>
 static int run_bn_partials(int mode, const void* x, const void* dy, const void* y, const float* gamma, const float* beta, const float* mean,
-                           const float* invstd, int relu, long long M, int G, int C, float* ws, hipStream_t st) {
+                           const float* invstd, int relu, long long M, int G, int C, float* ws, hipStream_t st, void* dres = nullptr) {
   const long long Mg = M / G;
-  const int S = bn_stat_splits(Mg, C), rps = bn_rows_per_split(Mg, S);
+  const int S = dres ? bn_splits(Mg, C, BN_STAT_BLOCKS, 512) : bn_stat_splits(Mg, C), rps = bn_rows_per_split(Mg, S);
   const int S_eff = (int)((Mg + rps - 1) / rps);
   if (mode == 0)
     hipLaunchKernelGGL((bn_partials_kernel<T, 0>), dim3(C / 64, S_eff, G), dim3(BN_THREADS), 0, st, (const T*)x, (const T*)nullptr,
                        (const T*)nullptr, (const float*)nullptr, (const float*)nullptr, (const float*)nullptr, (const float*)nullptr, Mg, C,
                        rps, 0, ws);
+  else if (dres)
+    hipLaunchKernelGGL((bn_partials_kernel<T, 1, true>), dim3(C / 64, S_eff, G), dim3(BN_THREADS), 0, st, (const T*)x, (const T*)dy,
+                       (const T*)y, mean, invstd, gamma, beta, Mg, C, rps, relu, ws, (T*)dres);
   else
     hipLaunchKernelGGL((bn_partials_kernel<T, 1>), dim3(C / 64, S_eff, G), dim3(BN_THREADS), 0, st, (const T*)x, (const T*)dy,
                        (const T*)y, mean, invstd, gamma, beta, Mg, C, rps, relu, ws);
@@ -692,6 +700,27 @@
   return TD_ERR_UNSUPPORTED;
 }
 
+extern "C" int td_bn_bwd_partials_dres_rows(long long M, int groups, int C) {
+  if (!bn_shape_ok(M, groups, C) || C % 64 != 0) return 0;
+  const long long Mg = M / groups;
+  const int rps = td::bn_rows_per_split(Mg, td::bn_splits(Mg, C, td::BN_STAT_BLOCKS, 512));
+  return (int)((Mg + rps - 1) / rps);
+}
+extern "C" int td_bn_bwd_partials_dres(const void* dy, const void* x, const void* y, int dtype, const float* gamma, const float* beta,
+                                       const float* save_mean, const float* save_invstd, int relu, long long M, int groups, int C,
+                                       float* partials, void* dresidual, td_stream_t stream) {
+  if (!dy || !x || !gamma || !save_mean || !save_invstd || !partials || !dresidual || !bn_shape_ok(M, groups, C)) return TD_ERR_BAD_ARG;
+  if (relu < 0 || relu > 1 || (relu && !y && !beta)) return TD_ERR_BAD_ARG;
+  if (relu && !y) relu = 2;
+  if (C % 64 != 0 || M * (long long)C >= (1ll << 40)) return TD_ERR_UNSUPPORTED;
+  if (dtype == TD_DTYPE_BF16)
+    return td::run_bn_partials<__hip_bfloat16>(1, x, dy, y, gamma, beta, save_mean, save_invstd, relu, M, groups, C, partials, (hipStream_t)stream,
+                                               dresidual);
+  if (dtype == TD_DTYPE_F32)
+    return td::run_bn_partials<float>(1, x, dy, y, gamma, beta, save_mean, save_invstd, relu, M, groups, C, partials, (hipStream_t)stream, dresidual);
+  return TD_ERR_UNSUPPORTED;
+}
+
 extern "C" int td_bn_bwd_from_partials(const void* dy, const void* x, const void* y, int dtype, const float* gamma, const float* beta,
                                        const float* save_mean, const float* save_invstd, int relu, long long M, int groups, int C,
                                        float* partials, int stat_rows, void* dx, void* dresidual, float* dgamma, float* dbeta,
diff --git a/tripled-exploring-depth-estimation-with-self-supervised-representation-learning_amd/csrc/td_conv1x1.hip b/tripled-exploring-depth-estimation-with-self-supervised-representation-learning_amd/csrc/td_conv1x1.hip
--- a/tripled-exploring-depth-estimation-with-self-supervised-representation-learning_amd/csrc/td_conv1x1.hip
+++ b/tripled-exploring-depth-estimation-with-self-supervised-representation-learning_amd/csrc/td_conv1x1.hip
@@ -34,6 +34,8 @@
 
 constexpr int CV_PRO_MAX_K = 512;
 constexpr int CV_PRO_MAX_S = 16;
+constexpr int CV_PRO3_MAX_K = 2048;
+constexpr int cv_pro_floats(int pro) { return pro == 0 ? 4 : pro == 1 ? 2 * CV_PRO_MAX_K : pro == 2 ? 5 * CV_PRO_MAX_K : 3 * CV_PRO3_MAX_K; }
 
 __device__ __forceinline__ uint4 cv_pro1(uint4 x, const float* sc, const float* sh) {
   const unsigned w[4] = {x.x, x.y, x.z, x.w};
@@ -64,6 +66,19 @@
   }
   return make_uint4(o[0], o[1], o[2], o[3]);
 }
+__device__ __forceinline__ uint4 cv_pro3(uint4 g, uint4 z, const float* k0, const float* k1, const float* k2) {
+  const unsigned gw[4] = {g.x, g.y, g.z, g.w}, zw[4] = {z.x, z.y, z.z, z.w};
+  unsigned o[4];
+#pragma unroll
+  for (int e = 0; e < 4; ++e) {
+    const float z0 = bf2f((unsigned short)(zw[e] & 0xffff)), z1 = bf2f((unsigned short)(zw[e] >> 16));
+    const float g0 = bf2f((unsigned short)(gw[e] & 0xffff)), g1 = bf2f((unsigned short)(gw[e] >> 16));
+    const float v0 = fmaf(k0[2 * e], g0, fmaf(k1[2 * e], z0, k2[2 * e]));
+    const float v1 = fmaf(k0[2 * e + 1], g1, fmaf(k1[2 * e + 1], z1, k2[2 * e + 1]));
+    o[e] = (unsigned)f2bf(v0) | ((unsigned)f2bf(v1) << 16);
+  }
+  return make_uint4(o[0], o[1], o[2], o[3]);
+}
 
 __device__ __forceinline__ void cv_sum_rows(const float* __restrict__ part, int S, int stride, int K, int c, float& A, float& B) {
   float2 v[CV_PRO_MAX_S];
@@ -86,7 +101,8 @@
   using T = CvTile<BM, BN, BT>;
   constexpr int A_BYTES = T::A_BYTES, STAGE = T::STAGE, TN = T::TN, TM = T::TM;
   __shared__ __attribute__((aligned(16))) unsigned char lds[T::LDS_BYTES];
-  __shared__ __attribute__((aligned(16))) float s_pro[PRO == 0 ? 4 : (PRO == 1 ? 2 : 5) * CV_PRO_MAX_K];
+  __shared__ __attribute__((aligned(16))) float s_pro[cv_pro_floats(PRO)];
+  constexpr int PK = PRO == 3 ? CV_PRO3_MAX_K : CV_PRO_MAX_K;
 
   const int tid = threadIdx.x, lane = tid & 63, wid = tid >> 6;
   const int wm = wid >> 1, wn = wid & 1, l31 = lane & 31, h = lane >> 5;
@@ -127,8 +143,8 @@
     ra0##S = CV_LD(pa0, kt);                                   \
     ra1##S = CV_LD(pa1, kt);                                   \
     if (NA > 2) { ra2##S = CV_LD(pa2, kt); ra3##S = CV_LD(pa3, kt); } \
-    if constexpr (PRO == 2) {                                  \
-      rz0##S = CV_LD(fz.a2 + oa0, kt);                         \
+    if constexpr (PRO == 2 || PRO == 3) {                      \
+      rz0##S = CV_LD(fz.a2 + oa0, kt);                      \
       rz1##S = CV_LD(fz.a2 + oa1, kt);                         \
       if (NA > 2) { rz2##S = CV_LD(fz.a2 + oa2, kt); rz3##S = CV_LD(fz.a2 + oa3, kt); } \
     }                                                          \
@@ -148,19 +164,23 @@
       const int c0_ = (kt) * CV_BK + lc * 8;                                                            \
       float q0[8], q1[8], q2[8], q3[8], q4[8];                                                          \
       _Pragma("unroll") for (int e = 0; e < 8; ++e) {                                                   \
-        q0[e] = s_pro[0 * CV_PRO_MAX_K + c0_ + e];                                                      \
-        q1[e] = s_pro[1 * CV_PRO_MAX_K + c0_ + e];                                                      \
+        q0[e] = s_pro[0 * PK + c0_ + e];                                                                \
+        q1[e] = s_pro[1 * PK + c0_ + e];                                                                \
+        if constexpr (PRO == 2 || PRO == 3) q2[e] = s_pro[2 * PK + c0_ + e];                            \
         if constexpr (PRO == 2) {                                                                       \
-          q2[e] = s_pro[2 * CV_PRO_MAX_K + c0_ + e];                                                    \
-          q3[e] = s_pro[3 * CV_PRO_MAX_K + c0_ + e];                                                    \
-          q4[e] = s_pro[4 * CV_PRO_MAX_K + c0_ + e];                                                    \
+          q3[e] = s_pro[3 * PK + c0_ + e];                                                              \
+          q4[e] = s_pro[4 * PK + c0_ + e];                                                              \
         }                                                                                               \
       }                                                                                                 \
       if constexpr (PRO == 1) {                                                                         \
         ra0##S = cv_pro1(ra0##S, q0, q1);                                                               \
         ra1##S = cv_pro1(ra1##S, q0, q1);                                                               \
         if (NA > 2) { ra2##S = cv_pro1(ra2##S, q0, q1); ra3##S = cv_pro1(ra3##S, q0, q1); }             \
-      } else {                                                                                          \
+      } else if constexpr (PRO == 3) {                                                                  \
+        ra0##S = cv_pro3(ra0##S, rz0##S, q0, q1, q2);                                                   \
+        ra1##S = cv_pro3(ra1##S, rz1##S, q0, q1, q2);                                                   \
+        if (NA > 2) { ra2##S = cv_pro3(ra2##S, rz2##S, q0, q1, q2); ra3##S = cv_pro3(ra3##S, rz3##S, q0, q1, q2); } \
+      } else {                                                                                     \
         ra0##S = cv_pro2(ra0##S, rz0##S, q0, q1, q2, q3, q4);                                           \
         ra1##S = cv_pro2(ra1##S, rz1##S, q0, q1, q2, q3, q4);                                           \
         if (NA > 2) { ra2##S = cv_pro2(ra2##S, rz2##S, q0, q1, q2, q3, q4); ra3##S = cv_pro2(ra3##S, rz3##S, q0, q1, q2, q3, q4); } \
@@ -265,6 +285,40 @@
     }
     __syncthreads();
   }
+  if constexpr (PRO == 3) {
+    const float* part = fz.part + (size_t)grp * fz.part_rows * K * 2;
+    const float inv_m = 1.f / (float)Mg;
+    const bool first = (s == 0 && nt == 0 && grp == 0);
+    for (int c = tid; c < K; c += CV_THREADS) {
+      float A, B;
+      if (fz.part_S == 1) {
+        const float2 v = *reinterpret_cast<const float2*>(part + (size_t)c * 2);
+        A = v.x;
+        B = v.y;
+      } else {
+        cv_sum_rows(part, fz.part_S, fz.part_stride, K, c, A, B);
+      }
+      const float is = fz.invstd[(size_t)grp * K + c], mu = fz.mean[(size_t)grp * K + c];
+      const float dg = B * is;
+      const float c0 = fz.gamma[c] * is;
+      const float c1 = -c0 * is * dg * inv_m;
+      s_pro[0 * PK + c] = c0;
+      s_pro[1 * PK + c] = c1;
+      s_pro[2 * PK + c] = -c0 * A * inv_m - c1 * mu;
+      if (first) {
+        float dg_tot = 0.f, db_tot = 0.f;
+        for (int g2 = 0; g2 < fz.G; ++g2) {
+          float A2 = A, B2 = B;
+          if (g2 != 0) cv_sum_rows(fz.part + (size_t)g2 * fz.part_rows * K * 2, fz.part_S, fz.part_stride, K, c, A2, B2);
+          dg_tot += B2 * fz.invstd[(size_t)g2 * K + c];
+          db_tot += A2;
+        }
+        fz.dgamma[c] = dg_tot;
+        fz.dbeta[c] = db_tot;
+      }
+    }
+    __syncthreads();
+  }
 
   CV_WRITE_LDS(0, 0, A)
   __syncthreads();
@@ -543,12 +597,12 @@
   const long long Mg = M / G;
   ConvTile t = cv_pick_tile(Mg, G, N);
   const bool deep = K >= 3 * CV_BK;
-  if constexpr (PRO == 2) {
+  if constexpr (PRO == 2 || PRO == 3) {
     if (t.bm == 128 && t.bn == 128) t.bn = 64;
   } else
     if (t.bm == 128 && t.bn == 128) return cv_launch<128, 128, BT, PRO, EPI, false>(x, w, y, ws, Mg, G, K, N, geom, st, fz);
   if (t.bm == 128 && t.bn == 64) {
-    if constexpr (PRO == 0)
+    if constexpr (PRO == 0 || PRO == 3)
       if (deep) return cv_launch<128, 64, BT, PRO, EPI, true>(x, w, y, ws, Mg, G, K, N, geom, st, fz);
     return cv_launch<128, 64, BT, PRO, EPI, false>(x, w, y, ws, Mg, G, K, N, geom, st, fz);
   }
@@ -653,6 +707,28 @@
   const td::ConvRows geom = {0, 0, 0, 0, 1};
   if (residual) return td::cv_dispatch<true, 2, 1>(g, w, dx, nullptr, M, groups, Cout, Cin, geom, st, fz);
   return td::cv_dispatch<true, 2, 0>(g, w, dx, nullptr, M, groups, Cout, Cin, geom, st, fz);
+}
+
+extern "C" int td_conv1x1_dgrad_bnbwd_masked(const void* g, const void* z, const void* w, long long M, int groups, int Cout, int Cin,
+                                             float* in_partials, int in_rows, int finish_rows, const float* gamma, const float* save_mean,
+                                             const float* save_invstd, float* dgamma, float* dbeta, void* dz_side, const void* ez,
+                                             const float* egamma, const float* ebeta, const float* emean, const float* einvstd,
+                                             float* out_partials, void* dx, td_stream_t stream) {
+  if (!g || !z || !w || !dx || !in_partials || in_rows < 1 || finish_rows < 1 || finish_rows > td::CV_PRO_MAX_S || !gamma || !save_mean ||
+      !save_invstd || !dgamma || !dbeta || !cv_shape_ok(M, groups, Cout, Cin))
+    return TD_ERR_BAD_ARG;
+  if (ez && (!egamma || !ebeta || !emean || !einvstd || !out_partials)) return TD_ERR_BAD_ARG;
+  if (Cout > td::CV_PRO3_MAX_K || M * (long long)(Cout > Cin ? Cout : Cin) >= (1ll << 40)) return TD_ERR_UNSUPPORTED;
+  hipStream_t st = (hipStream_t)stream;
+  const td::BnRows rows = td::bn_shrink_partials_to(in_partials, in_rows, groups, Cout, finish_rows, st);
+  td::CvFuse fz = {};
+  fz.a2 = (const __hip_bfloat16*)z; fz.part = in_partials; fz.part_S = rows.n; fz.part_stride = rows.stride; fz.part_rows = in_rows;
+  fz.gamma = gamma; fz.mean = const_cast<float*>(save_mean); fz.invstd = const_cast<float*>(save_invstd);
+  fz.dgamma = dgamma; fz.dbeta = dbeta; fz.a_side = (__hip_bfloat16*)dz_side; fz.G = groups;
+  const td::ConvRows geom = {0, 0, 0, 0, 1};
+  if (!ez) return td::cv_dispatch<true, 3, 0>(g, w, dx, nullptr, M, groups, Cout, Cin, geom, st, fz);
+  fz.ep.z = (const __hip_bfloat16*)ez; fz.ep.gamma = egamma; fz.ep.beta = ebeta; fz.ep.mean = emean; fz.ep.invstd = einvstd;
+  return td::cv_dispatch<true, 3, 2>(g, w, dx, out_partials, M, groups, Cout, Cin, geom, st, fz);
 }
 
 extern "C" long long td_conv1x1_wgrad_workspace_floats(long long M, int K, int N) {
diff --git a/tripled-exploring-depth-estimation-with-self-supervised-representation-learning_amd/hostside/mono/model/networks.py b/tripled-exploring-depth-estimation-with-self-supervised-representation-learning_amd/hostside/mono/model/networks.py
--- a/tripled-exploring-depth-estimation-with-self-supervised-representation-learning_amd/hostside/mono/model/networks.py
+++ b/tripled-exploring-depth-estimation-with-self-supervised-representation-learning_amd/hostside/mono/model/networks.py
@@ -175,6 +175,8 @@
 
 FUSED_1X1_OFF = bool(os.environ.get("TD_NO_MFMA_1X1"))
 FUSED_BLOCK_OFF = bool(os.environ.get("TD_NO_FUSED_BLOCK"))
+BN3_GEMM_OFF = bool(os.environ.get("TD_NO_BN3_GEMM"))
+_IN_STAGE = [False]
 
 
 def conv_bn_act(conv, bn, x, residual=None, relu=True):
@@ -318,7 +320,8 @@
         g = _BN_GROUPS[0]
         for b in bns:
             b._pending += g
-        return _ops().bottleneck(xb, w1, self.bn1, w2, self.bn2, w3, self.bn3, wd, bnd, groups=g, stride=self.stride)
+        return _ops().bottleneck(xb, w1, self.bn1, w2, self.bn2, w3, self.bn3, wd, bnd, groups=g, stride=self.stride,
+                                 bn3_gemm=_IN_STAGE[0] and not BN3_GEMM_OFF)
 
     def forward(self, x):
         y = self._fused(x)
@@ -327,6 +330,17 @@
         y = conv_bn_act(self.conv1, self.bn1, x)
         y = bn_act(self.bn2, self.conv2(y))
         return conv_bn_act(self.conv3, self.bn3, y, self._shortcut(x))
+
+
+class BottleneckStage(nn.Sequential):
+
+    def forward(self, x):
+        prev = _IN_STAGE[0]
+        _IN_STAGE[0] = True
+        try:
+            return super().forward(x)
+        finally:
+            _IN_STAGE[0] = prev
 
 
 class ResNet(nn.Module):
@@ -354,7 +368,7 @@
         stage = [block(self.inplanes, planes, stride, shortcut)]
         self.inplanes = out_ch
         stage += [block(out_ch, planes) for _ in range(1, blocks)]
-        return nn.Sequential(*stage)
+        return BottleneckStage(*stage) if block is Bottleneck else nn.Sequential(*stage)
 
     def stem(self, x):
         return bn_act(self.bn1, self.conv1(x))
diff --git a/tripled-exploring-depth-estimation-with-self-supervised-representation-learning_amd/native.py b/tripled-exploring-depth-estimation-with-self-supervised-representation-learning_amd/native.py
--- a/tripled-exploring-depth-estimation-with-self-supervised-representation-learning_amd/native.py
+++ b/tripled-exploring-depth-estimation-with-self-supervised-representation-learning_amd/native.py
@@ -69,6 +69,10 @@
     "td_conv1x1_dgrad": (_I, [_P, _P, ctypes.c_longlong, _I, _I, _I, _P, _P, _P]),
     "td_conv1x1_dgrad_bnsums": (_I, [_P, _P, ctypes.c_longlong, _I, _I, _I, _P, _P, _P, _P, _P, _P, _P, _P]),
     "td_conv1x1_dgrad_bnbwd": (_I, [_P, _P, _P, ctypes.c_longlong, _I, _I, _I, _P, _I, _P, _P, _P, _P, _P, _P, _P, _P, _P, _P]),
+    "td_bn_bwd_partials_dres_rows": (_I, [ctypes.c_longlong, _I, _I]),
+    "td_bn_bwd_partials_dres": (_I, [_P, _P, _P, _I, _P, _P, _P, _P, _I, ctypes.c_longlong, _I, _I, _P, _P, _P]),
+    "td_conv1x1_dgrad_bnbwd_masked": (_I, [_P, _P, _P, ctypes.c_longlong, _I, _I, _I, _P, _I, _I, _P, _P, _P, _P, _P, _P, _P, _P, _P, _P, _P,
+                                           _P, _P, _P]),
     "td_bn_bwd": (_I, [_P, _P, _P, _I, _P, _P, _P, _P, _I, ctypes.c_longlong, _I, _I, _P, _P, _P, _P, _P, _P]),
     "td_edge_weights": (_I, [_P, _I, _I, _I, _F, ctypes.POINTER(ctypes.c_float), _P, _P]),
     "td_featreg_num_blocks": (_I, [_I, _I, _I, _I]),
diff --git a/tripled-exploring-depth-estimation-with-self-supervised-representation-learning_amd/ops.py b/tripled-exploring-depth-estimation-with-self-supervised-representation-learning_amd/ops.py
--- a/tripled-exploring-depth-estimation-with-self-supervised-representation-learning_amd/ops.py
+++ b/tripled-exploring-depth-estimation-with-self-supervised-representation-learning_amd/ops.py
@@ -608,7 +608,7 @@
 class _Bottleneck(torch.autograd.Function):
 
     @staticmethod
-    def forward(ctx, x, w1, w2, w3, g1, b1, g2, b2, g3, b3, wd, gd, bd, st1, st2, st3, std, groups, stride):
+    def forward(ctx, x, w1, w2, w3, g1, b1, g2, b2, g3, b3, wd, gd, bd, st1, st2, st3, std, groups, stride, bn3_gemm=False):
         lib = native.load()
         Nb = x.shape[0]
         c, Cout = w1.shape[0], w3.shape[0]
@@ -637,7 +637,7 @@
         y, mean3, invstd3 = _bn_apply(z3, p3, S3, g3, b3, st3, shortcut, True, groups)
         ctx.save_for_backward(x, w1, w2, w3, g1, b1, g2, b2, g3, b3, wd, gd, bd, z1, a1, z2, a2, z3, y, zd, mean1, invstd1,
                               mean2, invstd2, mean3, invstd3, meand, invstdd)
-        ctx.groups, ctx.stride = groups, stride
+        ctx.groups, ctx.stride, ctx.bn3_gemm = groups, stride, bool(bn3_gemm)
         return y
 
     @staticmethod
@@ -660,11 +660,23 @@
 
         wgrad = conv1x1_wgrad
 
-        dz3, dres, dg3, db3 = _bn_backward(dy, z3, y, g3, b3, mean3, invstd3, True, True, groups)
+        if ctx.bn3_gemm:
+            R3 = lib.td_bn_bwd_partials_dres_rows(M2, groups, Cout)
+            q3 = _f32(groups * R3 * Cout * 2, x)
+            dres = torch.empty_like(z3, memory_format=_CL)
+            call("td_bn_bwd_partials_dres", dy, z3, y, BF, g3, b3, mean3, invstd3, 1, M2, groups, Cout, q3, dres)
+            dz3 = torch.empty_like(z3, memory_format=_CL)
+            dg3, db3 = _f32(Cout, x), _f32(Cout, x)
+        else:
+            dz3, dres, dg3, db3 = _bn_backward(dy, z3, y, g3, b3, mean3, invstd3, True, True, groups)
         da2 = torch.empty_like(z2, memory_format=_CL)
         S2 = lib.td_conv1x1_stat_rows(M2, groups, c)
         q2 = _f32(groups * S2 * c * 2, x)
-        call("td_conv1x1_dgrad_bnsums", dz3, w3, M2, groups, Cout, c, z2, g2, b2, mean2, invstd2, da2, q2)
+        if ctx.bn3_gemm:
+            call("td_conv1x1_dgrad_bnbwd_masked", dres, z3, w3, M2, groups, Cout, c, q3, R3, bn3_finish_rows(Cout), g3, mean3, invstd3,
+                 dg3, db3, dz3, z2, g2, b2, mean2, invstd2, q2, da2)
+        else:
+            call("td_conv1x1_dgrad_bnsums", dz3, w3, M2, groups, Cout, c, z2, g2, b2, mean2, invstd2, da2, q2)
         dw3 = wgrad(dz3, a2, w3, M2, c, Cout, Ho, Wo, 1)
         dz2 = torch.empty_like(z2, memory_format=_CL)
         dg2, db2 = _f32(c, x), _f32(c, x)
@@ -679,7 +691,17 @@
         q1 = _f32(groups * R1 * c * 2, x)
         call("td_bn_bwd_partials", da1, z1, None, BF, g1, b1, mean1, invstd1, 1, M1, groups, c, q1)
         dwd = dgd = dbd = None
-        if wd is not None:
+        if wd is not None and stride == 1 and ctx.bn3_gemm:
+            Rd = lib.td_bn_partial_rows(M2, groups, Cout)
+            qd = _f32(groups * Rd * Cout * 2, x)
+            call("td_bn_bwd_partials", dres, zd, None, BF, gd, bd, meand, invstdd, 0, M2, groups, Cout, qd)
+            dzd = torch.empty_like(zd, memory_format=_CL)
+            dgd, dbd = _f32(Cout, x), _f32(Cout, x)
+            res_in = torch.empty_like(x, memory_format=_CL)
+            call("td_conv1x1_dgrad_bnbwd_masked", dres, zd, wd, M2, groups, Cout, Cin, qd, Rd, bn3_finish_rows(Cout), gd, meand, invstdd,
+                 dgd, dbd, dzd, None, None, None, None, None, None, res_in)
+            dwd = wgrad(dzd, x, wd, M2, Cin, Cout, H, W, stride)
+        elif wd is not None:
             dzd, _, dgd, dbd = _bn_backward(dres, zd, None, gd, bd, meand, invstdd, False, False, groups)
             if stride == 1:
                 res_in = torch.empty_like(x, memory_format=_CL)
@@ -698,7 +720,17 @@
         cast = lambda t, like: None if t is None else t.to(like.dtype)
         return (dx, dw1, dw2, dw3, cast(dg1, g1), cast(db1, b1), cast(dg2, g2), cast(db2, b2), cast(dg3, g3), cast(db3, b3),
                 dwd, cast(dgd, gd) if gd is not None else None, cast(dbd, bd) if bd is not None else None,
-                None, None, None, None, None, None)
+                None, None, None, None, None, None, None)
+
+
+BN3_FINISH_ROWS = int(os.environ.get("TD_BN3_FINISH_ROWS", "0"))
+
+
+def bn3_finish_rows(C):
+    return BN3_FINISH_ROWS or (16 if C <= 512 else 1)
+
+
+BN3_GEMM_MAX_C = int(os.environ.get("TD_BN3_GEMM_MAX_C", "512"))
 
 
 def bottleneck_supported(x, w1, w2, w3, g1, wd=None, stride=1):
@@ -711,14 +743,15 @@
             and (wd is not None or (stride == 1 and w3.shape[0] == x.shape[1])))
 
 
-def bottleneck(x, w1, bn1, w2, bn2, w3, bn3, wd=None, bnd=None, groups=1, stride=1):
+def bottleneck(x, w1, bn1, w2, bn2, w3, bn3, wd=None, bnd=None, groups=1, stride=1, bn3_gemm=False):
     if x.shape[0] % groups:
         raise ValueError("batch %d is not %d stacked passes" % (x.shape[0], groups))
     if not bottleneck_supported(x, w1, w2, w3, bn1.weight, wd, stride):
         raise native.NativeLibraryError("bottleneck needs bf16 channels_last HIP tensors, channels % 64 == 0, planes <= 512")
     return _Bottleneck.apply(x, w1, w2, w3, bn1.weight, bn1.bias, bn2.weight, bn2.bias, bn3.weight, bn3.bias, wd,
                              bnd.weight if bnd is not None else None, bnd.bias if bnd is not None else None,
-                             BnState(bn1), BnState(bn2), BnState(bn3), BnState(bnd) if bnd is not None else None, groups, stride)
+                             BnState(bn1), BnState(bn2), BnState(bn3), BnState(bnd) if bnd is not None else None, groups, stride,
+                             bn3_gemm and w3.shape[0] <= min(BN3_GEMM_MAX_C, 2048))
 
 
 def batchnorm_act_supported(x, weight):
```

Result: no change. 440.7 (median of 6 runs) (+0.5%).
